# mstebelev/wormhole

Hardware: AMD Instinct MI355X
Metric: examples/sec, DiFacto FM on Criteo-1TB-shaped sparse at 1/2/4/8 MI355X (higher is better)
Workload: dtype fp32; 1 GPU; model=difacto-fm-dim64, global_batch=100000, seq_len=39, parallelism=dp1+kvshard1, minibatch_per_gpu=100000, threshold=100, nnz_per_example=39

## Files before the change

csrc/bind/hip_ops.cc:

```cpp
#include <torch/extension.h>
#include <pybind11/stl.h>
#include <c10/core/DeviceGuard.h>
#include <c10/hip/HIPStream.h>
#include <c10/hip/HIPGuard.h>
#include <c10/hip/HIPCachingAllocator.h>
#include <hip/hip_runtime.h>
#include <torch/csrc/distributed/c10d/ProcessGroup.hpp>
#include <torch/csrc/distributed/c10d/Work.hpp>

#include <algorithm>
#include <map>
#include <array>
#include <cstdio>
#include <cstdlib>
#include <cstring>
#include <chrono>
#include <cmath>
#include <functional>
#include <deque>
#include <map>
#include <mutex>
#include <condition_variable>
#include <thread>
#include <memory>
// ... 603 lines not shown
    wh::kv_occupied(table(), ptr<int32_t>(out), ptr<int64_t>(n), cur_stream(keys_));
    return out.narrow(0, 0, n.item<int64_t>());
  }

  Tensor linear_pull(const Tensor& slot) {
    CHECK_IN(slot, torch::kInt32);
    c10::DeviceGuard g(slot.device());
    auto out = torch::empty({slot.numel()}, slot.options().dtype(torch::kFloat32));
    wh::linear_pull(table(), ptr<int32_t>(slot), slot.numel(), ptr<float>(out), cur_stream(slot));
    return out;
  }

  void linear_push(const Tensor& slot, const Tensor& grad, int64_t algo, double alpha, double beta,
                   double l1, double l2, double sgd_eta) {
    CHECK_IN(slot, torch::kInt32);
    CHECK_IN(grad, torch::kFloat32);
    TORCH_CHECK(grad.numel() >= slot.numel());
    c10::DeviceGuard g(slot.device());
    wh::LinearHP hp{(int)algo, (float)alpha, (float)beta, (float)l1, (float)l2, (float)sgd_eta};
    wh::linear_push(table(), ptr<int32_t>(slot), ptr<float>(grad), slot.numel(), hp,
                    cur_stream(slot));
  }

  static wh::DifactoHP dhp(const std::vector<double>& h, int64_t threshold, bool l1_shrk,
                           int64_t seed) {
    TORCH_CHECK(h.size() == 8, "difacto hyper-parameter vector must have 8 entries");
    wh::DifactoHP hp;
    hp.alpha = (float)h[0]; hp.beta = (float)h[1]; hp.l1 = (float)h[2]; hp.l2 = (float)h[3];
    hp.v_alpha = (float)h[4]; hp.v_beta = (float)h[5]; hp.v_l2 = (float)h[6];
    hp.v_init = (float)h[7];
    hp.threshold = (uint32_t)threshold;
    hp.l1_shrk = l1_shrk ? 1 : 0;
    hp.seed = (uint64_t)seed;
    return hp;
  }

  void difacto_push_cnt(const Tensor& slot, const Tensor& cnt, const std::vector<double>& h,
                        int64_t threshold, bool l1_shrk, int64_t seed) {
    CHECK_IN(slot, torch::kInt32);
    CHECK_DEV(cnt); CHECK_CONT(cnt);
    TORCH_CHECK(cnt.scalar_type() == torch::kFloat32 || cnt.scalar_type() == torch::kInt32,
                "counts must be float32 or int32");
    TORCH_CHECK(cnt.numel() >= slot.numel());
    c10::DeviceGuard g(slot.device());
    const bool f = cnt.scalar_type() == torch::kFloat32;
    wh::difacto_push_cnt(table(), ptr<int32_t>(slot), f ? ptr<float>(cnt) : nullptr,
                         f ? nullptr : ptr<int32_t>(cnt), slot.numel(),
                         dhp(h, threshold, l1_shrk, seed), cur_stream(slot));
  }

  std::vector<Tensor> difacto_pull(const Tensor& slot, bool l1_shrk) {
    CHECK_IN(slot, torch::kInt32);
    c10::DeviceGuard g(slot.device());
    auto s = cur_stream(slot);
    const int64_t n = slot.numel();
    auto f32 = slot.options().dtype(torch::kFloat32);
    auto hdr = torch::empty({n, 2}, f32);
    const int64_t mcap = vstride_ > 0 ? n : 0;
    auto vc = torch::empty({mcap, (int64_t)std::max(vstride_, 1)}, f32);
    if (n > 0) {
      auto vpos = torch::empty({n + 1}, slot.options().dtype(torch::kInt64));
      if (wh::difacto_pull_fused(table(), ptr<int32_t>(slot), n, l1_shrk ? 1 : 0,
                                 lookback(slot.device()), ptr<float>(hdr), ptr<int64_t>(vpos),
                                 ptr<float>(vc), s))
        return {hdr, vc, vpos};
    }
    auto vflag = torch::empty({std::max<int64_t>(n, 1)}, slot.options());
    auto vpos = torch::zeros({n + 1}, slot.options().dtype(torch::kInt64));
    wh::difacto_pull_hdr(table(), ptr<int32_t>(slot), n, l1_shrk ? 1 : 0, ptr<float>(hdr),
                         ptr<int32_t>(vflag), s);
    if (vstride_ > 0 && n > 0) {
      auto stmp = torch::empty({wh::scan_tmp_elems(n)}, vpos.options());
      wh::scan_i32(ptr<int32_t>(vflag), ptr<int64_t>(vpos), n, ptr<int64_t>(stmp), s);
      wh::difacto_pull_rows(table(), ptr<int32_t>(slot), n, ptr<int32_t>(vflag),
                            ptr<int64_t>(vpos), ptr<float>(hdr), ptr<float>(vc), s);
    }
    return {hdr, vc, vpos};
  }

  std::vector<Tensor> difacto_open_pull(const Tensor& keys, bool insert,
                                        const c10::optional<Tensor>& cnt,
                                        const std::vector<double>& h, int64_t threshold,
                                        bool l1_shrk, int64_t seed, bool direct) {
    CHECK_IN(keys, torch::kInt64);
    const int32_t* cp = nullptr;
    if (cnt.has_value() && cnt->defined()) {
      CHECK_IN((*cnt), torch::kInt32);
      TORCH_CHECK(cnt->numel() >= keys.numel(), "open_pull: count size mismatch");
      cp = ptr<int32_t>(*cnt);
    }
    c10::DeviceGuard g(keys.device());
    auto s = cur_stream(keys);
    const int64_t n = keys.numel();
    auto f32 = keys.options().dtype(torch::kFloat32);
    auto slot = torch::empty({n}, keys.options().dtype(torch::kInt32));
    auto hdr = torch::empty({n, 2}, f32);
    auto vpos = torch::empty({n + 1}, keys.options());
    direct = direct && vstride_ > 0;
    auto vc = direct ? V_ : torch::empty({vstride_ > 0 ? n : 0, (int64_t)std::max(vstride_, 1)}, f32);
    if (n == 0) {
      vpos.zero_();
      return {slot, hdr, vc, vpos};
    }
    if (!wh::difacto_open_pull(table(), reinterpret_cast<const uint64_t*>(keys.data_ptr()), n,
                               cp, dhp(h, threshold, l1_shrk, seed), insert ? 1 : 0,
                               lookback(keys.device()), ptr<int32_t>(slot), ptr<float>(hdr),
                               ptr<int64_t>(vpos), direct ? nullptr : ptr<float>(vc), s)) {
      slot = find(keys, insert);
      if (cp) difacto_push_cnt(slot, *cnt, h, threshold, l1_shrk, seed);
      auto r = difacto_pull(slot, l1_shrk);
      return {slot, r[0], r[1], r[2]};
    }
    return {slot, hdr, vc, vpos};
  }

  void difacto_push(const Tensor& slot, const Tensor& hdr, const Tensor& gw, const Tensor& gvc,
                    const std::vector<double>& h, int64_t threshold, bool l1_shrk,
                    int64_t seed) {
    CHECK_IN(slot, torch::kInt32);
    CHECK_IN(hdr, torch::kFloat32);
    CHECK_IN(gw, torch::kFloat32);
    CHECK_DEV(gvc); CHECK_CONT(gvc); CHECK_DT(gvc, torch::kFloat32);
    const int64_t n = slot.numel();
    TORCH_CHECK(hdr.numel() == 2 * n && gw.numel() == n, "push: hdr/gw size mismatch");
    TORCH_CHECK(vstride_ == 0 || (gvc.dim() == 2 && gvc.size(1) == vstride_),
                "push: gvc must be [m, vstride]");
    c10::DeviceGuard g(slot.device());
    wh::difacto_push(table(), ptr<int32_t>(slot), ptr<float>(hdr), ptr<float>(gw),
                     gvc.numel() ? ptr<float>(gvc) : nullptr, n, dhp(h, threshold, l1_shrk, seed),
                     cur_stream(slot));
  }

  std::vector<Tensor> ps_open(const Tensor& keys, bool use_cnt, const Tensor& segS,
                              const Tensor& segHS, int64_t rows_cap, bool insert, bool chains,
                              const std::vector<double>& h, int64_t threshold, bool l1_shrk,
                              int64_t seed, const c10::optional<Tensor>& chain_in = c10::nullopt) {
    CHECK_DEV(keys); CHECK_CONT(keys);
    CHECK_IN(segS, torch::kInt64);
    CHECK_IN(segHS, torch::kInt64);
    const bool rec = keys.scalar_type() == torch::kInt32;
    TORCH_CHECK(rec ? (keys.dim() == 2 && keys.size(1) == 3) : keys.scalar_type() == torch::kInt64,
                "ps_open: keys must be int64 [n] or int32 records [n, 3]");
    TORCH_CHECK(!use_cnt || rec, "ps_open: counts travel in the records");
    const int64_t n = keys.size(0);
    const int P = (int)segS.numel() - 1;
    TORCH_CHECK(P >= 1 && segHS.numel() == P + 1, "ps_open: bad segment tables");
    TORCH_CHECK(n < (1 << 24), "ps_open: at most 2^24 - 1 keys per minibatch and shard");
    epoch_ = epoch_ % 255 + 1;
    ++opens_;
    TORCH_CHECK(vstride_ == 0 || rows_cap >= n, "ps_open: reply buffer too small");
    c10::DeviceGuard g(keys.device());
    auto s = cur_stream(keys);
    auto i32 = keys.options().dtype(torch::kInt32);
    auto f32 = keys.options().dtype(torch::kFloat32);
    const int64_t n1 = std::max<int64_t>(n, 1);
    int64_t at = 0;
    auto carve = [&](int64_t bytes) {
      const int64_t o = at;
      at += (bytes + 255) / 256 * 256;
      return o;
    };
    const int64_t o_s = carve(n1 * 4), o_w = carve(n1 * 4), o_p = carve((n + 1) * 8),
                  o_h = carve(n1);
    auto blk = torch::empty({at}, keys.options().dtype(torch::kUInt8));
    auto slot = blk.narrow(0, o_s, n1 * 4).view(torch::kInt32);
    auto wout = blk.narrow(0, o_w, n1 * 4).view(torch::kFloat32);
    auto vpos = blk.narrow(0, o_p, (n + 1) * 8).view(torch::kInt64);
    const bool prepped = chain_in.has_value() && chain_in->defined() && chain_in->numel() > 0;
    if (prepped) {
      CHECK_IN((*chain_in), torch::kInt32);
      TORCH_CHECK(chain_in->numel() >= std::max<int64_t>(n, 1), "ps_open: prepped chain too small");
      TORCH_CHECK(vbase_.defined(), "ps_open: prepped without a push prep");
    }
    auto chain = prepped ? *chain_in : torch::empty({n1}, i32);
    auto head = blk.narrow(0, o_h, n1);
    auto rbuf = torch::empty({vstride_ > 0 ? rows_cap : 0, (int64_t)std::max(vstride_, 1)}, f32);
    Tensor vcnt;
    if (vstride_ == 0) {
      if (!vcnt0_.defined() || vcnt0_.numel() != P || vcnt0_.device() != keys.device())
        vcnt0_ = torch::zeros({P}, keys.options().dtype(torch::kInt64));
      vcnt = vcnt0_;
    } else {
      vcnt = torch::empty({P}, keys.options().dtype(torch::kInt64));
    }
    if (!vbase_.defined()) vbase_ = torch::empty({1}, vnext_.options());
    const bool ok = wh::ps_open(
        table(), rec ? nullptr : reinterpret_cast<const uint64_t*>(keys.data_ptr()),
        rec ? ptr<int32_t>(keys) : nullptr, n, use_cnt ? 1 : 0, dhp(h, threshold, l1_shrk, seed),
        insert ? 1 : 0, chains ? 1 : 0, (uint32_t)epoch_, ptr<int32_t>(vbase_),
        ptr<int64_t>(segS), ptr<int64_t>(segHS), P, lookback(keys.device()), ptr<int32_t>(slot),
        ptr<float>(wout), ptr<int64_t>(vpos), reinterpret_cast<uint32_t*>(chain.data_ptr()),
        reinterpret_cast<uint8_t*>(head.data_ptr()), ptr<float>(rbuf), ptr<int64_t>(vcnt), s,
        prepped ? 1 : 0);
    TORCH_CHECK(ok, "ps_open: limits exceeded (P <= 256, n < 2^24)");
    return {slot.narrow(0, 0, n), vpos, chain.narrow(0, 0, n), head.narrow(0, 0, n),
            vstride_ > 0 ? rbuf : wout.narrow(0, 0, n), vcnt};
  }

  wh::PsPrep push_prep(const c10::optional<Tensor>& prep_chain, int64_t prep_n) {
    wh::PsPrep pr;
    if (!(prep_chain.has_value() && prep_chain->defined() && prep_chain->numel() > 0)) return pr;
    CHECK_IN((*prep_chain), torch::kInt32);
    TORCH_CHECK(prep_n >= 0 && prep_n <= prep_chain->numel(), "push prep: chain too small");
    if (!vbase_.defined()) vbase_ = torch::empty({1}, vnext_.options());
    pr.chain = reinterpret_cast<uint32_t*>(prep_chain->data_ptr());
    pr.n = prep_n;
    pr.vbase = ptr<int32_t>(vbase_);
    return pr;
  }

  void ps_push_linear(const Tensor& slot, const c10::optional<Tensor>& chain,
                      const c10::optional<Tensor>& head, const Tensor& segS, const Tensor& g,
                      int64_t algo, double alpha, double beta, double l1, double l2, double t0,
// ... 123 lines not shown
  int64_t opens_ = 0;

 private:
  void set_slots(const Tensor& sl) {
    slots_ = sl;
    auto as_i64 = slots_.view(torch::kInt64);
    auto as_f32 = slots_.view(torch::kFloat32);
    keys_ = as_i64.select(1, 0);
    w_ = as_f32.select(1, 2);
    z_ = as_f32.select(1, 3);
    sq_ = as_f32.select(1, 4);
    vrow_ = slots_.select(1, 5);
    cnt_ = slots_.select(1, 6);
  }

  int64_t cap_ = 0, vcap_ = 0, dim_ = 0;
  int vstride_ = 0;
};

static void check_vstride(int64_t vstride) {
  TORCH_CHECK(vstride == 0 || (vstride >= 4 && vstride <= 256 && (vstride & (vstride - 1)) == 0),
              "vstride must be 0 or 4 * 2^k <= 256, got ", vstride);
}

std::vector<Tensor> fm_forward(const Tensor& offset, const Tensor& lid,
                               const c10::optional<Tensor>& val, const Tensor& w_or_hdr,
                               const c10::optional<Tensor>& vc, int64_t vstride,
                               const Tensor& label, int64_t loss, const Tensor& met) {
  check_vstride(vstride);
  CHECK_IN(offset, torch::kInt64);
  CHECK_IN(lid, torch::kInt32);
  CHECK_IN(w_or_hdr, torch::kFloat32);
  CHECK_IN(label, torch::kFloat32);
  CHECK_IN(met, torch::kFloat64);
  TORCH_CHECK(met.numel() >= 4, "met needs 4 doubles");
  const int64_t nrows = offset.numel() - 1;
  TORCH_CHECK(label.numel() == nrows, "label size mismatch");
  const float* vcp = nullptr;
  if (vstride > 0) {
    TORCH_CHECK(w_or_hdr.dim() == 2 && w_or_hdr.size(1) == 2, "hdr must be [U, 2]");
    TORCH_CHECK(vc.has_value() && vc->defined(), "vc required");
    CHECK_IN((*vc), torch::kFloat32);
    TORCH_CHECK(vc->numel() == 0 || (vc->dim() == 2 && vc->size(1) == vstride), "vc must be [m, vstride]");
    vcp = vc->numel() ? ptr<float>(*vc) : nullptr;
  }
  const float* vp = optptr<float>(val);
  c10::DeviceGuard g(offset.device());
  int64_t at = 0;
  auto carve = [&](int64_t bytes) {
    const int64_t o = at;
    at += (bytes + 255) / 256 * 256;
    return o;
  };
  const int64_t nxv = vstride > 0 ? nrows * vstride : 0;
  const int64_t o_py = carve(nrows * 4), o_du = carve(nrows * 4), o_xv = carve(nxv * 4),
                o_pt = carve(wh::fm_fwd_partials() * 8);
  auto blk = torch::empty({std::max<int64_t>(at, 256)}, offset.options().dtype(torch::kUInt8));
  auto py = blk.narrow(0, o_py, nrows * 4).view(torch::kFloat32);
  auto dual = blk.narrow(0, o_du, nrows * 4).view(torch::kFloat32);
  auto xv = blk.narrow(0, o_xv, nxv * 4).view(torch::kFloat32);
  auto part = blk.narrow(0, o_pt, wh::fm_fwd_partials() * 8).view(torch::kFloat64);
  const int lossf = (int)loss | (met.numel() >= 5 ? 256 : 0);
  wh::fm_forward(nrows, ptr<int64_t>(offset), ptr<int32_t>(lid), vp, ptr<float>(w_or_hdr), vcp,
                 (int)vstride, ptr<float>(label), lossf, ptr<float>(py), ptr<float>(dual),
                 vstride > 0 ? ptr<float>(xv) : nullptr, ptr<double>(met), ptr<double>(part),
                 ptr<unsigned int>(dev_ws(offset.device()).fwd_ticket), cur_stream(offset));
  return {py, dual, xv};
}

static std::vector<Tensor> fm_bwd_alloc(const Tensor& csc_off, int64_t nnz, int64_t vc_rows,
                                        int64_t vstride, bool from_ws) {
  auto f32 = csc_off.options().dtype(torch::kFloat32);
  auto u8 = csc_off.options().dtype(torch::kUInt8);
  const int64_t U = csc_off.numel() - 1;
  const int64_t need = wh::fm_bwd_layout(U, nnz, (int)vstride, deterministic());
  Tensor fresh;
  Tensor& scratch = from_ws ? dev_ws(csc_off.device()).bwd_scratch[cur_stream(csc_off)] : fresh;
  if (!scratch.defined() || scratch.numel() < need)
    scratch = torch::empty({from_ws ? need + need / 4 : need}, u8);
  return {torch::empty({U}, f32),
          vstride > 0 ? torch::empty({vc_rows, vstride}, f32) : torch::empty({0}, f32), scratch};
}

static void fm_bwd_launch(const std::vector<Tensor>& pl, const Tensor& csc_off,
                          const Tensor& csc_row, const float* csc_val, const float* dual,
                          const float* xv, const float* hdr, const float* vc, int64_t vstride,
                          int64_t nrows, wh::FmBwdPhase phase, bool two_pass = false) {
  wh::FmBwdProblem p;
  p.nuniq = csc_off.numel() - 1;
  p.nnz = csc_row.numel();
  p.nrows = nrows;
  p.csc_off = ptr<int64_t>(csc_off);
  p.csc_row = ptr<int32_t>(csc_row);
  p.csc_val = csc_val;
  p.dual = dual;
  p.xv = xv;
  p.hdr = hdr;
  p.vc = vc;
  p.vstride = (int)vstride;
  p.gw = ptr<float>(pl[0]);
  p.gvc = pl[1].numel() ? ptr<float>(pl[1]) : nullptr;
  p.deterministic = deterministic();
  const wh::Lookback lb = lookback(csc_off.device());
  wh::fm_backward(p, pl[2].data_ptr(), two_pass ? nullptr : &lb, cur_stream(csc_off), phase);
}

static void fm_bwd_check(const Tensor& csc_off, const Tensor& csc_row, const Tensor& w_or_hdr,
                         int64_t vstride) {
  check_vstride(vstride);
  CHECK_IN(csc_off, torch::kInt64);
  CHECK_IN(csc_row, torch::kInt32);
  CHECK_IN(w_or_hdr, torch::kFloat32);
  TORCH_CHECK(w_or_hdr.numel() == (csc_off.numel() - 1) * (vstride > 0 ? 2 : 1),
              "w/hdr must have U rows");
}

static int64_t fm_bwd_check_run(const Tensor& dual, const c10::optional<Tensor>& xv,
                                const c10::optional<Tensor>& vc, int64_t vstride) {
  CHECK_IN(dual, torch::kFloat32);
  if (vstride == 0) return 0;
  TORCH_CHECK(vc.has_value() && vc->defined() && xv.has_value() && xv->defined(), "vc/xv required");
  CHECK_IN((*vc), torch::kFloat32);
  CHECK_IN((*xv), torch::kFloat32);
  return vc->numel() ? vc->size(0) : 0;
}

std::vector<Tensor> fm_backward(const Tensor& csc_off, const Tensor& csc_row,
                                const c10::optional<Tensor>& csc_val, const Tensor& dual,
                                const c10::optional<Tensor>& xv, const Tensor& w_or_hdr,
                                const c10::optional<Tensor>& vc, int64_t vstride) {
  fm_bwd_check(csc_off, csc_row, w_or_hdr, vstride);
  const int64_t vrows = fm_bwd_check_run(dual, xv, vc, vstride);
  c10::DeviceGuard g(csc_off.device());
  auto pl = fm_bwd_alloc(csc_off, csc_row.numel(), vrows, vstride, true);
  fm_bwd_launch(pl, csc_off, csc_row, optptr<float>(csc_val), ptr<float>(dual),
                vstride > 0 ? optptr<float>(xv) : nullptr, ptr<float>(w_or_hdr),
                vstride > 0 ? optptr<float>(vc) : nullptr, vstride, dual.numel(),
                wh::FmBwdPhase::kAll);
  return {pl[0], pl[1]};
}

std::vector<Tensor> fm_backward_plan(const Tensor& csc_off, const Tensor& csc_row,
                                     const Tensor& w_or_hdr, int64_t vc_rows, int64_t nrows,
                                     int64_t vstride, bool two_pass) {
  fm_bwd_check(csc_off, csc_row, w_or_hdr, vstride);
  TORCH_CHECK(vc_rows >= 0 && nrows >= 0, "bad sizes");
  c10::DeviceGuard g(csc_off.device());
  auto pl = fm_bwd_alloc(csc_off, csc_row.numel(), vc_rows, vstride, false);
  fm_bwd_launch(pl, csc_off, csc_row, nullptr, nullptr, nullptr, ptr<float>(w_or_hdr), nullptr,
                vstride, nrows, wh::FmBwdPhase::kPlan, two_pass);
  return pl;
}

std::vector<Tensor> fm_backward_run(const std::vector<Tensor>& plan, const Tensor& csc_off,
                                    const Tensor& csc_row, const c10::optional<Tensor>& csc_val,
                                    const Tensor& dual, const c10::optional<Tensor>& xv,
                                    const Tensor& w_or_hdr, const c10::optional<Tensor>& vc,
                                    int64_t vstride) {
  fm_bwd_check(csc_off, csc_row, w_or_hdr, vstride);
  const int64_t vrows = fm_bwd_check_run(dual, xv, vc, vstride);
  TORCH_CHECK(plan.size() == 3, "fm_backward_run: not a backward plan");
  const Tensor &gw = plan[0], &gvc = plan[1], &scratch = plan[2];
  CHECK_IN(gw, torch::kFloat32);
  CHECK_IN(gvc, torch::kFloat32);
  CHECK_IN(scratch, torch::kUInt8);
  const int64_t U = csc_off.numel() - 1;
  TORCH_CHECK(gw.numel() == U, "fm_backward_run: U differs from the plan's");
  TORCH_CHECK(vstride > 0 ? gvc.dim() == 2 && gvc.size(0) == vrows && gvc.size(1) == vstride
                          : gvc.numel() == 0,
              "fm_backward_run: vc rows or vstride differ from the plan's");
  TORCH_CHECK(scratch.numel() == wh::fm_bwd_layout(U, csc_row.numel(), (int)vstride, deterministic()),
              "fm_backward_run: the plan was made for a CSC of another size");
  c10::DeviceGuard g(csc_off.device());
  for (const Tensor& t : plan)
    if (t.numel())
      c10::hip::HIPCachingAllocator::recordStream(
          t.storage().data_ptr(), c10::hip::getCurrentHIPStream(csc_off.device().index()));
  fm_bwd_launch(plan, csc_off, csc_row, optptr<float>(csc_val), ptr<float>(dual),
                vstride > 0 ? optptr<float>(xv) : nullptr, ptr<float>(w_or_hdr),
                vstride > 0 ? optptr<float>(vc) : nullptr, vstride, dual.numel(),
                wh::FmBwdPhase::kRun);
  return {gw, gvc};
}

void fm_grad_post(const Tensor& gvc, const Tensor& m, int64_t dim, double clip, double dropout,
                  int64_t seed, bool normalize) {
  CHECK_IN(gvc, torch::kFloat32);
  CHECK_IN(m, torch::kInt64);
  if (gvc.numel() == 0) return;
  TORCH_CHECK(gvc.dim() == 2, "gvc must be [m, vstride]");
  const int64_t vstride = gvc.size(1);
  c10::DeviceGuard g(gvc.device());
  auto s = cur_stream(gvc);
  Tensor sumsq;
  if (normalize) sumsq = torch::zeros({1}, gvc.options().dtype(torch::kFloat64));
  wh::fm_grad_post(ptr<int64_t>(m), gvc.size(0), ptr<float>(gvc), (int)vstride, (int)dim,
                   (float)clip, (float)dropout, (uint64_t)seed,
                   normalize ? ptr<double>(sumsq) : nullptr, s);
  if (normalize)
    wh::fm_grad_scale(ptr<int64_t>(m), gvc.size(0), ptr<float>(gvc), (int)vstride, (int)dim,
                      ptr<double>(sumsq), s);
}

std::vector<Tensor> ps_unpack(const Tensor& rbuf, int64_t U, const Tensor& segS,
                              const Tensor& segHS, const Tensor& vrecv) {
  CHECK_IN(rbuf, torch::kFloat32);
  CHECK_IN(segS, torch::kInt64);
  CHECK_IN(segHS, torch::kInt64);
  CHECK_IN(vrecv, torch::kInt64);
  TORCH_CHECK(rbuf.dim() == 2, "ps_unpack: rbuf must be [R, vstride]");
  const int P = (int)segS.numel() - 1;
  TORCH_CHECK(segHS.numel() == P + 1 && vrecv.numel() == P, "ps_unpack: bad segment tables");
  c10::DeviceGuard g(rbuf.device());
  auto hdr = torch::empty({U, 2}, rbuf.options());
  auto rows = torch::empty({1}, segS.options());
  TORCH_CHECK(wh::ps_unpack(ptr<float>(rbuf), U, (int)rbuf.size(1), ptr<int64_t>(segS),
                            ptr<int64_t>(segHS), ptr<int64_t>(vrecv), P, ptr<float>(hdr),
                            ptr<int64_t>(rows), cur_stream(rbuf)),
              "ps_unpack: limits exceeded");
  return {hdr, rows};
}

Tensor ps_records(const Tensor& uniq, const c10::optional<Tensor>& ucnt) {
  CHECK_IN(uniq, torch::kInt64);
  const int32_t* cp = nullptr;
  if (ucnt.has_value() && ucnt->defined()) {
    CHECK_IN((*ucnt), torch::kInt32);
    TORCH_CHECK(ucnt->numel() == uniq.numel(), "ps_records: count size mismatch");
    cp = ptr<int32_t>(*ucnt);
  }
  c10::DeviceGuard g(uniq.device());
  auto rec = torch::empty({uniq.numel(), 3}, uniq.options().dtype(torch::kInt32));
  wh::ps_records(reinterpret_cast<const uint64_t*>(uniq.data_ptr()), cp, uniq.numel(),
                 ptr<int32_t>(rec), cur_stream(uniq));
  return rec;
}

std::vector<Tensor> ps_c0(const Tensor& owner_cnt, const c10::optional<Tensor>& vcnt, int64_t P,
                          int64_t flag, bool loopback = false) {
  CHECK_IN(owner_cnt, torch::kInt64);
  const int S = (int)owner_cnt.numel() - 1;
  TORCH_CHECK(S >= 1 && S <= P, "ps_c0: owner counts must cover 1..P shards");
  const int64_t* vp = nullptr;
  if (vcnt.has_value() && vcnt->defined()) {
    CHECK_IN((*vcnt), torch::kInt64);
    TORCH_CHECK(vcnt->numel() == P, "ps_c0: vcnt size mismatch");
    vp = ptr<int64_t>(*vcnt);
  }
  c10::DeviceGuard g(owner_cnt.device());
  auto send = torch::empty({4 * P}, owner_cnt.options());
  auto payload = torch::empty({S + 1 + 5 * P}, owner_cnt.options());
  TORCH_CHECK(wh::ps_c0(ptr<int64_t>(owner_cnt), vp, S, (int)P, flag, ptr<int64_t>(send),
                        ptr<int64_t>(payload), cur_stream(owner_cnt), loopback ? 1 : 0),
              "ps_c0: too many peers");
  return {send, payload};
}

void ps_pack_gw(const Tensor& gw, const Tensor& gbuf, const Tensor& segS, const Tensor& segHS,
                const Tensor& vrecv) {
  CHECK_IN(gw, torch::kFloat32);
  CHECK_IN(gbuf, torch::kFloat32);
  CHECK_IN(segS, torch::kInt64);
  CHECK_IN(segHS, torch::kInt64);
  CHECK_IN(vrecv, torch::kInt64);
  TORCH_CHECK(gbuf.dim() == 2, "ps_pack_gw: gbuf must be [R, vstride]");
// ... 1839 lines not shown
#include "step_common.inl"
#include "linear_step.inl"

#include "rccl_comm.h"
#include "psx_native.inl"
#include "difacto_step.inl"

PYBIND11_MODULE(_hip, m) {
  m.doc() = "wormhole_amd gfx950 HIP kernels";
  m.def("scan_excl", &scan_excl);
  py::class_<LocalizeJob>(m, "LocalizeJob")
      .def(py::init<const Tensor&, const Tensor&, const c10::optional<Tensor>&, int64_t, int64_t,
                    py::object, bool>(),
           py::arg("keys"), py::arg("offset"), py::arg("val") = py::none(), py::arg("nshard") = 1,
           py::arg("hint") = 0, py::arg("exchange") = py::none(),
           py::arg("defer_exchange") = false)
      .def("exchange", &LocalizeJob::exchange)
      .def("counts", &LocalizeJob::counts)
      .def("finish", &LocalizeJob::finish);
  m.def("loc_timing_read", []() { return loc_timing_buf().clone(); });
  m.def("loc_retries", []() { return loc_retries(); },
        "localize jobs redone on the hash path after a partition overflow (count)");
  py::class_<LinearStep>(m, "LinearStep")
      .def(py::init<KVStore*, int64_t, double, double, double, double, int64_t, double, bool>(),
           py::arg("store"), py::arg("algo"), py::arg("alpha"), py::arg("beta"), py::arg("l1"),
           py::arg("l2"), py::arg("loss"), py::arg("max_load") = 0.7, py::arg("direct") = true,
           py::keep_alive<1, 2>())
      .def("step", &LinearStep::step, py::arg("keys"), py::arg("offset"), py::arg("val"),
           py::arg("label"), py::arg("train"), py::arg("met"), py::arg("auc_sum"),
           py::arg("next_keys") = py::none(), py::arg("next_offset") = py::none(),
           py::arg("next_val") = py::none(), py::arg("ready") = 0)
      .def("reset", &LinearStep::reset)
      .def("guard_sync", &LinearStep::guard_sync)
      .def_property_readonly("grows", &LinearStep::grows)
      .def_property_readonly("direct", [](const LinearStep& l) { return l.direct(); })
      .def_property("pushes", &LinearStep::pushes, &LinearStep::set_pushes);
  py::class_<RcclComm, std::shared_ptr<RcclComm>>(m, "RcclComm")
      .def(py::init<const std::string&, int64_t, int64_t, int64_t>(), py::arg("uid"),
           py::arg("nranks"), py::arg("rank"), py::arg("device"))
      .def_static("unique_id", &RcclComm::unique_id)
      .def("close", &RcclComm::close)
      .def("a2av", &RcclComm::a2av_t, py::arg("x"), py::arg("send_rows"), py::arg("recv_rows"))
      .def("allreduce_sum", [](RcclComm& c, Tensor t) { c.allreduce_sum(t); })
      .def_property_readonly("size", &RcclComm::size)
      .def_property_readonly("rank", &RcclComm::rank)
      .def_property_readonly("device", &RcclComm::device);
  m.attr("PSX_TX_IDENTITY") = (int)kTxIdentity;
  m.attr("PSX_TX_RCCL") = (int)kTxRccl;
  m.attr("PSX_TX_STAGED") = (int)kTxStaged;
  py::class_<PsxStep>(m, "PsxStep")
      .def(py::init<KVStore*, int64_t, int64_t, int64_t, int64_t, py::object, py::object, bool,
                    std::vector<double>, std::vector<double>, int64_t, bool, int64_t, int64_t,
                    Tensor, Tensor, int64_t, double, int64_t, std::vector<int64_t>,
                    std::vector<double>>(),
           py::arg("store"), py::arg("P"), py::arg("S"), py::arg("rank"), py::arg("tx"),
           py::arg("pg"), py::arg("rccl"), py::arg("linear"), py::arg("lin_hp"), py::arg("hp"), py::arg("threshold"),
           py::arg("l1_shrk"), py::arg("seed"), py::arg("loss"), py::arg("met"),
           py::arg("auc_sum"), py::arg("tau"), py::arg("max_load"), py::arg("cu_reserve"),
           py::arg("filt") = std::vector<int64_t>{0, 0},
           py::arg("post") = std::vector<double>{0.0, 0.0, 0.0, 0.0},
           py::keep_alive<1, 2>())
      .def("train", &PsxStep::train, py::arg("keys"), py::arg("offset"), py::arg("val"),
           py::arg("label"), py::arg("data_pass"), py::arg("next_keys") = py::none(),
           py::arg("next_offset") = py::none(), py::arg("next_val") = py::none(),
           py::arg("ready") = 0)
      .def("flush", &PsxStep::flush)
      .def("drop_job", &PsxStep::drop_job)
      .def("guard_sync", &PsxStep::guard_sync)
      .def("wire", &PsxStep::wire)
      .def("wire_reset", &PsxStep::wire_reset)
      .def("xtime", &PsxStep::xtime,
           "sampled GPU us per exchange C0..C3 and the sample counts (RCCL transport)")
      .def_property_readonly("watchdog_deadline", &PsxStep::watchdog_deadline)
      .def_property_readonly("busy", &PsxStep::busy)
      .def_property_readonly("grows", &PsxStep::grows)
      .def_property_readonly("vgrows", &PsxStep::vgrows)
      .def_property("requests", &PsxStep::requests, &PsxStep::set_requests)
      .def_property("step", &PsxStep::step, &PsxStep::set_step);
  m.def("a2a_plan", &a2a_plan_py, py::arg("rank"), py::arg("world"), py::arg("row_bytes"),
        py::arg("send_rows"), py::arg("recv_rows"),
        "one rank's per-peer all-to-all-v plan: (esz, (own_src, own_dst, own_bytes), sends, recvs)");
  py::class_<DifactoStep>(m, "DifactoStep")
      .def(py::init<KVStore*, std::vector<double>, int64_t, bool, int64_t, int64_t,
                    std::vector<double>, double, bool>(),
           py::arg("store"), py::arg("hp"), py::arg("threshold"), py::arg("l1_shrk"),
           py::arg("seed"), py::arg("loss"), py::arg("post"), py::arg("max_load"),
           py::arg("direct"), py::keep_alive<1, 2>())
      .def("step", &DifactoStep::step, py::arg("keys"), py::arg("offset"), py::arg("val"),
           py::arg("label"), py::arg("train"), py::arg("data_pass"), py::arg("met"),
           py::arg("auc_sum"), py::arg("step"), py::arg("next_keys") = py::none(),
           py::arg("next_offset") = py::none(), py::arg("next_val") = py::none(),
           py::arg("ready") = 0)
      .def("reset", &DifactoStep::reset)
      .def("guard_sync", &DifactoStep::guard_sync)
      .def_property_readonly("direct", &DifactoStep::direct)
      .def_property_readonly("grows", &DifactoStep::grows)
      .def_property_readonly("vgrows", &DifactoStep::vgrows);
  m.def("c10d_a2a_rows", &c10d_a2a_rows, py::arg("pg"), py::arg("x"), py::arg("send_rows"),
        py::arg("recv_rows"));
  m.def("localize", &localize, py::arg("keys"), py::arg("offset"), py::arg("val") = py::none(),
        py::arg("nshard") = 1, py::arg("hint") = 0, py::arg("exchange") = py::none());
  m.def("fm_forward", &fm_forward);
  m.def("set_cu_reserve", [](int64_t n) { wh::fm_set_cu_reserve((int)n); },
        "CUs the persistent FM kernels leave free for concurrent collectives");
  m.def("cu_reserve", []() { return (int64_t)wh::fm_cu_reserve(); });
  m.def("fm_backward", &fm_backward);
  m.def("fm_backward_plan", &fm_backward_plan, py::arg("csc_off"), py::arg("csc_row"),
        py::arg("hdr"), py::arg("vc_rows"), py::arg("nrows"), py::arg("vstride"),
        py::arg("two_pass") = false);
  m.def("fm_backward_run", &fm_backward_run);
  m.def("fm_grad_post", &fm_grad_post);
  m.def("vidx_renumber", &vidx_renumber);
  m.def("ps_unpack", &ps_unpack);
  m.def("ps_pack_gw", &ps_pack_gw);
  m.def("ps_records", &ps_records);
  m.def("ps_c0", &ps_c0, py::arg("owner_cnt"), py::arg("vcnt"), py::arg("P"), py::arg("flag"),
        py::arg("loopback") = false);
  m.def("auc", &auc);
  m.def("quant_rows", &quant_rows);
  m.def("key_mod", &key_mod);
  m.def("dequant_rows", &dequant_rows);
  m.def("trunc_u8", &trunc_u8);
  m.def("ps_qpack", &ps_qpack, py::arg("x"), py::arg("desc"), py::arg("rows"), py::arg("W"),
        py::arg("nb"), py::arg("seed"));
  m.def("ps_qunpack", &ps_qunpack, py::arg("q"), py::arg("desc"), py::arg("W"), py::arg("nb"),
        py::arg("out"));
  m.def("auc_acc", &auc_acc);
  m.def("auc_acc_side", &auc_acc_side);
  m.def("auc_join", &auc_join);
  m.def("auc_host_threads", [](int n) { HostAuc::enable(n); },
        "large training minibatches' AUC on n host threads (0: the device chain)");
  m.def("timing_flush", &timing_flush);
  m.def("auc_sorted", &auc_sorted);
  m.def("synth_criteo", &synth_criteo);
  m.def("gather_rows", &gather_rows);
  m.def("vstride_for", &vstride_for);
  m.def("spmv", &spmv, py::arg("offset"), py::arg("col"), py::arg("val"), py::arg("x"));
  m.def("gbdt_bin", &gbdt_bin);
  m.def("gbdt_hist", &gbdt_hist, py::arg("B"), py::arg("nbin"), py::arg("ridx"), py::arg("gpair"),
        py::arg("qscale"), py::arg("tasks"), py::arg("red"), py::arg("max_fcnt"), py::arg("hist"));
  m.def("gbdt_partition", &gbdt_partition, py::arg("B"), py::arg("ridx"), py::arg("pos_node"),
        py::arg("node_feat"), py::arg("node_bin"), py::arg("node_defl"), py::arg("seg_beg"),
        py::arg("seg_end"), py::arg("nleft"), py::arg("Bc") = py::none());
  m.def("gbdt_seg_fill", &gbdt_seg_fill);
  m.def("gbdt_split", &gbdt_split);
  m.def("owlqn_dir", &owlqn_dir, py::arg("g"), py::arg("w"), py::arg("l1"),
        py::arg("out") = py::none());
  m.def("owlqn_fix_dot", &owlqn_fix_dot);
  m.def("owlqn_step", &owlqn_step);
  m.def("multi_dot", &multi_dot);
  m.def("hist_dots", &hist_dots, py::arg("H"), py::arg("probes"));
  m.def("dir_fix_dot", &dir_fix_dot, py::arg("H"), py::arg("rows"), py::arg("coef"),
        py::arg("steep_row"), py::arg("fix"), py::arg("n") = -1);
  m.def("glm_heads", &glm_heads, py::arg("csc_off"), py::arg("nnz"));
  m.def("glm_fwd", &glm_fwd, py::arg("mode"), py::arg("offset"), py::arg("gcol"), py::arg("val"),
        py::arg("w"), py::arg("bias"), py::arg("base"), py::arg("label"), py::arg("loss"));
  m.def("glm_xtg", &glm_xtg, py::arg("crow"), py::arg("cval"), py::arg("hb"), py::arg("col0"),
        py::arg("ucol"), py::arg("g"), py::arg("grad"), py::arg("all_atomic") = false);
  m.def("glm_grad_from_margin", &glm_grad_from_margin, py::arg("margin"), py::arg("label"),
        py::arg("loss"));
  m.def("glm_runs_reduce", &glm_runs_reduce, py::arg("coff"), py::arg("rlist"), py::arg("S"),
        py::arg("cgid"), py::arg("grad"));
  m.def("gbdt_leaf_add", &gbdt_leaf_add);
  m.def("gbdt_leaf_walk", &gbdt_leaf_walk, py::arg("B"), py::arg("feat"), py::arg("bin"),
        py::arg("defl"), py::arg("left"), py::arg("right"), py::arg("val"), py::arg("margin"),
        py::arg("lds") = true, "margins += the tree's leaf per row (lds: the LDS-resident walk "
        "when the tree and row tile fit; else the global-memory walk)");
  m.def("gbdt_predict", &gbdt_predict);
  m.def("kmeans_pack_x", &kmeans_pack_x);
  m.def("kmeans_pack_c", &kmeans_pack_c);
  m.def("kmeans_assign", &kmeans_assign);
  m.def("kmeans_accum", &kmeans_accum);
  m.def("kmeans_update", &kmeans_update);
  m.def("kmeans_assign_csr", &kmeans_assign_csr, py::arg("offset"), py::arg("col"),
        py::arg("val"), py::arg("Ct"), py::arg("K"));
  m.def("kmeans_accum_csr", &kmeans_accum_csr, py::arg("offset"), py::arg("col"), py::arg("val"),
        py::arg("assign"), py::arg("K"), py::arg("F"));
  m.def("kmeans_pack_x3", &kmeans_pack_x3);
  m.def("gbdt_grow", &gbdt_grow, py::arg("B"), py::arg("Bc"), py::arg("ridx0"), py::arg("gpair"),
        py::arg("qscale"), py::arg("valid"), py::arg("nbin"), py::arg("fgroups"), py::arg("max_fcnt"),
        py::arg("root_tot"), py::arg("cut_vals"), py::arg("cut_off"), py::arg("eta"), py::arg("alpha"),
        py::arg("reg_lambda"), py::arg("min_child_weight"), py::arg("max_depth"), py::arg("rt_eps"),
        py::arg("allreduce"));
  m.def("gbdt_grow_dev", &gbdt_grow_dev, py::arg("B"), py::arg("Bc"), py::arg("ridx0"), py::arg("gpair"),
        py::arg("qscale"), py::arg("valid"), py::arg("nbin"), py::arg("fgroups"), py::arg("max_fcnt"),
        py::arg("root_tot"), py::arg("cut_vals"), py::arg("cut_off"), py::arg("eta"), py::arg("alpha"),
        py::arg("reg_lambda"), py::arg("min_child_weight"), py::arg("max_depth"), py::arg("rt_eps"),
        py::arg("allreduce"), py::arg("reduce_scatter") = py::none(), py::arg("pick") = py::none(),
        py::arg("f_lo") = 0, py::arg("walk") = false, py::arg("defer") = false);
  m.def("gbdt_tree_from_nodes", &gbdt_tree_from_nodes);
  m.def("gbdt_walk_heap", &gbdt_walk_heap, py::arg("B"), py::arg("nodes"), py::arg("margin"),
        py::arg("lds") = true);
  m.def("gbdt_gpair", &gbdt_gpair);
  m.def("gbdt_gpair_softmax", &gbdt_gpair_softmax);
  m.def("gbdt_softmax_out", &gbdt_softmax_out);
  m.def("gbdt_multi_eval", &gbdt_multi_eval);
  m.def("gbdt_qscale", &gbdt_qscale);
  m.def("parse_criteo", &parse_criteo, py::call_guard<py::gil_scoped_release>());
  m.def("parse_libsvm", &parse_libsvm, py::call_guard<py::gil_scoped_release>());
  m.def("csr_gather", &csr_gather, py::call_guard<py::gil_scoped_release>());
  m.def("gbdt_bin_csr", &gbdt_bin_csr);
  m.def("gbdt_hist_csr", &gbdt_hist_csr);
  m.def("gbdt_split_csr", &gbdt_split_csr);
  m.def("gbdt_partition_csr", &gbdt_partition_csr);
  m.def("gbdt_predict_csr", &gbdt_predict_csr);
  m.def("kmeans_pack_c3", &kmeans_pack_c3);
  m.def("kmeans_assign_x3", &kmeans_assign_x3);
  m.def("spmv_t", &spmv_t, py::arg("csc_off"), py::arg("csc_row"), py::arg("csc_val"),
        py::arg("p"));
  py::class_<KVStore>(m, "KVStore")
      .def(py::init<int64_t, int64_t, int64_t, int64_t>(), py::arg("cap"), py::arg("vcap"),
           py::arg("dim"), py::arg("device"))
      .def("find", &KVStore::find)
      .def("occupied", &KVStore::occupied)
      .def("linear_pull", &KVStore::linear_pull)
      .def("linear_push", &KVStore::linear_push)
      .def("difacto_push_cnt", &KVStore::difacto_push_cnt)
      .def("difacto_pull", &KVStore::difacto_pull)
      .def("difacto_open_pull", &KVStore::difacto_open_pull, py::arg("keys"), py::arg("insert"),
           py::arg("cnt"), py::arg("h"), py::arg("threshold"), py::arg("l1_shrk"), py::arg("seed"),
           py::arg("direct") = false)
      .def("difacto_push", &KVStore::difacto_push)
      .def("ps_open", &KVStore::ps_open, py::arg("keys"), py::arg("use_cnt"), py::arg("segS"),
           py::arg("segHS"), py::arg("rows_cap"), py::arg("insert"), py::arg("chains"), py::arg("h"),
           py::arg("threshold"), py::arg("l1_shrk"), py::arg("seed"),
           py::arg("chain_in") = py::none())
      .def("ps_push", &KVStore::ps_push, py::arg("slot"), py::arg("vpos"), py::arg("chain"),
           py::arg("head"), py::arg("segS"), py::arg("segHS"), py::arg("gbuf"), py::arg("h"),
           py::arg("threshold"), py::arg("l1_shrk"), py::arg("seed"),
           py::arg("prep_chain") = py::none(), py::arg("prep_n") = 0)
      .def("ps_push_linear", &KVStore::ps_push_linear, py::arg("slot"), py::arg("chain"),
           py::arg("head"), py::arg("segS"), py::arg("g"), py::arg("algo"), py::arg("alpha"),
           py::arg("beta"), py::arg("l1"), py::arg("l2"), py::arg("t0"),
           py::arg("prep_chain") = py::none(), py::arg("prep_n") = 0)
      .def("grow", &KVStore::grow)
      .def("grow_v", &KVStore::grow_v)
      .def("summary", &KVStore::summary)
      .def("summary_async", &KVStore::summary_async)
      .def("summary_read", &KVStore::summary_read)
      .def_property_readonly("dim", &KVStore::dim)
      .def_property_readonly("vstride", &KVStore::vstride)
      .def_property_readonly("cap", &KVStore::cap)
      .def_property_readonly("vcap", &KVStore::vcap)
      .def_readonly("ps_opens", &KVStore::opens_)
      .def_readonly("slots", &KVStore::slots_)
      .def_readonly("keys", &KVStore::keys_)
      .def_readonly("w", &KVStore::w_)
      .def_readonly("z", &KVStore::z_)
      .def_readonly("sq", &KVStore::sq_)
      .def_readonly("cnt", &KVStore::cnt_)
      .def_readonly("vrow", &KVStore::vrow_)
      .def_readonly("V", &KVStore::V_)
      .def_readonly("VG", &KVStore::VG_)
      .def_readonly("vnext", &KVStore::vnext_)
      .def_property_readonly("stats", [](const KVStore& k) {
        return k.stats_.narrow(1, 0, wh::kStatCount).sum(0);
      })
      .def("reset_stats", [](KVStore& k, int64_t i0, int64_t i1) {
        k.stats_.narrow(1, i0, i1 - i0).zero_();
      })
      .def("add_stat", [](KVStore& k, int64_t i, int64_t v) {
        k.stats_.select(1, i).narrow(0, 0, 1).add_(v);
      });
}
```

csrc/hip/fm.hip:

```cpp
#include "wh_common.h"
#include <string>
#include "wh_kernels.h"
#include "wh_lookback.h"
#include "wh_loss.h"

#include <algorithm>
#include <cstdlib>
#include <type_traits>

namespace wh {
namespace {

constexpr int kThreads = 256;
constexpr int kChunk = 32;
constexpr int kFwdBlocks = 2048;

template <int G>
struct Shape {
  static constexpr int SUB = 64 / G;
  static constexpr int NI = G;
#ifndef WH_FM_TI
#define WH_FM_TI 4
#endif
  static constexpr int TI = G < WH_FM_TI ? G : WH_FM_TI;
  static constexpr int VS = 4 * G;
};

__device__ float kZeroRow[256];

template <int G>
__device__ __forceinline__ void stage_pairs(int2* st, int lane, int idx_val, float f) {
  using S = Shape<G>;
  st[(lane % S::SUB) * S::NI + lane / S::SUB] = make_int2(idx_val, __float_as_int(f));
  __builtin_amdgcn_fence(__ATOMIC_RELEASE, "wavefront");
  __builtin_amdgcn_wave_barrier();
  __builtin_amdgcn_fence(__ATOMIC_ACQUIRE, "wavefront");
}

template <int G>
__device__ __forceinline__ int stage_pairs_compact(int2* st, int lane, int vid, float f) {
  using S = Shape<G>;
  const bool has = vid >= 0;
  const uint64_t m = __ballot(has);
  const int nv = __popcll(m);
  const int pos = __popcll(m & ((1ull << lane) - 1ull));
  if (has) st[(pos % S::SUB) * S::NI + pos / S::SUB] = make_int2(vid, __float_as_int(f));
  __builtin_amdgcn_fence(__ATOMIC_RELEASE, "wavefront");
  __builtin_amdgcn_wave_barrier();
  __builtin_amdgcn_fence(__ATOMIC_ACQUIRE, "wavefront");
  return nv;
}

template <int G>
__global__ __launch_bounds__(kThreads) void k_fm_fwd(int64_t nrows, const int64_t* __restrict__ off,
                                                     const int32_t* __restrict__ lid,
                                                     const float* __restrict__ val,
                                                     const float2* __restrict__ hdr,
                                                     const float* __restrict__ vc, int vstride,
                                                     const float* __restrict__ label, int loss,
                                                     float* __restrict__ py_out,
                                                     float* __restrict__ dual_out,
                                                     float* __restrict__ xv, double* part,
                                                     double* met, unsigned int* ticket, int acc5) {
  using S = Shape<G>;
  __shared__ double sh[kThreads / 64];
  __shared__ int2 stage[kThreads / 64][64];
  const int lane = threadIdx.x & 63, gl = lane & (G - 1), sub = lane / G;
  const int64_t nw = (int64_t)gridDim.x * (kThreads / 64);
  const int64_t w0 =
      __builtin_amdgcn_readfirstlane((int)(((int64_t)blockIdx.x * kThreads + threadIdx.x) >> 6));
  double m_objv = 0, m_objw = 0, m_corr = 0, m_n = 0;
  auto bounds = [&](int64_t r, int64_t& b, int64_t& e) {
    if (r < nrows) {
      b = off[r];
      e = off[r + 1];
    } else {
      b = e = 0;
    }
  };
  auto load_ids = [&](int64_t b, int64_t e, int& l, float& x) {
    const bool ok = b + lane < e;
    l = ok ? lid[b + lane] : -1;
    x = ok ? (val ? val[b + lane] : 1.f) : 0.f;
  };
  auto load_hdr = [&](int l) {
    return l >= 0 ? hdr[l] : make_float2(0.f, __int_as_float(-1));
  };
  int2* st = stage[threadIdx.x >> 6];
  auto gather = [&](int vid, float x, float4& s, float4& q2, bool prefetch_first,
                    auto&& prefetch) {
    const int n = stage_pairs_compact<G>(st, lane, vid, x);
#pragma unroll
    for (int t0 = 0; t0 < S::NI; t0 += S::TI) {
      if (t0 * S::SUB >= n) break;
      float4 v[S::TI];
      float xs[S::TI];
#pragma unroll
// ... 30 lines not shown
    bool fetched = false;
    auto prefetch = [&]() {
      hn = load_hdr(ln);
      load_ids(b2, e2, l2, x2);
      bounds(r + 3 * nw, b3, e3);
      fetched = true;
    };
    gather(__float_as_int(hc.y), xc, s, q2, true, prefetch);
    if (!fetched) prefetch();
    for (int64_t pb = bc + 64; pb < ec; pb += 64) {
      int l;
      float x;
      load_ids(pb, ec, l, x);
      const float2 h = load_hdr(l);
      wl += x * h.x;
      gather(__float_as_int(h.y), x, s, q2, false, prefetch);
    }
#pragma unroll
    for (int o = G; o < 64; o <<= 1) {
      s.x += __shfl_xor(s.x, o, 64); s.y += __shfl_xor(s.y, o, 64);
      s.z += __shfl_xor(s.z, o, 64); s.w += __shfl_xor(s.w, o, 64);
      q2.x += __shfl_xor(q2.x, o, 64); q2.y += __shfl_xor(q2.y, o, 64);
      q2.z += __shfl_xor(q2.z, o, 64); q2.w += __shfl_xor(q2.w, o, 64);
    }
    const float wsum = wave_sum(wl);
    float pt = (s.x * s.x - q2.x) + (s.y * s.y - q2.y) + (s.z * s.z - q2.z) + (s.w * s.w - q2.w);
    pt = group_sum<G>(pt);
    if (sub == 0) reinterpret_cast<float4*>(xv + r * vstride)[gl] = s;
    if (lane == 0) {
      const float p = wsum + 0.5f * pt;
      const float y = label[r];
      const LossOut o = eval_loss(loss, y, p);
      const LossOut ow = eval_loss(loss, y, wsum);
      py_out[r] = p;
      dual_out[r] = o.dual;
      m_objv += o.objv;
      m_objw += ow.objv;
      m_corr += ((y > 0.f && p > 0.f) || (y <= 0.f && p <= 0.f)) ? 1.0 : 0.0;
      m_n += 1.0;
    }
    bc = bn; ec = en; xc = xn; hc = hn;
    bn = b2; en = e2; ln = l2; xn = x2;
    b2 = b3; e2 = e3;
  }
  block_partials(part, sh, m_objv, m_objw, m_corr, m_n, met, ticket, acc5);
}

template <int G>
__global__ __launch_bounds__(kThreads) void k_lin_fwd(int64_t nrows, const int64_t* __restrict__ off,
                                                      const int32_t* __restrict__ lid,
                                                      const float* __restrict__ val,
                                                      const float* __restrict__ w, int wstride,
                                                      const float* __restrict__ label, int loss,
                                                      float* __restrict__ py_out,
                                                      float* __restrict__ dual_out, double* part,
                                                      double* met, unsigned int* ticket, int acc5) {
  __shared__ double sh[kThreads / 64];
  const int gl = threadIdx.x & (G - 1);
  const int64_t ngroups = (int64_t)gridDim.x * (kThreads / G);
  double m_objv = 0, m_corr = 0, m_n = 0;
  for (int64_t row = ((int64_t)blockIdx.x * kThreads + threadIdx.x) / G; row < nrows;
       row += ngroups) {
    float acc = 0.f;
    const int64_t b = off[row], e = off[row + 1];
    for (int64_t j = b + gl; j < e; j += G) {
      const int32_t l = lid[j];
      if (wstride == 1) acc += (val ? val[j] : 1.f) * w[l];
      else if (l >= 0) acc += (val ? val[j] : 1.f) * w[(int64_t)l * wstride];
    }
    acc = group_sum<G>(acc);
    if (gl == 0) {
      const float y = label[row];
      const LossOut o = eval_loss(loss, y, acc);
      py_out[row] = acc;
      dual_out[row] = o.dual;
      m_objv += o.objv;
      m_corr += ((y > 0.f && acc > 0.f) || (y <= 0.f && acc <= 0.f)) ? 1.0 : 0.0;
      m_n += 1.0;
    }
  }
  block_partials(part, sh, m_objv, m_objv, m_corr, m_n, met, ticket, acc5);
}

constexpr int kChunkV = 64;

__device__ __forceinline__ int64_t key_chunks(int64_t cnt, bool isv) {
  return isv ? (cnt + kChunkV - 1) / kChunkV : (cnt + kChunk - 1) / kChunk;
}

__device__ __forceinline__ int32_t key_vidx(const float2* __restrict__ hdr, int64_t k) {
  return hdr ? __float_as_int(hdr[k].y) : -1;
}

struct ChunkOut {
  int32_t* key_s;
  int32_t* beg_s;
  int4* meta_v;
  float* gw;
  float* gvc;
  int vstride;
};

__device__ __forceinline__ void emit_key(const ChunkOut& o, int32_t k, int64_t c0, int32_t nc,
                                         int32_t b0, int32_t cnt, int32_t vid, int isv) {
  const int lane = threadIdx.x & 63;
  if (nc == 1) {
    if (isv) {
      o.meta_v[c0] = make_int4(k, b0, cnt, vid);
    } else {
      o.key_s[c0] = k;
      o.beg_s[c0] = b0;
    }
  }
  uint64_t m = __ballot(nc > 1);
  while (m) {
    const int src = __ffsll((unsigned long long)m) - 1;
    m &= m - 1;
    const int32_t jk = __shfl(k, src, 64);
    const int64_t jc0 = __shfl(c0, src, 64);
    const int32_t jnc = __shfl(nc, src, 64);
    const int32_t jb0 = __shfl(b0, src, 64);
    const int32_t jcnt = __shfl(cnt, src, 64);
    const int32_t jvid = __shfl(vid, src, 64);
    const int jv = __shfl(isv, src, 64);
    for (int32_t q = lane; q < jnc; q += 64) {
      if (jv) {
        const int32_t cb = q * kChunkV;
        const int32_t n = jcnt - cb < kChunkV ? jcnt - cb : kChunkV;
        o.meta_v[jc0 + q] = make_int4(jk, jb0 + cb, n | (1 << 8), jvid);
      } else {
        o.key_s[jc0 + q] = jk;
        o.beg_s[jc0 + q] = jb0 + q * kChunk;
      }
    }
    if (lane == 0) o.gw[jk] = 0.f;
    if (jv) {
      for (int d = lane * 4; d < o.vstride; d += 256)
        *reinterpret_cast<float4*>(o.gvc + (int64_t)jvid * o.vstride + d) =
            make_float4(0.f, 0.f, 0.f, 0.f);
    }
  }
}

__global__ __launch_bounds__(kThreads) void k_chunk_count(int64_t nuniq,
                                                          const int64_t* __restrict__ csc_off,
                                                          const float2* __restrict__ hdr,
                                                          int64_t* cnt_s, int64_t* cnt_v) {
  const int64_t k = (int64_t)blockIdx.x * kThreads + threadIdx.x;
  if (k < nuniq) {
    const bool isv = key_vidx(hdr, k) >= 0;
    const int64_t n = key_chunks(csc_off[k + 1] - csc_off[k], isv);
    cnt_s[k] = isv ? 0 : n;
    cnt_v[k] = isv ? n : 0;
  }
}

__global__ __launch_bounds__(kThreads) void k_chunk_fill(int64_t nuniq,
                                                         const int64_t* __restrict__ csc_off,
                                                         const int64_t* __restrict__ off_s,
                                                         const int64_t* __restrict__ off_v,
                                                         const float2* __restrict__ hdr,
                                                         ChunkOut out) {
  const int64_t k = (int64_t)blockIdx.x * kThreads + threadIdx.x;
  int64_t c0 = 0;
  int32_t nc = 0, b0 = 0, cnt = 0, vid = -1;
  if (k < nuniq) {
    vid = key_vidx(hdr, k);
    const int64_t* off = vid >= 0 ? off_v : off_s;
    c0 = off[k];
    nc = (int32_t)(off[k + 1] - c0);
    b0 = (int32_t)csc_off[k];
    cnt = (int32_t)(csc_off[k + 1] - b0);
  }
  emit_key(out, (int32_t)k, c0, nc, b0, cnt, vid, vid >= 0);
}

constexpr int kPlanPer = 4;
constexpr int kPlanTile = kThreads * kPlanPer;

__global__ __launch_bounds__(kThreads) void k_chunk_plan(int64_t nuniq,
                                                         const int64_t* __restrict__ csc_off,
                                                         const float2* __restrict__ hdr,
                                                         Lookback lb, int ntiles,
                                                         int64_t* off_s_tot, int64_t* off_v_tot,
                                                         ChunkOut out) {
  __shared__ uint32_t shs[16];
  __shared__ int sht;
  const int tile = lb_tile(lb, ntiles, &sht);
  const int64_t k0 = (int64_t)tile * kPlanTile + threadIdx.x * kPlanPer;
  int64_t co[kPlanPer + 1];
#pragma unroll
  for (int r = 0; r <= kPlanPer; ++r) co[r] = k0 + r <= nuniq ? csc_off[k0 + r] : 0;
  int32_t vid[kPlanPer];
#pragma unroll
  for (int r = 0; r < kPlanPer; ++r) vid[r] = k0 + r < nuniq ? key_vidx(hdr, k0 + r) : -1;
  uint32_t c[2] = {0u, 0u};
  uint32_t nc[kPlanPer];
#pragma unroll
  for (int r = 0; r < kPlanPer; ++r) {
    nc[r] = k0 + r < nuniq ? (uint32_t)key_chunks(co[r + 1] - co[r], vid[r] >= 0) : 0u;
    c[vid[r] >= 0 ? 1 : 0] += nc[r];
  }
  uint32_t ex[2], tot[2];
  lb_block_scan<2>(lb, tile, c, ex, tot, shs);
  if (tile == ntiles - 1 && threadIdx.x == 0) {
    *off_s_tot = tot[0];
    *off_v_tot = tot[1];
  }
#pragma unroll
  for (int r = 0; r < kPlanPer; ++r) {
    const int isv = vid[r] >= 0;
    emit_key(out, (int32_t)(k0 + r), isv ? ex[1] : ex[0], (int32_t)nc[r], (int32_t)co[r],
             (int32_t)(co[r + 1] - co[r]), vid[r], isv);
    ex[isv ? 1 : 0] += nc[r];
  }
}

constexpr int kBuckets = 256;
constexpr int kBucketBlocks = 128;
constexpr int kBucketU = 8;

__device__ __forceinline__ int row_bucket(int row, int shift) {
  const int b = row >> shift;
  return b < kBuckets ? b : kBuckets - 1;
// ... 29 lines not shown
constexpr int kScanParts = 4;
constexpr int kScanPer = kBucketBlocks / kScanParts;

__global__ __launch_bounds__(kBuckets * kScanParts) void k_vchunk_scan(int32_t* hist) {
  __shared__ int32_t part[kScanParts][kBuckets];
  __shared__ int32_t excl[kBuckets];
  __shared__ int32_t wtot[kBuckets / 64];
  const int b = threadIdx.x & (kBuckets - 1), q = threadIdx.x / kBuckets;
  int32_t v[kScanPer];
#pragma unroll
  for (int i = 0; i < kScanPer; ++i) v[i] = hist[(q * kScanPer + i) * kBuckets + b];
  int32_t sum = 0;
#pragma unroll
  for (int i = 0; i < kScanPer; ++i) sum += v[i];
  part[q][b] = sum;
  __syncthreads();
  if (q == 0) {
    int32_t t = 0;
#pragma unroll
    for (int r = 0; r < kScanParts; ++r) t += part[r][b];
    const int lane = b & 63;
    int32_t x = t;
#pragma unroll
    for (int o = 1; o < 64; o <<= 1) {
      const int32_t y = __shfl_up(x, o, 64);
      if (lane >= o) x += y;
    }
    if (lane == 63) wtot[b >> 6] = x;
    excl[b] = x - t;
  }
  __syncthreads();
  int32_t base = excl[b];
  for (int w = 0; w < (b >> 6); ++w) base += wtot[w];
  for (int r = 0; r < q; ++r) base += part[r][b];
#pragma unroll
  for (int i = 0; i < kScanPer; ++i) {
    hist[(q * kScanPer + i) * kBuckets + b] = base;
    base += v[i];
  }
}

__global__ __launch_bounds__(kThreads) void k_vchunk_scatter(const int64_t* __restrict__ nchunk_p,
                                                             const int4* __restrict__ meta,
                                                             const int32_t* __restrict__ csc_row,
                                                             int shift,
                                                             const int32_t* __restrict__ hist,
                                                             int4* out) {
  __shared__ int32_t base[kBuckets];
  for (int i = threadIdx.x; i < kBuckets; i += kThreads) base[i] = hist[blockIdx.x * kBuckets + i];
  __syncthreads();
  const int64_t n = *nchunk_p;
  const int64_t per = (n + gridDim.x - 1) / gridDim.x;
  const int64_t c0 = per * blockIdx.x, c1 = c0 + per < n ? c0 + per : n;
  for (int64_t cb = c0 + threadIdx.x; cb < c1; cb += kThreads * kBucketU) {
    int4 m[kBucketU];
    int row[kBucketU];
#pragma unroll
    for (int u = 0; u < kBucketU; ++u) {
      const int64_t c = cb + (int64_t)u * kThreads;
      m[u] = c < c1 ? meta[c] : make_int4(0, -1, 0, 0);
    }
#pragma unroll
    for (int u = 0; u < kBucketU; ++u) row[u] = m[u].y >= 0 ? csc_row[m[u].y] : -1;
#pragma unroll
    for (int u = 0; u < kBucketU; ++u)
      if (row[u] >= 0) out[atomicAdd(&base[row_bucket(row[u], shift)], 1)] = m[u];
  }
}

__global__ __launch_bounds__(kThreads) void k_bwd_scalar(const int64_t* __restrict__ nchunk_p,
                                                         const int32_t* __restrict__ chunk_key,
                                                         const int32_t* __restrict__ chunk_beg,
                                                         const int64_t* __restrict__ csc_off,
                                                         const int32_t* __restrict__ csc_row,
                                                         const float* __restrict__ csc_val,
                                                         const float* __restrict__ dual,
                                                         float* __restrict__ gw_out,
                                                         float* __restrict__ part_gw) {
  const int64_t c = (int64_t)blockIdx.x * kThreads + threadIdx.x;
  if (c >= *nchunk_p) return;
  const int k = chunk_key[c];
  const int kb = (int)csc_off[k], ke = (int)csc_off[k + 1];
  const int b = chunk_beg[c];
  const int e = b + kChunk < ke ? b + kChunk : ke;
  float gw = 0.f;
  int p = b;
  for (; p + 3 < e; p += 4) {
    int i[4];
    float x[4];
#pragma unroll
    for (int u = 0; u < 4; ++u) {
      i[u] = csc_row[p + u];
      x[u] = csc_val ? csc_val[p + u] : 1.f;
    }
#pragma unroll
    for (int u = 0; u < 4; ++u) gw += dual[i[u]] * x[u];
  }
  for (; p < e; ++p) gw += dual[csc_row[p]] * (csc_val ? csc_val[p] : 1.f);
  if (ke - kb <= kChunk) gw_out[k] = gw;
  else if (part_gw) part_gw[c] = gw;
  else atomicAdd(gw_out + k, gw);
}

template <int G>
__global__ __launch_bounds__(kThreads) void k_bwd_v(const int64_t* __restrict__ nchunk_p,
                                                    const int4* __restrict__ meta,
                                                    const int32_t* __restrict__ csc_row,
                                                    const float* __restrict__ csc_val,
                                                    const float* __restrict__ dual,
                                                    const float* __restrict__ xv,
                                                    const float* __restrict__ vc, int vstride,
                                                    float* __restrict__ gw_out,
                                                    float* __restrict__ gvc,
                                                    float* __restrict__ part_gw,
                                                    float* __restrict__ part_gv) {
  using S = Shape<G>;
  __shared__ int2 stage[kThreads / 64][64];
  int2* st = stage[threadIdx.x >> 6];
  const int lane = threadIdx.x & 63, gl = lane & (G - 1), sub = lane / G;
  const int64_t nch = *nchunk_p, nw = (int64_t)gridDim.x * (kThreads / 64);
  const int64_t w0 =
      __builtin_amdgcn_readfirstlane((int)(((int64_t)blockIdx.x * kThreads + threadIdx.x) >> 6));
  auto get_meta = [&](int64_t c) {
    return c < nch ? meta[c] : make_int4(0, 0, 0, -1);
  };
  auto load_rows = [&](const int4& mt, int& r, float& x) {
    const bool ok = lane < (mt.z & 0xff);
    r = ok ? csc_row[mt.y + lane] : -1;
    x = ok ? (csc_val ? csc_val[mt.y + lane] : 1.f) : 0.f;
  };
  int64_t c = w0;
  int4 mc = get_meta(c), mn = get_meta(c + nw), m2 = get_meta(c + 2 * nw),
       m3 = make_int4(0, 0, 0, -1);
  int rc, rn, r2 = -1;
  float xc, xn, x2 = 0.f;
  load_rows(mc, rc, xc);
  float dc = rc >= 0 ? dual[rc] * xc : 0.f;
  load_rows(mn, rn, xn);
  float dn = 0.f;
  for (; c < nch; c += nw) {
    const int n = mc.z & 0xff;
    const bool multi = (mc.z >> 8) != 0;
    float4 acc = make_float4(0.f, 0.f, 0.f, 0.f);
    float4 v = make_float4(0.f, 0.f, 0.f, 0.f);
    stage_pairs<G>(st, lane, rc, dc);
    auto batch = [&](auto tb, int t0) {
      constexpr int TB = decltype(tb)::value;
      float4 a[TB];
      float du[TB];
#pragma unroll
      for (int t = 0; t < TB; ++t) {
        const int2 e = st[sub * S::NI + t0 + t];
        du[t] = __int_as_float(e.y);
        const float* src = e.x >= 0 ? xv + (uint32_t)e.x * (uint32_t)S::VS : kZeroRow;
        a[t] = reinterpret_cast<const float4*>(src)[gl];
      }
      if (t0 == 0) {
        v = reinterpret_cast<const float4*>(vc + (uint32_t)mc.w * (uint32_t)S::VS)[gl];
        dn = rn >= 0 ? dual[rn] * xn : 0.f;
        load_rows(m2, r2, x2);
        m3 = get_meta(c + 3 * nw);
      }
#pragma unroll
      for (int t = 0; t < TB; ++t) {
        acc.x += du[t] * a[t].x; acc.y += du[t] * a[t].y;
        acc.z += du[t] * a[t].z; acc.w += du[t] * a[t].w;
      }
    };
    if (n > S::NI * S::SUB / 2) {
      batch(std::integral_constant<int, S::NI>(), 0);
    } else {
#pragma unroll
      for (int t0 = 0; t0 < S::NI; t0 += S::TI) {
        if (t0 * S::SUB >= n) break;
        batch(std::integral_constant<int, S::TI>(), t0);
      }
    }
    if (n == 0) {
      dn = rn >= 0 ? dual[rn] * xn : 0.f;
      load_rows(m2, r2, x2);
      m3 = get_meta(c + 3 * nw);
    }
    const float gw = wave_sum(dc);
    const float xxp = wave_sum(dc * xc);
#pragma unroll
    for (int o = G; o < 64; o <<= 1) {
      acc.x += __shfl_xor(acc.x, o, 64); acc.y += __shfl_xor(acc.y, o, 64);
      acc.z += __shfl_xor(acc.z, o, 64); acc.w += __shfl_xor(acc.w, o, 64);
    }
    if (lane == 0) {
      if (!multi) gw_out[mc.x] = gw;
      else if (part_gw) part_gw[c] = gw;
      else atomicAdd(gw_out + mc.x, gw);
    }
    acc.x -= xxp * v.x; acc.y -= xxp * v.y; acc.z -= xxp * v.z; acc.w -= xxp * v.w;
    if (!multi || part_gv) {
      float* dst = multi ? part_gv + c * (int64_t)vstride : gvc + (int64_t)mc.w * vstride;
      if (sub == 0) *reinterpret_cast<float4*>(dst + gl * 4) = acc;
    } else {
      float* gv = gvc + (int64_t)mc.w * vstride;
#pragma unroll
      for (int c = 0; c < (S::VS + 63) / 64; ++c) {
        const int d = c * 64 + lane;
        const int src = (d >> 2) & (G - 1);
        const float ax = __shfl(acc.x, src, 64), ay = __shfl(acc.y, src, 64);
        const float az = __shfl(acc.z, src, 64), aw = __shfl(acc.w, src, 64);
        const int comp = d & 3;
        const float a = comp == 0 ? ax : comp == 1 ? ay : comp == 2 ? az : aw;
        if (d < S::VS) atomicAdd(gv + d, a);
      }
    }
    mc = mn; rc = rn; xc = xn; dc = dn;
    mn = m2; rn = r2; xn = x2;
    m2 = m3;
  }
}

__global__ __launch_bounds__(kThreads) void k_bwd_reduce_s(const int64_t* __restrict__ nchunk_p,
                                                           const int32_t* __restrict__ chunk_key,
                                                           const int32_t* __restrict__ chunk_beg,
                                                           const int64_t* __restrict__ csc_off,
                                                           const float* __restrict__ part_gw,
                                                           float* __restrict__ gw_out) {
  const int64_t c = (int64_t)blockIdx.x * kThreads + threadIdx.x;
  if (c >= *nchunk_p) return;
  const int k = chunk_key[c];
  const int64_t kb = csc_off[k], cnt = csc_off[k + 1] - kb;
  if (cnt <= kChunk || chunk_beg[c] != kb) return;
  const int64_t n = (cnt + kChunk - 1) / kChunk;
  float s = 0.f;
  for (int64_t q = 0; q < n; ++q) s += part_gw[c + q];
  gw_out[k] = s;
}

__global__ __launch_bounds__(kThreads) void k_bwd_reduce_v(const int64_t* __restrict__ nchunk_p,
                                                           const int4* __restrict__ meta,
                                                           const int64_t* __restrict__ csc_off,
                                                           const float* __restrict__ part_gw,
                                                           const float* __restrict__ part_gv,
                                                           int vstride, float* __restrict__ gw_out,
                                                           float* __restrict__ gvc) {
  const int lane = threadIdx.x & 63;
  const int64_t c = ((int64_t)blockIdx.x * kThreads + threadIdx.x) >> 6;
  if (c >= *nchunk_p) return;
  const int4 m = meta[c];
  if ((m.z >> 8) == 0 || (int64_t)m.y != csc_off[m.x]) return;
  const int64_t cnt = csc_off[m.x + 1] - m.y;
  const int64_t n = (cnt + kChunkV - 1) / kChunkV;
  float g = 0.f;
  for (int64_t q = 0; q < n; ++q) g += part_gw[c + q];
  for (int d = lane; d < vstride; d += 64) {
    float a = 0.f;
    for (int64_t q = 0; q < n; ++q) a += part_gv[(c + q) * vstride + d];
    gvc[(int64_t)m.w * vstride + d] = a;
  }
  if (lane == 0) gw_out[m.x] = g;
}

__global__ __launch_bounds__(kThreads) void k_grad_post(const int64_t* __restrict__ m_p,
                                                        float* gvc, int vstride, int dim,
                                                        float clip, float dropout, uint64_t seed,
                                                        double* sumsq) {
  __shared__ double sh[kThreads / 64];
  const int64_t total = *m_p * vstride;
  double ss = 0;
  for (int64_t t = (int64_t)blockIdx.x * kThreads + threadIdx.x; t < total;
       t += (int64_t)gridDim.x * kThreads) {
    const int64_t r = t / vstride;
    const int d = (int)(t % vstride);
    if (d >= dim) continue;
    float v = gvc[t];
    if (clip > 0.f) v = fminf(fmaxf(v, -clip), clip);
    if (dropout > 0.f && uhash01(seed, (uint64_t)r, (uint64_t)d) > 1.f - dropout) v = 0.f;
    gvc[t] = v;
    ss += (double)v * v;
  }
  if (sumsq) {
    const double s = block_sum_d(ss, sh);
    if (threadIdx.x == 0) atomicAdd(sumsq, s);
  }
}

__global__ __launch_bounds__(kThreads) void k_grad_scale(const int64_t* __restrict__ m_p,
                                                         float* gvc, int vstride, int dim,
                                                         const double* sumsq) {
  const int64_t t = (int64_t)blockIdx.x * kThreads + threadIdx.x;
  const double n2 = *sumsq;
  if (n2 < 1e-10 || t / vstride >= *m_p || (int)(t % vstride) >= dim) return;
  gvc[t] = (float)(gvc[t] / sqrt(n2));
}

}

template <typename F>
static void dispatch_g(int G, F&& f) {
  switch (G) {
    case 1: f(std::integral_constant<int, 1>()); break;
    case 2: f(std::integral_constant<int, 2>()); break;
    case 4: f(std::integral_constant<int, 4>()); break;
    case 8: f(std::integral_constant<int, 8>()); break;
    case 16: f(std::integral_constant<int, 16>()); break;
    case 32: f(std::integral_constant<int, 32>()); break;
    case 64: f(std::integral_constant<int, 64>()); break;
    default:
      fprintf(stderr, "fm.hip: no kernel for vstride %d (4 * 2^k <= 256 only)\n", 4 * G);
      abort();
  }
}

int64_t fm_fwd_partials() { return 4 * kFwdBlocks; }
int64_t fwd_ticket_words() { return kArriveWords; }

static int g_cu_reserve = 0;

void fm_set_cu_reserve(int cus) { g_cu_reserve = cus < 0 ? 0 : cus; }
int fm_cu_reserve() { return g_cu_reserve; }

static int device_cus() {
  static int cus = 0;
  if (cus == 0) {
    int dev = 0;
    WH_HIP_CHECK(hipGetDevice(&dev));
    WH_HIP_CHECK(hipDeviceGetAttribute(&cus, hipDeviceAttributeMultiprocessorCount, dev));
  }
  return std::max(1, cus - std::min(g_cu_reserve, cus / 2));
}

template <typename K>
static int resident_blocks(K kernel, int cap) {
  const int cus = device_cus();
  int per_cu = 0;
  WH_HIP_CHECK(hipOccupancyMaxActiveBlocksPerMultiprocessor(&per_cu, kernel, kThreads, 0));
  const int n = std::max(1, per_cu) * cus;
  return n < cap ? n : cap;
}

void fm_forward(int64_t nrows, const int64_t* offset, const int32_t* lid, const float* val,
                const float* w_or_hdr, const float* vc, int vstride, const float* label, int loss,
                float* py, float* dual, float* xv, double* met, double* part,
                unsigned int* ticket, hipStream_t s) {
  if (nrows <= 0) return;
  const int acc5 = (loss >> 8) & 1;
  loss &= 0xff;
  if (vstride == 0) {
    constexpr int G = 8;
    const int nblk = grid_for(nrows * G, kThreads, kFwdBlocks);
    hipLaunchKernelGGL(k_lin_fwd<G>, dim3(nblk), dim3(kThreads), 0, s, nrows, offset, lid, val,
                       w_or_hdr, 1, label, loss, py, dual, part, met, ticket, acc5);
    return;
  }
  const float2* hdr = reinterpret_cast<const float2*>(w_or_hdr);
  dispatch_g(vstride / 4, [&](auto g) {
    constexpr int G = decltype(g)::value;
    const int nblk =
        grid_for(nrows * 64, kThreads, resident_blocks(k_fm_fwd<G>, kFwdBlocks));
    hipLaunchKernelGGL(k_fm_fwd<G>, dim3(nblk), dim3(kThreads), 0, s, nrows, offset, lid, val,
                       hdr, vc, vstride, label, loss, py, dual, xv, part, met, ticket, acc5);
  });
}

void lin_forward_strided(int64_t nrows, const int64_t* offset, const int32_t* lid,
                         const float* val, const float* w, int wstride, const float* label,
                         int loss, float* py, float* dual, double* met, double* part,
                         unsigned int* ticket, hipStream_t s) {
  if (nrows <= 0) return;
  const int acc5 = (loss >> 8) & 1;
  loss &= 0xff;
  constexpr int G = 8;
  const int nblk = grid_for(nrows * G, kThreads, kFwdBlocks);
  hipLaunchKernelGGL(k_lin_fwd<G>, dim3(nblk), dim3(kThreads), 0, s, nrows, offset, lid, val, w,
                     wstride, label, loss, py, dual, part, met, ticket, acc5);
}

static int64_t scalar_cap(int64_t nuniq, int64_t nnz) { return nuniq + nnz / kChunk + 1; }
static int64_t v_cap(int64_t nuniq, int64_t nnz) { return nuniq + nnz / kChunkV + 1; }

static int bucket_shift(int64_t nrows) {
  int shift = 0;
  while ((((nrows - 1) >> shift) >= kBuckets)) ++shift;
  return shift;
}

int64_t fm_bwd_layout(int64_t nuniq, int64_t nnz, int vstride, bool deterministic,
                      FmBwdLayout* out) {
  int64_t at = 0;
  auto carve = [&](int64_t bytes) {
    const int64_t o = at;
    at += (bytes + 255) / 256 * 256;
    return o;
  };
  const int64_t cap_s = scalar_cap(nuniq, nnz), cap_v = vstride > 0 ? v_cap(nuniq, nnz) : 0;
  FmBwdLayout l;
  l.key_s = carve(cap_s * 4);
  l.beg_s = carve(cap_s * 4);
  l.meta_v = carve(2 * cap_v * 16);
  l.hist = carve(vstride > 0 ? (int64_t)kBuckets * kBucketBlocks * 4 : 0);
  l.det_s = carve(deterministic ? cap_s * 4 : 0);
  l.det_vw = carve(deterministic ? cap_v * 4 : 0);
  l.det_v = carve(deterministic ? cap_v * vstride * 4 : 0);
  l.off = carve(2 * (nuniq + 1) * 8);
  l.cnt = carve(2 * nuniq * 8);
  l.scan_tmp = carve(scan_tmp_elems(nuniq) * 8);
  if (out) *out = l;
  return at;
}

void fm_backward(const FmBwdProblem& p, void* scratch, const Lookback* lb, hipStream_t s,
                 FmBwdPhase phase) {
  const int64_t nuniq = p.nuniq;
  if (nuniq <= 0) return;
  const int vstride = p.vstride;
  const float2* hdr = vstride > 0 ? reinterpret_cast<const float2*>(p.hdr) : nullptr;
  FmBwdLayout l;
  fm_bwd_layout(nuniq, p.nnz, vstride, p.deterministic, &l);
  char* base = static_cast<char*>(scratch);
  int32_t* key_s = reinterpret_cast<int32_t*>(base + l.key_s);
  int32_t* beg_s = reinterpret_cast<int32_t*>(base + l.beg_s);
  int4* meta_v = reinterpret_cast<int4*>(base + l.meta_v);
  int64_t* off_s = reinterpret_cast<int64_t*>(base + l.off);
  int64_t* off_v = off_s + nuniq + 1;
  const int64_t cap_s = scalar_cap(nuniq, p.nnz), cap_v = v_cap(nuniq, p.nnz);
  const bool bucket =
      hdr && !p.deterministic && p.nrows * (int64_t)vstride * 4 > ((int64_t)2 << 20);
  int4* meta_sorted = bucket ? meta_v + cap_v : meta_v;
  if (phase != FmBwdPhase::kRun) {
    const ChunkOut out = {key_s, beg_s, meta_v, p.gw, p.gvc, vstride};
    const int64_t ntiles = (nuniq + kPlanTile - 1) / kPlanTile;
    if (lb && ntiles <= kLbMaxTiles) {
      hipLaunchKernelGGL(k_chunk_plan, dim3((unsigned)ntiles), dim3(kThreads), 0, s, nuniq,
                         p.csc_off, hdr, *lb, (int)ntiles, off_s + nuniq, off_v + nuniq, out);
    } else {
      int64_t* cnt_s = reinterpret_cast<int64_t*>(base + l.cnt);
      int64_t* cnt_v = cnt_s + nuniq;
      int64_t* scan_tmp = reinterpret_cast<int64_t*>(base + l.scan_tmp);
      const dim3 grid(grid_for(nuniq, kThreads));
      hipLaunchKernelGGL(k_chunk_count, grid, dim3(kThreads), 0, s, nuniq, p.csc_off, hdr, cnt_s,
                         cnt_v);
      scan_i64(cnt_s, off_s, nuniq, scan_tmp, s);
      if (hdr) scan_i64(cnt_v, off_v, nuniq, scan_tmp, s);
      hipLaunchKernelGGL(k_chunk_fill, grid, dim3(kThreads), 0, s, nuniq, p.csc_off, off_s, off_v,
                         hdr, out);
    }
    if (bucket) {
      int32_t* hist = reinterpret_cast<int32_t*>(base + l.hist);
      const int shift = bucket_shift(std::max<int64_t>(p.nrows, 1));
      hipLaunchKernelGGL(k_vchunk_hist, dim3(kBucketBlocks), dim3(kThreads), 0, s, off_v + nuniq,
                         meta_v, p.csc_row, shift, hist);
      hipLaunchKernelGGL(k_vchunk_scan, dim3(1), dim3(kBuckets * kScanParts), 0, s, hist);
      hipLaunchKernelGGL(k_vchunk_scatter, dim3(kBucketBlocks), dim3(kThreads), 0, s,
                         off_v + nuniq, meta_v, p.csc_row, shift, hist, meta_sorted);
    }
  }
  if (phase == FmBwdPhase::kPlan) return;
  const bool det = p.deterministic;
  float* pgs = det ? reinterpret_cast<float*>(base + l.det_s) : nullptr;
  float* pgv_w = det ? reinterpret_cast<float*>(base + l.det_vw) : nullptr;
  float* pgv = det ? reinterpret_cast<float*>(base + l.det_v) : nullptr;
  hipLaunchKernelGGL(k_bwd_scalar, dim3(grid_for(cap_s, kThreads)), dim3(kThreads), 0, s,
                     off_s + nuniq, key_s, beg_s, p.csc_off, p.csc_row, p.csc_val, p.dual, p.gw,
                     pgs);
  if (det)
    hipLaunchKernelGGL(k_bwd_reduce_s, dim3(grid_for(cap_s, kThreads)), dim3(kThreads), 0, s,
                       off_s + nuniq, key_s, beg_s, p.csc_off, pgs, p.gw);
  if (!hdr) return;
  dispatch_g(vstride / 4, [&](auto g) {
    constexpr int G = decltype(g)::value;
    const int64_t vblk =
        std::min<int64_t>((cap_v + 3) / 4, resident_blocks(k_bwd_v<G>, 2048));
    hipLaunchKernelGGL(k_bwd_v<G>, dim3((unsigned)vblk), dim3(kThreads), 0, s, off_v + nuniq,
                       meta_sorted, p.csc_row, p.csc_val, p.dual, p.xv, p.vc, vstride, p.gw,
                       p.gvc, pgv_w, pgv);
  });
  if (det)
    hipLaunchKernelGGL(k_bwd_reduce_v, dim3(grid_for(cap_v * 64, kThreads)), dim3(kThreads), 0, s,
                       off_v + nuniq, meta_v, p.csc_off, pgv_w, pgv, vstride, p.gw, p.gvc);
}

void fm_grad_post(const int64_t* m, int64_t m_cap, float* gvc, int vstride, int dim, float clip,
                  float dropout, uint64_t seed, double* sumsq, hipStream_t s) {
  if (m_cap <= 0 || vstride == 0) return;
  hipLaunchKernelGGL(k_grad_post, dim3(grid_for(m_cap * vstride, kThreads, 1024)), dim3(kThreads),
                     0, s, m, gvc, vstride, dim, clip, dropout, seed, sumsq);
}

void fm_grad_scale(const int64_t* m, int64_t m_cap, float* gvc, int vstride, int dim,
                   const double* sumsq, hipStream_t s) {
  if (m_cap <= 0 || vstride == 0) return;
  hipLaunchKernelGGL(k_grad_scale, dim3(grid_for(m_cap * vstride, kThreads)), dim3(kThreads), 0,
                     s, m, gvc, vstride, dim, sumsq);
}

}
```

csrc/hip/kv_device.h:

```cpp
#pragma once
#include "wh_common.h"
#include "wh_kernels.h"

namespace wh {
namespace kvd {

constexpr int kThreads = 256;
constexpr int kMaxProbe = 256;
constexpr int kPullPer = 4;
constexpr int kPullTile = kThreads * kPullPer;
constexpr int kRowBatch = 8;
constexpr int kPushBatch = 4;

__device__ __forceinline__ uint64_t ld_relaxed(const uint64_t* p) {
  return __hip_atomic_load(p, __ATOMIC_RELAXED, __HIP_MEMORY_SCOPE_AGENT);
}
__device__ __forceinline__ int32_t ld_relaxed_i32(const int32_t* p) {
  return __hip_atomic_load(p, __ATOMIC_RELAXED, __HIP_MEMORY_SCOPE_AGENT);
}

__device__ __forceinline__ unsigned long long* stat_ptr(int64_t* stats, int idx) {
  const int shard =
      (int)((blockIdx.x * (blockDim.x >> 6) + (threadIdx.x >> 6)) & (kStatShards - 1));
  return reinterpret_cast<unsigned long long*>(stats + shard * kStatStride + idx);
}

__device__ __forceinline__ int32_t probe_slot(KVSlot* sl, uint64_t mask, uint64_t k, uint64_t h,
                                              uint64_t pv, int insert, bool* created) {
  for (int probe = 0; probe < kMaxProbe; ++probe) {
    if (pv == k) return (int32_t)h;
    if (pv == kEmptyKey) {
      if (!insert) return -1;
      const uint64_t old = atomicCAS((unsigned long long*)(&sl[h].key),
                                     (unsigned long long)kEmptyKey, (unsigned long long)k);
      if (old == kEmptyKey) { *created = true; return (int32_t)h; }
      if (old == k) return (int32_t)h;
    }
    h = (h + 1) & mask;
    pv = ld_relaxed(&sl[h].key);
  }
  return -1;
}

__device__ __forceinline__ int32_t wave_alloc_rows(const KVTable& t, bool want) {
  const uint64_t m = __ballot(want);
  if (!m) return -1;
  const int lane = threadIdx.x & 63;
  int32_t base = 0;
  const int leader = __ffsll((unsigned long long)m) - 1;
  if (lane == leader) base = atomicAdd(t.vnext, (int)__popcll(m));
  base = __shfl(base, leader, 64);
  if (!want) return -1;
  const int32_t row = base + (int32_t)__popcll(m & ((1ull << lane) - 1));
  if (row >= t.vcap) {
    atomicAdd(stat_ptr(t.stats, 3), 1ull);
    return -1;
  }
  return row;
}

__device__ __forceinline__ float v_init_val(const DifactoHP& hp, uint64_t key, int d, int dim) {
  return d < dim ? (uhash01(hp.seed, key, (uint64_t)d) * 2.f - 1.f) * hp.v_init : 0.f;
}

__device__ __forceinline__ float4 v_init4(const DifactoHP& hp, uint64_t key, int c, int dim) {
  return make_float4(v_init_val(hp, key, c, dim), v_init_val(hp, key, c + 1, dim),
                     v_init_val(hp, key, c + 2, dim), v_init_val(hp, key, c + 3, dim));
}

__device__ __forceinline__ void init_v_row(const KVTable& t, uint64_t key, int32_t row, int gl,
                                           int G, const DifactoHP& hp) {
  float* V = t.V + (int64_t)row * t.vstride;
  float* VG = t.VG + (int64_t)row * t.vstride;
  for (int c = gl * 4; c < t.vstride; c += 4 * G) {
    *reinterpret_cast<float4*>(V + c) = v_init4(hp, key, c, t.dim);
    *reinterpret_cast<float4*>(VG + c) = make_float4(0.f, 0.f, 0.f, 0.f);
  }
}

__device__ __forceinline__ float difacto_ftrl(float w, float gw, float& sq, float& z,
                                              const DifactoHP& hp) {
  const float g = gw + hp.l2 * w;
  const float cg = sq;
  const float cg_new = sqrtf(cg * cg + g * g);
  sq = cg_new;
  z = z - (g - (cg_new - cg) / hp.alpha * w);
  if (z <= hp.l1 && z >= -hp.l1) return 0.f;
  const float eta = (hp.beta + cg_new) / hp.alpha;
  return (z > 0 ? z - hp.l1 : z + hp.l1) / eta;
}

__device__ __forceinline__ void adagrad4(float4& v, float4& cg, const float4& g,
                                         const DifactoHP& hp) {
  float* pv = &v.x;
  float* pc = &cg.x;
  const float* pg = &g.x;
#pragma unroll
  for (int e = 0; e < 4; ++e) {
    const float gg = pg[e] + hp.v_l2 * pv[e];
    pc[e] = sqrtf(pc[e] * pc[e] + gg * gg);
    pv[e] -= hp.v_alpha / (pc[e] + hp.v_beta) * gg;
  }
}

__device__ __forceinline__ float l1l2_solve(float z, float eta, float l1, float l2) {
  if (z <= l1 && z >= -l1) return 0.f;
  return (z > 0 ? z - l1 : z + l1) / (eta + l2);
}

__device__ __forceinline__ float linear_update(KVSlot& e, float g, const LinearHP& hp,
                                               float sgd_eta) {
  const float oldw = e.w;
  float neww;
  if (hp.algo == 1) {
    neww = l1l2_solve(sgd_eta * oldw - g, sgd_eta, hp.l1, hp.l2);
  } else if (hp.algo == 2) {
    const float sq = sqrtf(e.sq * e.sq + g * g);
    e.sq = sq;
    const float eta = (sq + hp.beta) / hp.alpha;
    neww = l1l2_solve(eta * oldw - g, eta, hp.l1, hp.l2);
  } else if (hp.algo == 4) {
    const float gg = g + hp.l2 * oldw;
    const float cg = e.sq;
    const float cg_new = sqrtf(cg * cg + gg * gg);
    e.sq = cg_new;
    const float z = e.z - (gg - (cg_new - cg) / hp.alpha * oldw);
    e.z = z;
    neww = (z <= hp.l1 && z >= -hp.l1)
               ? 0.f
               : (z > 0 ? z - hp.l1 : z + hp.l1) / ((hp.beta + cg_new) / hp.alpha);
  } else {
    const float sq0 = e.sq;
    const float sq = sqrtf(sq0 * sq0 + g * g);
    e.sq = sq;
    const float sigma = (sq - sq0) / hp.alpha;
    const float z = e.z + g - sigma * oldw;
    e.z = z;
    neww = l1l2_solve(-z, (hp.beta + sq) / hp.alpha, hp.l1, hp.l2);
  }
  e.w = neww;
  return neww;
}

__device__ __forceinline__ void count_nnz_delta(float oldw, float neww, int64_t* stats) {
  const int d = (oldw == 0.f && neww != 0.f) ? 1 : ((oldw != 0.f && neww == 0.f) ? -1 : 0);
  long long s = wave_sum_ll(d);
  if ((threadIdx.x & 63) == 0 && s) atomicAdd(stat_ptr(stats, 0), (unsigned long long)s);
}

inline int lanes_per_key(int vstride) {
  if (vstride <= 0) return 1;
  int q = vstride / 4;
  return q >= 64 ? 64 : q;
}

}
}

#define WH_DISPATCH_G(G, KERNEL, ...)                                            \
  switch (G) {                                                                   \
    case 1: hipLaunchKernelGGL(KERNEL<1>, __VA_ARGS__); break;                   \
    case 2: hipLaunchKernelGGL(KERNEL<2>, __VA_ARGS__); break;                   \
    case 4: hipLaunchKernelGGL(KERNEL<4>, __VA_ARGS__); break;                   \
    case 8: hipLaunchKernelGGL(KERNEL<8>, __VA_ARGS__); break;                   \
    case 16: hipLaunchKernelGGL(KERNEL<16>, __VA_ARGS__); break;                 \
    case 32: hipLaunchKernelGGL(KERNEL<32>, __VA_ARGS__); break;                 \
    default: hipLaunchKernelGGL(KERNEL<64>, __VA_ARGS__); break;                 \
  }
```

csrc/hip/kvstore.hip:

```cpp
#include "wh_common.h"
#include "wh_kernels.h"
#include "wh_lookback.h"
#include "kv_device.h"

namespace wh {
namespace {

using namespace kvd;

__global__ __launch_bounds__(kThreads) void k_kv_find(const uint64_t* keys_in, int64_t n,
                                                      KVSlot* tsl, int64_t cap, int insert,
                                                      int32_t* slot, int64_t* stats) {
  const int64_t i = (int64_t)blockIdx.x * kThreads + threadIdx.x;
  bool created = false, failed = false;
  if (i < n) {
    const uint64_t k = keys_in[i];
    const uint64_t mask = (uint64_t)cap - 1;
    const uint64_t h = mix64(k) & mask;
    const int32_t res = probe_slot(tsl, mask, k, h, ld_relaxed(&tsl[h].key), insert, &created);
    if (insert && res < 0) failed = true;
    slot[i] = (int32_t)res;
  }
  const uint64_t bc = __ballot(created), bf = __ballot(failed);
  if ((threadIdx.x & 63) == 0) {
    if (bc) atomicAdd(stat_ptr(stats, 4), (unsigned long long)__popcll(bc));
    if (bf) atomicAdd(stat_ptr(stats, 2), (unsigned long long)__popcll(bf));
  }
}

__global__ __launch_bounds__(kThreads) void k_kv_occupied(const KVSlot* tsl, int64_t cap,
                                                          int32_t* out, int64_t* out_n) {
  const int64_t i = (int64_t)blockIdx.x * kThreads + threadIdx.x;
  const bool occ = i < cap && tsl[i].key != kEmptyKey;
  const uint64_t b = __ballot(occ);
  const int lane = threadIdx.x & 63;
  int64_t base = 0;
  if (lane == 0 && b)
    base = (int64_t)atomicAdd((unsigned long long*)out_n, (unsigned long long)__popcll(b));
  base = __shfl(base, 0, 64);
  if (occ) {
    const int rank = __popcll(b & ((1ull << lane) - 1));
    out[base + rank] = (int32_t)i;
  }
}

__global__ __launch_bounds__(kThreads) void k_linear_pull(const KVSlot* tsl, const int32_t* slot,
                                                          int64_t n, float* out) {
  const int64_t i = (int64_t)blockIdx.x * kThreads + threadIdx.x;
  if (i < n) {
    const int32_t s = slot[i];
    out[i] = s >= 0 ? tsl[s].w : 0.f;
  }
}

__global__ __launch_bounds__(kThreads) void k_linear_push(KVTable t, const int32_t* slot,
                                                          const float* grad, int64_t n,
                                                          LinearHP hp) {
  const int64_t i = (int64_t)blockIdx.x * kThreads + threadIdx.x;
  float oldw = 0.f, neww = 0.f;
  if (i < n) {
    const int32_t s = slot[i];
    if (s >= 0) {
      oldw = t.sl[s].w;
      neww = linear_update(t.sl[s], grad[i], hp, hp.sgd_eta);
    }
  }
  count_nnz_delta(oldw, neww, t.stats);
}



template <int G>
__global__ __launch_bounds__(kThreads) void k_difacto_push_cnt(KVTable t, const int32_t* slot,
                                                               const float* cnt,
                                                               const int32_t* cnti, int64_t n,
                                                               DifactoHP hp) {
  const int lane = threadIdx.x & 63;
  const int64_t i = (int64_t)blockIdx.x * kThreads + threadIdx.x;
  int32_t s = -1;
  bool want = false;
  if (i < n) {
    s = slot[i];
    if (s >= 0) {
      const uint32_t c = t.sl[s].cnt + (cnt ? (uint32_t)cnt[i] : (uint32_t)cnti[i]);
      t.sl[s].cnt = c;
      want = t.vstride > 0 && c > hp.threshold && t.sl[s].vrow < 0 &&
// ... 46 lines not shown
  }
  for_each_row_job<G>(row >= 0, [&](int src, int gl) {
    const int sl = src >= 0 ? src : lane;
    const int32_t jr = __shfl(row, sl, 64), jp = __shfl(vp, sl, 64);
    if (src >= 0) {
      const float* V = t.V + (int64_t)jr * t.vstride;
      float* o = vc + (int64_t)jp * t.vstride;
      for (int c = gl * 4; c < t.vstride; c += 4 * G)
        *reinterpret_cast<float4*>(o + c) = *reinterpret_cast<const float4*>(V + c);
    }
  });
}


template <int G>
__global__ __launch_bounds__(kThreads) void k_difacto_pull(KVTable t, const int32_t* slot,
                                                           int64_t n, int l1_shrk, Lookback lb,
                                                           int ntiles, float2* hdr, int64_t* vpos,
                                                           float* vc) {
  __shared__ uint32_t shs[16];
  __shared__ int sht;
  const int tile = lb_tile(lb, ntiles, &sht);
  const int lane = threadIdx.x & 63;
  const int64_t i0 = (int64_t)tile * kPullTile + threadIdx.x * kPullPer;
  int32_t sl[kPullPer];
  bool vec = false;
  if constexpr (kPullPer == 4) {
    if (i0 + kPullPer <= n && (reinterpret_cast<uintptr_t>(slot) & 15) == 0) {
      const int4 q = *reinterpret_cast<const int4*>(slot + i0);
      sl[0] = q.x; sl[1] = q.y; sl[2] = q.z; sl[3] = q.w;
      vec = true;
    }
  }
  if (!vec) {
#pragma unroll
    for (int r = 0; r < kPullPer; ++r) sl[r] = i0 + r < n ? slot[i0 + r] : -1;
  }
  float w[kPullPer];
  int32_t row[kPullPer];
#pragma unroll
  for (int r = 0; r < kPullPer; ++r) {
    w[r] = sl[r] >= 0 ? t.sl[sl[r]].w : 0.f;
    row[r] = (sl[r] >= 0 && t.vstride > 0) ? t.sl[sl[r]].vrow : -1;
  }
  uint32_t f[1] = {0u}, ex[1], tot[1];
#pragma unroll
  for (int r = 0; r < kPullPer; ++r) {
    if (l1_shrk && w[r] == 0.f) row[r] = -1;
    f[0] += row[r] >= 0 ? 1u : 0u;
  }
  lb_block_scan<1>(lb, tile, f, ex, tot, shs);
  int32_t vp[kPullPer];
  uint32_t run = ex[0];
#pragma unroll
  for (int r = 0; r < kPullPer; ++r) {
    vp[r] = row[r] >= 0 ? (int32_t)run : -1;
    if (i0 + r < n) {
      hdr[i0 + r] = make_float2(w[r], __int_as_float(vp[r]));
      vpos[i0 + r] = run;
    }
    run += row[r] >= 0 ? 1u : 0u;
  }
  if (tile == ntiles - 1 && threadIdx.x == 0) vpos[n] = tot[0];
  if (t.vstride == 0) return;
#pragma unroll
  for (int r = 0; r < kPullPer; ++r) {
    for_each_row_job<G>(row[r] >= 0, [&](int src, int gl) {
      const int sl2 = src >= 0 ? src : lane;
      const int32_t jr = __shfl(row[r], sl2, 64), jp = __shfl(vp[r], sl2, 64);
      if (src >= 0) {
        const float* V = t.V + (int64_t)jr * t.vstride;
        float* o = vc + (int64_t)jp * t.vstride;
        for (int c = gl * 4; c < t.vstride; c += 4 * G)
          *reinterpret_cast<float4*>(o + c) = *reinterpret_cast<const float4*>(V + c);
      }
    });
  }
}

template <int G>
__global__ __launch_bounds__(kThreads) void k_difacto_open_pull(
    KVTable t, const uint64_t* __restrict__ keys, int64_t n, const int32_t* __restrict__ cnt,
    DifactoHP hp, int insert, Lookback lb, int ntiles, int32_t* __restrict__ slot_out,
    float2* hdr, int64_t* vpos, float* vc) {
  __shared__ uint32_t shs[16];
  __shared__ int sht;
  const int tile = lb_tile(lb, ntiles, &sht);
  const int lane = threadIdx.x & 63;
  const int64_t i0 = (int64_t)tile * kPullTile + threadIdx.x * kPullPer;
  const uint64_t mask = (uint64_t)t.cap - 1;
  uint64_t k[kPullPer];
  int32_t sl[kPullPer];
  uint64_t h[kPullPer], prev[kPullPer];
#pragma unroll
  for (int r = 0; r < kPullPer; ++r) k[r] = i0 + r < n ? keys[i0 + r] : kEmptyKey;
#pragma unroll
  for (int r = 0; r < kPullPer; ++r) {
    h[r] = mix64(k[r]) & mask;
    prev[r] = k[r] != kEmptyKey ? ld_relaxed(&t.sl[h[r]].key) : 0;
  }
  int created = 0, failed = 0;
#pragma unroll
  for (int r = 0; r < kPullPer; ++r) {
    sl[r] = -1;
    if (k[r] == kEmptyKey) continue;
    bool cr = false;
    sl[r] = probe_slot(t.sl, mask, k[r], h[r], prev[r], insert, &cr);
    created += cr ? 1 : 0;
    if (insert && sl[r] < 0) ++failed;
    if (i0 + r < n) slot_out[i0 + r] = sl[r];
  }
  float w[kPullPer];
  int32_t row[kPullPer];
  bool fresh[kPullPer];
#pragma unroll
  for (int r = 0; r < kPullPer; ++r) {
    w[r] = 0.f;
    row[r] = -1;
    fresh[r] = false;
    if (sl[r] < 0) continue;
    KVSlot& e = t.sl[sl[r]];
    w[r] = e.w;
    row[r] = t.vstride > 0 ? e.vrow : -1;
    if (cnt) {
      const uint32_t c = e.cnt + (uint32_t)cnt[i0 + r];
      e.cnt = c;
      fresh[r] = t.vstride > 0 && c > hp.threshold && row[r] < 0 &&
                 (!hp.l1_shrk || w[r] != 0.f);
    }
  }
  long long newv = 0;
  if (cnt && t.vstride > 0) {
#pragma unroll
    for (int r = 0; r < kPullPer; ++r) {
      const int32_t nr = wave_alloc_rows(t, fresh[r]);
      fresh[r] = nr >= 0;
      if (nr >= 0) {
        t.sl[sl[r]].vrow = nr;
        row[r] = nr;
        newv += t.dim;
      }
    }
  }
  uint32_t f[1] = {0u}, ex[1], tot[1];
#pragma unroll
  for (int r = 0; r < kPullPer; ++r) {
    if (hp.l1_shrk && w[r] == 0.f) row[r] = -1;
    f[0] += row[r] >= 0 ? 1u : 0u;
  }
  const bool direct = vc == nullptr;
  lb_block_scan<1>(lb, tile, f, ex, tot, shs);
  int32_t vp[kPullPer];
  uint32_t run = ex[0];
#pragma unroll
  for (int r = 0; r < kPullPer; ++r) {
    vp[r] = row[r] >= 0 ? (int32_t)run : -1;
    if (i0 + r < n) {
      hdr[i0 + r] = make_float2(w[r], __int_as_float(direct ? row[r] : vp[r]));
      if (!direct) vpos[i0 + r] = run;
    }
    run += row[r] >= 0 ? 1u : 0u;
  }
  if (tile == ntiles - 1 && threadIdx.x == 0) vpos[n] = tot[0];
  const long long ci = wave_sum_ll(created), cf = wave_sum_ll(failed), cv = wave_sum_ll(newv);
  if (lane == 0) {
    if (ci) atomicAdd(stat_ptr(t.stats, 4), (unsigned long long)ci);
    if (cf) atomicAdd(stat_ptr(t.stats, 2), (unsigned long long)cf);
    if (cv) atomicAdd(stat_ptr(t.stats, 1), (unsigned long long)cv);
  }
  if (t.vstride == 0) return;
  if (t.vstride == 4 * G) {
    constexpr int NG = 64 / G;
    __shared__ int4 jobs[kThreads / 64][kPullPer * 64];
    int4* jl = jobs[threadIdx.x >> 6];
    int nj = 0;
#pragma unroll
    for (int r = 0; r < kPullPer; ++r) {
      const bool has = row[r] >= 0 && (!direct || fresh[r]);
      const uint64_t m = __ballot(has);
      if (has)
        jl[nj + __popcll(m & ((1ull << lane) - 1ull))] =
            make_int4(row[r], vp[r] | (fresh[r] ? (int)0x80000000 : 0), (int)(uint32_t)k[r],
                      (int)(uint32_t)(k[r] >> 32));
      nj += __popcll(m);
    }
    __builtin_amdgcn_fence(__ATOMIC_RELEASE, "wavefront");
    __builtin_amdgcn_wave_barrier();
    __builtin_amdgcn_fence(__ATOMIC_ACQUIRE, "wavefront");
    const int grp = lane / G, gl = lane & (G - 1), c = gl * 4;
    for (int j0 = 0; j0 < nj; j0 += NG * kRowBatch) {
      float4 v[kRowBatch];
#pragma unroll
      for (int b = 0; b < kRowBatch; ++b) {
        const int jj = j0 + b * NG + grp;
        v[b] = make_float4(0.f, 0.f, 0.f, 0.f);
        if (jj < nj) {
          const int4 d = jl[jj];
          if (d.y >= 0) v[b] = *reinterpret_cast<const float4*>(t.V + (int64_t)d.x * t.vstride + c);
        }
      }
#pragma unroll
      for (int b = 0; b < kRowBatch; ++b) {
        const int jj = j0 + b * NG + grp;
        if (jj >= nj) continue;
        const int4 d = jl[jj];
        const int jp = d.y & 0x7fffffff;
        if (d.y < 0) {
          const uint64_t jk = (uint64_t)(uint32_t)d.z | ((uint64_t)(uint32_t)d.w << 32);
          v[b] = v_init4(hp, jk, c, t.dim);
          *reinterpret_cast<float4*>(t.V + (int64_t)d.x * t.vstride + c) = v[b];
          *reinterpret_cast<float4*>(t.VG + (int64_t)d.x * t.vstride + c) =
              make_float4(0.f, 0.f, 0.f, 0.f);
        }
        if (!direct) *reinterpret_cast<float4*>(vc + (int64_t)jp * t.vstride + c) = v[b];
      }
    }
    return;
  }
#pragma unroll
  for (int r = 0; r < kPullPer; ++r) {
    for_each_row_job<G>(row[r] >= 0 && (!direct || fresh[r]), [&](int src, int gl) {
      const int s2 = src >= 0 ? src : lane;
      const int32_t jr = __shfl(row[r], s2, 64), jp = __shfl(vp[r], s2, 64);
      const int jf = __shfl((int)fresh[r], s2, 64);
      const uint64_t jk = __shfl(k[r], s2, 64);
      if (src < 0) return;
      float* V = t.V + (int64_t)jr * t.vstride;
      float* o = vc + (int64_t)jp * t.vstride;
      if (jf) {
        float* VG = t.VG + (int64_t)jr * t.vstride;
        for (int c = gl * 4; c < t.vstride; c += 4 * G) {
          const float4 v = v_init4(hp, jk, c, t.dim);
          *reinterpret_cast<float4*>(V + c) = v;
          *reinterpret_cast<float4*>(VG + c) = make_float4(0.f, 0.f, 0.f, 0.f);
          if (!direct) *reinterpret_cast<float4*>(o + c) = v;
        }
      } else {
        for (int c = gl * 4; c < t.vstride; c += 4 * G)
          *reinterpret_cast<float4*>(o + c) = *reinterpret_cast<const float4*>(V + c);
      }
    });
  }
}

__global__ __launch_bounds__(kThreads) void k_vidx_renumber(float2* hdr, int64_t n, Lookback lb,
                                                            int ntiles, int64_t* count) {
  __shared__ uint32_t shs[16];
  __shared__ int sht;
  const int tile = lb_tile(lb, ntiles, &sht);
  const int64_t i = (int64_t)tile * kThreads + threadIdx.x;
  const bool has = i < n && __float_as_int(hdr[i].y) >= 0;
  uint32_t f[1] = {has ? 1u : 0u}, ex[1], tot[1];
  lb_block_scan<1>(lb, tile, f, ex, tot, shs);
  if (has) hdr[i].y = __int_as_float((int32_t)ex[0]);
  if (tile == ntiles - 1 && threadIdx.x == 0) *count = tot[0];
}

__global__ __launch_bounds__(kThreads) void k_vidx_flag(const float2* hdr, int64_t n,
                                                        int32_t* flag) {
  const int64_t i = (int64_t)blockIdx.x * kThreads + threadIdx.x;
  if (i < n) flag[i] = __float_as_int(hdr[i].y) >= 0 ? 1 : 0;
}

__global__ __launch_bounds__(kThreads) void k_vidx_set(float2* hdr, int64_t n,
                                                       const int32_t* flag, const int64_t* pos) {
  const int64_t i = (int64_t)blockIdx.x * kThreads + threadIdx.x;
  if (i < n && flag[i]) hdr[i].y = __int_as_float((int32_t)pos[i]);
}

template <int G>
__global__ __launch_bounds__(kThreads) void k_difacto_push(KVTable t, const int32_t* slot,
                                                           const float2* __restrict__ hdr,
                                                           const float* __restrict__ gw,
                                                           const float* __restrict__ gvc,
                                                           int64_t n, DifactoHP hp) {
  const int lane = threadIdx.x & 63;
  const int64_t i = (int64_t)blockIdx.x * kThreads + threadIdx.x;
  float oldw = 0.f, neww = 0.f;
  bool want = false;
  int32_t s = -1, row = -1, gvid = -1;
  if (i < n) {
    s = slot[i];
    if (s >= 0) {
      if (t.vstride > 0) gvid = __float_as_int(hdr[i].y);
      const float w = t.sl[s].w;
      const float g = gw[i] + hp.l2 * w;
      const float cg = t.sl[s].sq;
      const float cg_new = sqrtf(cg * cg + g * g);
      t.sl[s].sq = cg_new;
      const float z = t.sl[s].z - (g - (cg_new - cg) / hp.alpha * w);
      t.sl[s].z = z;
      float nw;
      if (z <= hp.l1 && z >= -hp.l1) {
        nw = 0.f;
      } else {
        const float eta = (hp.beta + cg_new) / hp.alpha;
        nw = (z > 0 ? z - hp.l1 : z + hp.l1) / eta;
      }
      t.sl[s].w = nw;
      oldw = w;
      neww = nw;
      if (t.vstride > 0) {
        row = t.sl[s].vrow;
        if (w == 0.f && nw != 0.f) want = t.sl[s].cnt > hp.threshold && row < 0;
      }
    }
  }
  count_nnz_delta(oldw, neww, t.stats);
  if (t.vstride == 0) return;
  const int32_t nrow = wave_alloc_rows(t, want);
  int kind = 0;
  if (nrow >= 0) {
    t.sl[s].vrow = nrow;
    row = nrow;
    kind = 1;
  } else if (gvid >= 0 && row >= 0) {
    kind = 2;
  }
  long long newv = kind == 1 ? t.dim : 0;
  if (t.vstride == 4 * G) {
    constexpr int NG = 64 / G;
    __shared__ int4 jobs[kThreads / 64][64];
    int4* jl = jobs[threadIdx.x >> 6];
    const uint64_t m = __ballot(kind != 0);
    if (kind != 0) jl[__popcll(m & ((1ull << lane) - 1ull))] = make_int4(row, gvid, kind, s);
    const int nj = __popcll(m);
    __builtin_amdgcn_fence(__ATOMIC_RELEASE, "wavefront");
    __builtin_amdgcn_wave_barrier();
    __builtin_amdgcn_fence(__ATOMIC_ACQUIRE, "wavefront");
    const int grp = lane / G, gl = lane & (G - 1), c = gl * 4;
    for (int j0 = 0; j0 < nj; j0 += NG * kPushBatch) {
      float4 v[kPushBatch], cg[kPushBatch], g[kPushBatch];
      uint64_t kk[kPushBatch];
#pragma unroll
      for (int b = 0; b < kPushBatch; ++b) {
        const int jj = j0 + b * NG + grp;
        kk[b] = 0;
        if (jj >= nj) continue;
        const int4 d = jl[jj];
        if (d.z == 2) {
          v[b] = *reinterpret_cast<const float4*>(t.V + (int64_t)d.x * t.vstride + c);
          cg[b] = *reinterpret_cast<const float4*>(t.VG + (int64_t)d.x * t.vstride + c);
          g[b] = *reinterpret_cast<const float4*>(gvc + (int64_t)d.y * t.vstride + c);
        } else {
          kk[b] = t.sl[d.w].key;
        }
      }
#pragma unroll
      for (int b = 0; b < kPushBatch; ++b) {
        const int jj = j0 + b * NG + grp;
        if (jj >= nj) continue;
        const int4 d = jl[jj];
        float* V = t.V + (int64_t)d.x * t.vstride + c;
        float* VG = t.VG + (int64_t)d.x * t.vstride + c;
        if (d.z == 1) {
          *reinterpret_cast<float4*>(V) = v_init4(hp, kk[b], c, t.dim);
          *reinterpret_cast<float4*>(VG) = make_float4(0.f, 0.f, 0.f, 0.f);
          continue;
        }
        float* pv = &v[b].x;
        float* pc = &cg[b].x;
        const float* pg = &g[b].x;
#pragma unroll
        for (int e = 0; e < 4; ++e) {
          const float gg = pg[e] + hp.v_l2 * pv[e];
          pc[e] = sqrtf(pc[e] * pc[e] + gg * gg);
          pv[e] -= hp.v_alpha / (pc[e] + hp.v_beta) * gg;
        }
        *reinterpret_cast<float4*>(V) = v[b];
        *reinterpret_cast<float4*>(VG) = cg[b];
      }
    }
    newv = wave_sum_ll(newv);
    if (lane == 0 && newv) atomicAdd(stat_ptr(t.stats, 1), (unsigned long long)newv);
    return;
  }
  for_each_row_job<G>(kind != 0, [&](int src, int gl) {
    const int sl = src >= 0 ? src : lane;
    const int32_t js = __shfl(s, sl, 64), jr = __shfl(row, sl, 64);
    const int jk = __shfl(kind, sl, 64), jv = __shfl(gvid, sl, 64);
    if (src < 0) return;
    if (jk == 1) {
      init_v_row(t, t.sl[js].key, jr, gl, G, hp);
      return;
    }
    float* V = t.V + (int64_t)jr * t.vstride;
    float* VG = t.VG + (int64_t)jr * t.vstride;
    const float* gv = gvc + (int64_t)jv * t.vstride;
    for (int c = gl * 4; c < t.vstride; c += 4 * G) {
      float4 v = *reinterpret_cast<float4*>(V + c);
      float4 cg = *reinterpret_cast<float4*>(VG + c);
      const float4 g = *reinterpret_cast<const float4*>(gv + c);
      float* pv = &v.x;
      float* pc = &cg.x;
      const float* pg = &g.x;
#pragma unroll
      for (int e = 0; e < 4; ++e) {
        const float gg = pg[e] + hp.v_l2 * pv[e];
        pc[e] = sqrtf(pc[e] * pc[e] + gg * gg);
        pv[e] -= hp.v_alpha / (pc[e] + hp.v_beta) * gg;
      }
      *reinterpret_cast<float4*>(V + c) = v;
      *reinterpret_cast<float4*>(VG + c) = cg;
    }
  });
  newv = wave_sum_ll(newv);
  if (lane == 0 && newv) atomicAdd(stat_ptr(t.stats, 1), (unsigned long long)newv);
}

__global__ __launch_bounds__(kThreads) void k_gather_rows(const float* in, const int32_t* idx,
                                                          int64_t n, int width, float* out) {
  const int64_t tid = (int64_t)blockIdx.x * kThreads + threadIdx.x;
  if (width % 4 == 0) {
    const int q = width / 4;
    const int64_t r = tid / q, c = tid % q;
    if (r >= n) return;
    reinterpret_cast<float4*>(out + r * width)[c] =
        reinterpret_cast<const float4*>(in + (int64_t)idx[r] * width)[c];
  } else {
    const int64_t r = tid / width, c = tid % width;
    if (r >= n) return;
    out[r * width + c] = in[(int64_t)idx[r] * width + c];
  }
}

}

void kv_find(const KVTable& t, const uint64_t* keys, int64_t n, int insert, int32_t* slot,
             hipStream_t s) {
  if (n <= 0) return;
  hipLaunchKernelGGL(k_kv_find, dim3(grid_for(n, kThreads)), dim3(kThreads), 0, s, keys, n,
                     t.sl, t.cap, insert, slot, t.stats);
}

void kv_occupied(const KVTable& t, int32_t* out_slots, int64_t* out_n, hipStream_t s) {
  hipLaunchKernelGGL(k_kv_occupied, dim3(grid_for(t.cap, kThreads)), dim3(kThreads), 0, s,
                     t.sl, t.cap, out_slots, out_n);
}

void linear_pull(const KVTable& t, const int32_t* slot, int64_t n, float* out, hipStream_t s) {
  if (n <= 0) return;
  hipLaunchKernelGGL(k_linear_pull, dim3(grid_for(n, kThreads)), dim3(kThreads), 0, s, t.sl,
                     slot, n, out);
}

void linear_push(const KVTable& t, const int32_t* slot, const float* grad, int64_t n,
                 LinearHP hp, hipStream_t s) {
  if (n <= 0) return;
  hipLaunchKernelGGL(k_linear_push, dim3(grid_for(n, kThreads)), dim3(kThreads), 0, s, t, slot,
                     grad, n, hp);
}

void difacto_push_cnt(const KVTable& t, const int32_t* slot, const float* cnt,
                      const int32_t* cnti, int64_t n, DifactoHP hp, hipStream_t s) {
  if (n <= 0) return;
  const int G = lanes_per_key(t.vstride);
  const dim3 grid(grid_for(n, kThreads)), block(kThreads);
  WH_DISPATCH_G(G, k_difacto_push_cnt, grid, block, 0, s, t, slot, cnt, cnti, n, hp);
}

void difacto_pull_hdr(const KVTable& t, const int32_t* slot, int64_t n, int l1_shrk, float* hdr,
                      int32_t* vflag, hipStream_t s) {
  if (n <= 0) return;
  hipLaunchKernelGGL(k_difacto_pull_hdr, dim3(grid_for(n, kThreads)), dim3(kThreads), 0, s, t,
                     slot, n, l1_shrk, reinterpret_cast<float2*>(hdr), vflag);
}

void difacto_pull_rows(const KVTable& t, const int32_t* slot, int64_t n, const int32_t* vflag,
                       const int64_t* vpos, float* hdr, float* vc, hipStream_t s) {
  if (n <= 0 || t.vstride == 0) return;
  const int G = lanes_per_key(t.vstride);
  const dim3 grid(grid_for(n, kThreads)), block(kThreads);
  WH_DISPATCH_G(G, k_difacto_pull_rows, grid, block, 0, s, t, slot, n, vflag, vpos,
                reinterpret_cast<float2*>(hdr), vc);
}

void difacto_push(const KVTable& t, const int32_t* slot, const float* hdr, const float* gw,
                  const float* gvc, int64_t n, DifactoHP hp, hipStream_t s) {
  if (n <= 0) return;
  const int G = lanes_per_key(t.vstride);
  const dim3 grid(grid_for(n, kThreads)), block(kThreads);
  WH_DISPATCH_G(G, k_difacto_push, grid, block, 0, s, t, slot,
                reinterpret_cast<const float2*>(hdr), gw, gvc, n, hp);
}

void vidx_renumber(float* hdr, int64_t n, int32_t* flag_tmp, int64_t* pos_tmp, int64_t* scan_tmp,
                   hipStream_t s) {
  if (n <= 0) return;
  float2* h = reinterpret_cast<float2*>(hdr);
  hipLaunchKernelGGL(k_vidx_flag, dim3(grid_for(n, kThreads)), dim3(kThreads), 0, s, h, n,
                     flag_tmp);
  scan_i32(flag_tmp, pos_tmp, n, scan_tmp, s);
  hipLaunchKernelGGL(k_vidx_set, dim3(grid_for(n, kThreads)), dim3(kThreads), 0, s, h, n,
                     flag_tmp, pos_tmp);
}

void gather_rows(const float* in, const int32_t* idx, int64_t n, int width, float* out,
                 hipStream_t s) {
  if (n <= 0) return;
  const int64_t work = (width % 4 == 0) ? n * (width / 4) : n * width;
  hipLaunchKernelGGL(k_gather_rows, dim3((unsigned)((work + kThreads - 1) / kThreads)),
                     dim3(kThreads), 0, s, in, idx, n, width, out);
}

}

namespace wh {

bool difacto_pull_fused(const KVTable& t, const int32_t* slot, int64_t n, int l1_shrk,
                        const Lookback& lb, float* hdr, int64_t* vpos, float* vc, hipStream_t s) {
  const int64_t ntiles = (n + kPullTile - 1) / kPullTile;
  if (n <= 0 || ntiles > kLbMaxTiles) return false;
  const int G = lanes_per_key(t.vstride);
  const dim3 grid((unsigned)ntiles), block(kThreads);
  WH_DISPATCH_G(G, k_difacto_pull, grid, block, 0, s, t, slot, n, l1_shrk, lb, (int)ntiles,
                reinterpret_cast<float2*>(hdr), vpos, vc);
  return true;
}

bool vidx_renumber_fused(float* hdr, int64_t n, const Lookback& lb, int64_t* count,
                         hipStream_t s) {
  const int64_t ntiles = (n + kThreads - 1) / kThreads;
  if (n <= 0 || ntiles > kLbMaxTiles) return false;
  hipLaunchKernelGGL(k_vidx_renumber, dim3((unsigned)ntiles), dim3(kThreads), 0, s,
                     reinterpret_cast<float2*>(hdr), n, lb, (int)ntiles, count);
  return true;
}

}

namespace wh {

bool difacto_open_pull(const KVTable& t, const uint64_t* keys, int64_t n, const int32_t* cnt,
                       DifactoHP hp, int insert, const Lookback& lb, int32_t* slot, float* hdr,
                       int64_t* vpos, float* vc, hipStream_t s) {
  const int64_t ntiles = (n + kPullTile - 1) / kPullTile;
  if (n <= 0 || ntiles > kLbMaxTiles) return false;
  const int G = lanes_per_key(t.vstride);
  const dim3 grid((unsigned)ntiles), block(kThreads);
  WH_DISPATCH_G(G, k_difacto_open_pull, grid, block, 0, s, t, keys, n, cnt, hp, insert, lb,
                (int)ntiles, slot, reinterpret_cast<float2*>(hdr), vpos, vc);
  return true;
}

}

namespace wh {
namespace {

using namespace kvd;

__global__ __launch_bounds__(kThreads) void k_kv_rehash(const KVSlot* __restrict__ old,
                                                        int64_t oldcap, KVSlot* nt, int64_t newcap,
                                                        int32_t* remap, int64_t* stats) {
  const int64_t i = (int64_t)blockIdx.x * kThreads + threadIdx.x;
  bool failed = false;
  if (i < oldcap) {
    const KVSlot e = old[i];
    int32_t ns = -1;
    if (e.key != kEmptyKey) {
      const uint64_t mask = (uint64_t)newcap - 1;
      const uint64_t h = mix64(e.key) & mask;
      bool created = false;
      ns = probe_slot(nt, mask, e.key, h, ld_relaxed(&nt[h].key), 1, &created);
      if (ns >= 0) {
        nt[ns].w = e.w;
        nt[ns].z = e.z;
        nt[ns].sq = e.sq;
        nt[ns].cnt = e.cnt;
        nt[ns].vrow = e.vrow;
        nt[ns].tag = e.tag;
      } else {
        failed = true;
      }
    }
    remap[i] = ns;
  }
  const uint64_t bf = __ballot(failed);
  if ((threadIdx.x & 63) == 0 && bf) atomicAdd(stat_ptr(stats, 2), (unsigned long long)__popcll(bf));
}

__global__ __launch_bounds__(64) void k_kv_summary(const int64_t* stats, const int32_t* vnext,
                                                   int64_t* out) {
  const int lane = threadIdx.x;
  long long a = 0, b = 0, c = 0;
  for (int s = lane; s < kStatShards; s += 64) {
    a += stats[s * kStatStride + 4];
    b += stats[s * kStatStride + 2];
    c += stats[s * kStatStride + 3];
  }
  a = wave_sum_ll(a);
  b = wave_sum_ll(b);
  c = wave_sum_ll(c);
  if (lane == 0) {
    out[0] = a;
    out[1] = b;
    out[2] = c;
    out[3] = vnext ? (int64_t)*vnext : 0;
  }
}

}

void kv_rehash(const KVSlot* old, int64_t oldcap, KVSlot* nt, int64_t newcap, int32_t* remap,
               int64_t* stats, hipStream_t s) {
  if (oldcap <= 0) return;
  hipLaunchKernelGGL(k_kv_rehash, dim3(grid_for(oldcap, kThreads)), dim3(kThreads), 0, s, old,
                     oldcap, nt, newcap, remap, stats);
}

void kv_summary(const KVTable& t, int64_t* out, hipStream_t s) {
  hipLaunchKernelGGL(k_kv_summary, dim3(1), dim3(64), 0, s, t.stats, t.vnext, out);
}

}
```

csrc/hip/wh_kernels.h:

```cpp
#pragma once
#include <hip/hip_runtime.h>
#include <stdint.h>

namespace wh {

int64_t scan_tmp_elems(int64_t n);
void scan_i32(const int32_t* in, int64_t* out, int64_t n, int64_t* tmp, hipStream_t s);
void scan_i64(const int64_t* in, int64_t* out, int64_t n, int64_t* tmp, hipStream_t s);
constexpr int kLbMaxTiles = 1 << 16;
constexpr int kLbChannels = 2;
struct Lookback {
  unsigned long long* gran;
  unsigned int* ticket;
  unsigned int* err;
  unsigned int epoch;
};
int64_t lookback_ws_words();
Lookback lookback_bind(void* ws);

void loc_insert(const uint64_t* keys, int64_t nnz, uint64_t* tkeys, int64_t tsize,
                int32_t* slot_of, int64_t* overflow, hipStream_t s);
void key_mod(uint64_t* keys, int64_t n, uint64_t m, hipStream_t s);
int64_t loc_owner_blocks(int64_t tsize);
void loc_owner_count(const uint64_t* tkeys, int64_t tsize, int nshard, int64_t* blkcnt,
                     int64_t* owner_cnt, int64_t* overflow, hipStream_t s);
void loc_assign(uint64_t* tkeys, int64_t tsize, int nshard, const int64_t* blkoff,
                int32_t* tlid, uint64_t* uniq, hipStream_t s);
void loc_rows_lid(const int64_t* offset, int64_t nrows, const int32_t* slot_of,
                  const int32_t* tlid, int32_t* row_of, int32_t* lid, int32_t* pos,
                  hipStream_t s);
size_t loc_sort_tmp_bytes(int64_t nnz, int64_t nuniq);
void loc_csc(const int32_t* row_of, const float* val, int64_t nnz, int64_t nuniq,
             int32_t* lid, int32_t* pos,
             int32_t* slid, int32_t* spos, void* sort_tmp, size_t sort_tmp_bytes,
             int64_t* csc_off, int32_t* ucnt, int32_t* csc_row, float* csc_val, hipStream_t s);

constexpr int kPartMaxDigits = 1024;
constexpr int kPartMaxRows = 1024;
constexpr int kPartMaxOwners = 1024;
constexpr int kPartMaxHeavy = 512;
struct PartPlan {
  bool ok;
  int npo_bits, nho, stride, ndig, R;
  int64_t ntiles;
};
struct PartHeavy {
  const uint64_t* keys;
  const uint32_t* cnt;
  uint64_t* next_keys;
  uint32_t* next_cnt;
  int nho;
  int nho_next;
  uint32_t thr;
};
PartPlan loc_part_plan(int64_t nnz, int64_t nrows, int nshard, int64_t uest, bool heavy);
void loc_part_hist(const uint64_t* keys, const int64_t* offset, int64_t nrows, int nshard,
                   const PartPlan& pl, const PartHeavy& hv, uint32_t* hist, hipStream_t s);
int64_t loc_part_groups(const PartPlan& pl);
void loc_part_offsets(const PartPlan& pl, uint32_t* hist, uint32_t* gsum, int64_t* base,
                      hipStream_t s);
void loc_part_scatter(const uint64_t* keys, const float* val, const int64_t* offset,
                      int64_t nrows, int nshard, const PartPlan& pl, const PartHeavy& hv,
                      const int64_t* base, const uint32_t* gpre, const uint32_t* tpre,
                      uint64_t* pk, int32_t* pr, float* pv, int32_t* pos_of, hipStream_t s);
void loc_part_dedup(const uint64_t* pk, const int32_t* pr, const float* pv, int64_t nnz,
                    int nshard, const PartPlan& pl, const PartHeavy& hv, const int64_t* base,
                    const Lookback& lb,
                    uint64_t* uniq, int32_t* ucnt, int64_t* csc_off, int32_t* csc_row,
                    float* csc_val, int32_t* plid, unsigned long long* up, unsigned int* arrive,
                    int64_t* owner_cnt, hipStream_t s, int64_t* tim = nullptr);
void loc_part_lid(const int32_t* pos_of, const int32_t* plid, int64_t nnz, int32_t* lid,
                  hipStream_t s);
void loc_part_empty(int nshard, int64_t* owner_cnt, int64_t* csc_off, hipStream_t s);

struct alignas(32) KVSlot {
  uint64_t key;
  float w;
  float z;
  float sq;
  int32_t vrow;
  uint32_t cnt;
  uint32_t tag;
};
static_assert(sizeof(KVSlot) == 32, "KVSlot must be one 32-byte sector");
constexpr int kStatShards = 64, kStatStride = 16, kStatCount = 8;
struct KVTable {
  KVSlot* sl;
  float* V;
  float* VG;
  int32_t* vnext;
  int64_t* stats;
  int64_t cap;
  int64_t vcap;
  int vstride;
  int dim;
};
void kv_find(const KVTable& t, const uint64_t* keys, int64_t n, int insert, int32_t* slot,
             hipStream_t s);
void kv_occupied(const KVTable& t, int32_t* out_slots, int64_t* out_n, hipStream_t s);
void kv_rehash(const KVSlot* old, int64_t oldcap, KVSlot* nt, int64_t newcap, int32_t* remap,
               int64_t* stats, hipStream_t s);
void kv_summary(const KVTable& t, int64_t* out, hipStream_t s);

struct LinearHP {
  int algo;
  float alpha, beta, l1, l2;
  float sgd_eta;
};
void linear_pull(const KVTable& t, const int32_t* slot, int64_t n, float* out, hipStream_t s);
void linear_push(const KVTable& t, const int32_t* slot, const float* grad, int64_t n,
                 LinearHP hp, hipStream_t s);

struct DifactoHP {
  float alpha, beta, l1, l2;
  float v_alpha, v_beta, v_l2;
  float v_init;
  uint32_t threshold;
  int l1_shrk;
  uint64_t seed;
};
void difacto_push_cnt(const KVTable& t, const int32_t* slot, const float* cnt,
                      const int32_t* cnti, int64_t n, DifactoHP hp, hipStream_t s);
void difacto_pull_hdr(const KVTable& t, const int32_t* slot, int64_t n, int l1_shrk, float* hdr,
                      int32_t* vflag, hipStream_t s);
void difacto_pull_rows(const KVTable& t, const int32_t* slot, int64_t n, const int32_t* vflag,
                       const int64_t* vpos, float* hdr, float* vc, hipStream_t s);
void difacto_push(const KVTable& t, const int32_t* slot, const float* hdr, const float* gw,
                  const float* gvc, int64_t n, DifactoHP hp, hipStream_t s);
void vidx_renumber(float* hdr, int64_t n, int32_t* flag_tmp, int64_t* pos_tmp, int64_t* scan_tmp,
                   hipStream_t s);
bool difacto_pull_fused(const KVTable& t, const int32_t* slot, int64_t n, int l1_shrk,
                        const Lookback& lb, float* hdr, int64_t* vpos, float* vc, hipStream_t s);
bool difacto_open_pull(const KVTable& t, const uint64_t* keys, int64_t n, const int32_t* cnt,
                       DifactoHP hp, int insert, const Lookback& lb, int32_t* slot, float* hdr,
                       int64_t* vpos, float* vc, hipStream_t s);
bool vidx_renumber_fused(float* hdr, int64_t n, const Lookback& lb, int64_t* count,
                         hipStream_t s);

struct PsPrep {
  uint32_t* chain = nullptr;
  int64_t n = 0;
  int32_t* vbase = nullptr;
};
bool ps_open(const KVTable& t, const uint64_t* keys, const int32_t* rec, int64_t n, int use_cnt,
             DifactoHP hp, int insert, int chains, uint32_t epoch, int32_t* vbase,
             const int64_t* segS, const int64_t* segHS, int P, const Lookback& lb, int32_t* slot,
             float* w_out, int64_t* vpos, uint32_t* chain, uint8_t* head, float* rbuf,
             int64_t* vcnt, hipStream_t s, int prepped = 0);
bool ps_push(const KVTable& t, const int32_t* slot, const int64_t* vpos, const uint32_t* chain,
             const uint8_t* head, int64_t n, const int64_t* segS, const int64_t* segHS, int P,
             const float* gbuf, DifactoHP hp, hipStream_t s, PsPrep prep = PsPrep());
void ps_records(const uint64_t* uniq, const int32_t* ucnt, int64_t U, int32_t* rec,
                hipStream_t s);
bool ps_c0(const int64_t* owner_cnt, const int64_t* vcnt, int S, int P, int64_t flag,
           int64_t* send, int64_t* payload, hipStream_t s, int loop = 0);
bool ps_push_linear(const KVTable& t, const int32_t* slot, const uint32_t* chain,
                    const uint8_t* head, int64_t n, const int64_t* segS, int P, const float* g,
                    LinearHP hp, double t0, hipStream_t s, PsPrep prep = PsPrep());
bool ps_unpack(const float* rbuf, int64_t U, int vstride, const int64_t* segS,
               const int64_t* segHS, const int64_t* vrecv, int P, float* hdr, int64_t* rows_total,
               hipStream_t s);
bool ps_pack_gw(const float* gw, int64_t U, int vstride, const int64_t* segS,
                const int64_t* segHS, const int64_t* vrecv, int P, float* gbuf, hipStream_t s);

int64_t fm_fwd_partials();
int64_t fwd_ticket_words();
void lin_forward_strided(int64_t nrows, const int64_t* offset, const int32_t* lid,
                         const float* val, const float* w, int wstride, const float* label,
                         int loss, float* py, float* dual, double* met, double* part,
                         unsigned int* ticket, hipStream_t s);
int ld_rows_per_tile(int64_t nnz, int64_t nrows);
int ld_tile_table(int64_t nnz);
void ld_touch(const KVTable& t, const uint64_t* keys, const int64_t* off, int64_t nrows,
              int64_t nnz, int R, uint32_t stamp, int insert, int32_t* lid, int32_t* tlist,
              unsigned int* tcnt, int32_t* ovf, unsigned int* ovf_cnt, hipStream_t s);
void ld_backward(const int32_t* lid, const float* val, const int64_t* off, int64_t nrows,
                 int64_t nnz, int R, const float* dual, float* grad, hipStream_t s);
void ld_push(const KVTable& t, int64_t ntiles, int T, const int32_t* tlist,
             const unsigned int* tcnt, const int32_t* ovf, unsigned int* ovf_cnt, float* grad,
             LinearHP hp, hipStream_t s);
void fm_set_cu_reserve(int cus);
int fm_cu_reserve();
void fm_forward(int64_t nrows, const int64_t* offset, const int32_t* lid, const float* val,
                const float* w_or_hdr, const float* vc, int vstride, const float* label, int loss,
                float* py, float* dual, float* xv, double* met, double* part,
                unsigned int* ticket, hipStream_t s);
struct FmBwdProblem {
  int64_t nuniq, nnz, nrows;
  const int64_t* csc_off;
  const int32_t* csc_row;
  const float* csc_val;
  const float *dual, *xv;
  const float *hdr, *vc;
  int vstride;
  float *gw, *gvc;
  bool deterministic;
};
enum class FmBwdPhase { kAll, kPlan, kRun };
struct FmBwdLayout {
  int64_t key_s, beg_s;
  int64_t meta_v;
  int64_t hist;
  int64_t det_s, det_vw, det_v;
  int64_t off;
  int64_t cnt, scan_tmp;
};
int64_t fm_bwd_layout(int64_t nuniq, int64_t nnz, int vstride, bool deterministic,
                      FmBwdLayout* out = nullptr);
void fm_backward(const FmBwdProblem& p, void* scratch, const Lookback* lb, hipStream_t s,
                 FmBwdPhase phase);
void fm_grad_post(const int64_t* m, int64_t m_cap, float* gvc, int vstride, int dim, float clip,
                  float dropout, uint64_t seed, double* sumsq, hipStream_t s);
void fm_grad_scale(const int64_t* m, int64_t m_cap, float* gvc, int vstride, int dim,
                   const double* sumsq, hipStream_t s);

void spmv(int64_t nrows, const int64_t* off, const int32_t* col, const float* val, const float* x,
          float* y, hipStream_t s);
size_t auc_sort_tmp_bytes(int64_t n);
void sort_by_score(const float* py, const float* label, int64_t n, float* py_sorted,
                   float* label_sorted, void* tmp, size_t tmp_bytes, hipStream_t s);
void auc_from_sorted(const float* label_sorted, int64_t n, double* out, int64_t* tmp_i64,
                     hipStream_t s);
int64_t auc_ws_bytes(int64_t n);
int64_t auc_ws_persistent_bytes();
int64_t auc_ws_lohi_offset();
void auc_accumulate(const float* py, const float* label, int64_t n, void* persist, void* scratch,
                    double* auc_sum, hipStream_t s);

void synth_criteo(int64_t nrows, uint64_t seed, uint64_t step, const int64_t* card,
                  int nfield, uint64_t* keys, float* label, int64_t* offset, hipStream_t s);

int kmeans_ks(int f);
bool kmeans_x3_supported(int f);
int64_t kmeans_x3_xp_bytes(int64_t n, int f);
int64_t kmeans_x3_cp_bytes(int k, int f);
void kmeans_pack_x3(const float* X, int64_t n, int f, void* Xp3, hipStream_t s);
void kmeans_pack_c3(const float* C, int k, int f, void* Cp3, hipStream_t s);
void kmeans_assign_x3(const void* Xp3, const float* xnorm, const float* X, int64_t n, int f,
                      const void* Cp3, const float* C, int k, int32_t* assign, float* score,
                      int32_t* amb, float* ct, hipStream_t s);
void kmeans_pack_x(const float* X, int64_t n, int f, float* Xp, hipStream_t s);
int64_t kmeans_cp_elems(int k, int f);
void kmeans_pack_c(const float* C, int k, int f, float* Cp, hipStream_t s);
void kmeans_assign(const float* Xp, int64_t n, int f, const float* Cp, int k, int32_t* assign,
                   float* score, hipStream_t s);
void kmeans_accum(const float* X, int64_t n, int f, const int32_t* assign, float* sums,
                  hipStream_t s);
int64_t kmeans_accum_scratch(int64_t n, int k);
void kmeans_assign_csr(const int64_t* off, const int32_t* col, const float* val, int64_t n,
                       const float* Ct, int K, int Kp, int32_t* assign, hipStream_t s);
void kmeans_accum_csr(const int64_t* off, const int32_t* col, const float* val, int64_t n,
                      const int32_t* assign, int F, float* sums, hipStream_t s);
void kmeans_update(const float* sums, const float* C, int k, int f, float* out,
                   unsigned long long* nempty, hipStream_t s);
bool kmeans_accum_sorted(const float* X, int64_t n, int f, int k, const int32_t* assign,
                         float* sums, void* scratch, hipStream_t s);

void owlqn_dir(const float* g, const float* w, int64_t n, float l1, float* d, hipStream_t s);
int64_t owlqn_part_doubles();
void owlqn_fix_dot(float* d, const float* steep, int64_t n, int fix, double* part, double* vdot,
                   hipStream_t s);
void owlqn_step(const float* w, const float* d, int64_t n, float alpha, int fix, float* nw,
                double* part, double* l1sum, hipStream_t s);
bool hist_dots(const float* H, int R, int64_t n, int64_t ld, const int32_t* probe, int K,
               double* part, double* out, hipStream_t s);
bool dir_fix_dot(const float* H, int64_t n, int64_t ld, const int32_t* rows, const float* coef,
                 int nrow, int steep_row, int fix, float* d, double* part, double* vdot,
                 hipStream_t s);
bool multi_dot(const float* H, int R, int64_t n, const int32_t* ia, const int32_t* ib, int np,
               double* out, hipStream_t s);

void sum_parts(const double* part, int nblk, int nv, double* out, hipStream_t s, int stride = 0);
int64_t glm_fwd_blocks(int64_t nrows);
void glm_fwd(int mode, int64_t nrows, const int64_t* off, const int32_t* gcol, const float* val,
             const float* w, const float* bias, float base, const float* label, int loss,
             float* out, double* part, double* sums, hipStream_t s);
void glm_grad_from_margin(int64_t nrows, const float* margin, const float* label, int loss,
                          float* g, double* part, double* sums, hipStream_t s);
int64_t glm_xtg_waves(int64_t nnz);
void glm_runs_reduce(int64_t ncol, const int64_t* coff, const int32_t* rlist, const float* S,
                     const int32_t* cgid, float* grad, hipStream_t s);
int64_t glm_heads_words(int64_t nnz);
void glm_heads(const int64_t* csc_off, int64_t U, uint64_t* hb, int64_t words, hipStream_t s);
void glm_xtg(int64_t nnz, const int32_t* crow, const float* cval, const uint64_t* hb,
             const int32_t* col0w, const int32_t* ucol, const float* g, float* grad,
             int all_atomic, hipStream_t s);

void gbdt_bin(const float* X, int64_t n, int f, const float* cuts, const int32_t* cut_off,
              uint8_t* B, hipStream_t s);
size_t gbdt_hist_lds(int fcnt, int nbin);
int64_t gbdt_hist_pstride(int max_fcnt, int nbin);
// ... 109 lines not shown
```

csrc/hip/wh_lookback.h:

```cpp
#pragma once
#include <hip/hip_runtime.h>
#include <stdint.h>

#include "wh_kernels.h"

namespace wh {

__device__ __forceinline__ unsigned long long lb_load(const unsigned long long* p) {
  return __hip_atomic_load(p, __ATOMIC_RELAXED, __HIP_MEMORY_SCOPE_AGENT);
}
__device__ __forceinline__ void lb_store(unsigned long long* p, unsigned long long v) {
  __hip_atomic_store(p, v, __ATOMIC_RELAXED, __HIP_MEMORY_SCOPE_AGENT);
}

constexpr int kArriveGroups = 16;
constexpr int kArriveStride = 16;
constexpr int kArriveWords = (kArriveGroups + 1) * kArriveStride;
__device__ __forceinline__ bool arrive_last(unsigned int* ticket, unsigned bid, unsigned nb) {
  const unsigned ng = nb < (unsigned)kArriveGroups ? nb : (unsigned)kArriveGroups;
  const unsigned g = bid % ng, gsize = (nb - g + ng - 1) / ng;
  unsigned int* gc = ticket + g * kArriveStride;
  if (atomicAdd(gc, 1u) != gsize - 1) return false;
  __hip_atomic_store(gc, 0u, __ATOMIC_RELAXED, __HIP_MEMORY_SCOPE_AGENT);
  unsigned int* fc = ticket + kArriveGroups * kArriveStride;
// ... 30 lines not shown
  if (tile == 0) {
    if (lane == 0) lb_store(g, tag_i | agg);
    return 0;
  }
  if (lane == 0) lb_store(g + tile, tag_a | agg);
  uint32_t run = 0;
  int base = tile - 1;
  while (true) {
    unsigned long long v[kW];
#pragma unroll
    for (int j = 0; j < kW; ++j) {
      const int t = base - (j * 64 + lane);
      v[j] = t >= 0 ? lb_load(g + t) : tag_i;
    }
    unsigned spins = 0;
    while (true) {
      bool ready = true;
#pragma unroll
      for (int j = 0; j < kW; ++j) {
        const unsigned long long tg = v[j] & hi;
        ready &= tg == tag_a || tg == tag_i;
      }
      if (__all(ready)) break;
      if (++spins > (1u << 22)) {
        if (lane == 0) atomicOr(lb.err, 1u);
#pragma unroll
        for (int j = 0; j < kW; ++j) v[j] = tag_i;
        break;
      }
      __builtin_amdgcn_s_sleep(1);
#pragma unroll
      for (int j = 0; j < kW; ++j) {
        const unsigned long long tg = v[j] & hi;
        const int t = base - (j * 64 + lane);
        if (tg != tag_a && tg != tag_i && t >= 0) v[j] = lb_load(g + t);
      }
    }
    bool done = false;
#pragma unroll
    for (int j = 0; j < kW; ++j) {
      if (done) break;
      const uint64_t inc = __ballot((v[j] & hi) == tag_i);
      const int first = inc ? __ffsll((unsigned long long)inc) - 1 : 63;
      run += lb_wave_sum(lane <= first ? (uint32_t)v[j] : 0u);
      done = inc != 0;
    }
    if (done) break;
    base -= 64 * kW;
  }
  if (lane == 0) lb_store(g + tile, tag_i | (uint32_t)(run + agg));
  return run;
}

template <int NV>
__device__ __forceinline__ void lb_block_scan(const Lookback& lb, int tile, const uint32_t (&v)[NV],
                                              uint32_t (&excl)[NV], uint32_t (&total)[NV],
                                              uint32_t* sh) {
  const int lane = threadIdx.x & 63, wid = threadIdx.x >> 6;
  const int nw = blockDim.x >> 6;
  uint32_t inc[NV];
#pragma unroll
  for (int c = 0; c < NV; ++c) {
    uint32_t x = v[c];
#pragma unroll
    for (int o = 1; o < 64; o <<= 1) {
      const uint32_t y = __shfl_up(x, o, 64);
      if (lane >= o) x += y;
    }
    inc[c] = x;
    if (lane == 63) sh[c * 4 + wid] = x;
  }
  __syncthreads();
  uint32_t wbase[NV], btot[NV];
#pragma unroll
  for (int c = 0; c < NV; ++c) {
    wbase[c] = 0;
    btot[c] = 0;
    for (int i = 0; i < nw; ++i) {
      const uint32_t s = sh[c * 4 + i];
      if (i < wid) wbase[c] += s;
      btot[c] += s;
    }
  }
  if (wid == 0) {
#pragma unroll
    for (int c = 0; c < NV; ++c) {
      const uint32_t p = lb_exclusive(lb, c, tile, btot[c]);
      if (lane == 0) sh[8 + c] = p;
    }
  }
  __syncthreads();
#pragma unroll
  for (int c = 0; c < NV; ++c) {
    const uint32_t p = sh[8 + c];
    excl[c] = p + wbase[c] + inc[c] - v[c];
    total[c] = p + btot[c];
  }
}

}
```

wormhole_amd/models/difacto.py:

```python

import os

import torch

from .. import ops
from ._pipeline import begin_next, localize_current
from ..kv import ShardedKV, make_store
from ..utils import trace

TRAIN, VAL, PRED = 0, 1, 2


class DifactoLearner:
    def __init__(self, conf, comm, device, cap=1 << 22, vcap=1 << 20, seed=0, nshard=None):
        self.conf = conf
        self.comm = comm
        self.device = torch.device(device)
        emb = conf.embedding[0] if conf.embedding else None
        self.dim = emb.dim if emb is not None else 0
        self.emb = emb
        self.vstride = ops.vstride_for(self.dim)
        self.store = make_store(cap, vcap, self.dim, self.device)
        self.kv = ShardedKV(self.store, comm, nshard, fixed_bytes=getattr(conf, "fixed_bytes", 0),
                            seed=seed)
        if hasattr(comm, "set_compression"):
            comm.set_compression(getattr(conf, "msg_compression", False))
        self.seed = seed
        self.l1_shrk = bool(conf.l1_shrk)
        if emb is not None:
            v_alpha = emb.lr_eta if emb.has("lr_eta") else conf.lr_eta
            v_beta = emb.lr_beta if emb.has("lr_beta") else conf.lr_beta
            self.hp = [conf.lr_eta, conf.lr_beta, conf.lambda_l1, conf.lambda_l2,
                       v_alpha, v_beta, emb.lambda_l2, emb.init_scale]
            self.threshold = int(emb.threshold)
        else:
            self.hp = [conf.lr_eta, conf.lr_beta, conf.lambda_l1, conf.lambda_l2,
                       conf.lr_eta, conf.lr_beta, 0.0, 0.01]
            self.threshold = 0
        self.met = torch.zeros(4, dtype=torch.float64, device=self.device)
        self.auc_sum = torch.zeros(1, dtype=torch.float64, device=self.device)
        self.n_mb = 0
        self.max_key = 0
        self._job = None
        self.uhint = 0
        self.defer_push = True
        self.step = 0
        self.last_sizes = None
        self.loss = ops.LOSS_LOGIT
        self.last_empty = False
        post = emb is not None and (emb.grad_clipping > 0 or emb.dropout > 0
                                    or bool(emb.grad_normalization))
        self.direct_pull = (self.device.type == "cuda" and comm.size == 1 and self.vstride > 0
                            and not post)
        self.psx = None
        if comm.size > 1:
            from ..kv.psx import Psx
            self.psx = Psx(self)
        self._nat = None
        if (self.psx is None and self.device.type == "cuda" and self.vstride > 0
                and os.environ.get("WH_DIFACTO_NATIVE", "1") != "0"):
            from .. import _native
            e = emb
            self._nat = _native.hip().DifactoStep(
                store=self.store, hp=[float(x) for x in self.hp], threshold=self.threshold,
                l1_shrk=self.l1_shrk, seed=int(seed), loss=int(self.loss),
                post=[float(e.grad_clipping), float(e.dropout),
                      1.0 if e.grad_normalization else 0.0, float(self.dim)],
                max_load=float(self.kv.guard.max_load), direct=self.direct_pull)

    def psx_linear_hp(self):
        c = self.conf
        return 4, float(c.lr_eta), float(c.lr_beta), float(c.lambda_l1), float(c.lambda_l2)

    def process(self, keys, offset, val, label, wtype=TRAIN, data_pass=0, next_batch=None):
        train = wtype == TRAIN
        if self.psx is not None:
            if train:
                self.psx.train(keys, offset, val, label, data_pass, next_batch)
                self.last_empty = self.psx.last_empty
                return None
            py = self.psx.evaluate(keys, offset, val, label)
            self.last_empty = self.psx.last_empty
            return py if wtype == PRED else None
        self.last_empty = offset.numel() <= 1 and self.comm.size == 1
        if self._nat is not None and not self.max_key:
            nk = no = nv = None
            ready = 0
            if next_batch is not None:
                nk, no, nv = next_batch[:3]
                if len(next_batch) > 3 and next_batch[3] is not None:
                    ready = next_batch[3].cuda_event
            py, u, m = self._nat.step(keys=keys, offset=offset, val=val, label=label,
                                      train=train, data_pass=int(data_pass), met=self.met,
                                      auc_sum=self.auc_sum, step=self.step, next_keys=nk,
                                      next_offset=no, next_val=nv, ready=ready)
            self.last_sizes = (u, m)
            if label.numel():
                self.n_mb += 1
            self.step += 1
            return py if wtype == PRED else None
        with trace.span("localize"):
            loc = localize_current(self, keys, offset, val)
        uniq, ucnt, owner_cnt, lid, csc_off, csc_row, csc_val = loc[:7]
        self.uhint = uniq.numel()
        push_cnt = train and data_pass == 0 and self.dim > 0
        with trace.span("pull"):
            sess, hdr, vc = self.kv.difacto_open_pull(
                uniq, owner_cnt, train, ucnt if push_cnt else None, self.hp, self.threshold,
                self.l1_shrk, self.seed, recv=loc[7] if len(loc) > 7 else None,
                direct=self.direct_pull)
        self.last_sizes = (uniq.numel(), sess.m)
        if next_batch is not None:
            begin_next(self, next_batch, uniq.numel())
        if self.vstride == 0:
            hdr, vc = hdr[:, 0].contiguous(), None
        with trace.span("forward"):
            py, dual, xv = ops.fm_forward(offset, lid, val, hdr, vc, self.vstride, label,
                                          ops.LOSS_LOGIT, self.met)
            if not train:
                ops.auc_acc(py, label, self.auc_sum)
        if label.numel():
            self.n_mb += 1
        if train:
            with trace.span("backward"):
                gw, gvc = ops.fm_backward(csc_off, csc_row, csc_val, dual, xv, hdr, vc,
                                          self.vstride)
                if self.emb is not None and self.vstride > 0:
                    ops.fm_grad_post(gvc, sess.m, self.dim, self.emb.grad_clipping,
                                     self.emb.dropout, self.seed + 7919 * self.step + 1,
                                     bool(self.emb.grad_normalization))
            ops.auc_acc(py, label, self.auc_sum)
            with trace.span("push"):
                self.kv.difacto_push(sess, gw, gvc, self.hp, self.threshold, self.l1_shrk,
                                     self.seed, defer=self.defer_push)
        self.step += 1
        return py if wtype == PRED else None

    def flush(self):
        if self.psx is not None:
            self.psx.flush()
        if self._nat is not None:
            g = self.kv.guard
            g.grows, g.vgrows = max(g.grows, self._nat.grows), max(g.vgrows, self._nat.vgrows)
        self.kv.flush()

    def take_progress(self):
        self.kv.flush()
        ops.auc_join(self.auc_sum)
        m = self.met.tolist()
        a = float(self.auc_sum.item())
        st = self.store.stats
# ... 8 lines not shown
```

Baseline: 137.9 million examples/s.

## Fuse backward chunk planning into open-pull and V AdaGrad update into backward

Has the open/pull kernel emit the backward pass's chunk plan through a third lookback channel, so no separate planning pass is needed. Adds a fused mode where the V-gradient backward kernel applies the AdaGrad update directly to the embedding table instead of writing gvc for a later push. The push can then take unique counts. The changes target kernel launches and gradient round-trips through memory, at the cost of more complex kernels and a wider lookback scan. Fused V is on by default through an environment flag.

```diff
diff --git a/csrc/bind/hip_ops.cc b/csrc/bind/hip_ops.cc
--- a/csrc/bind/hip_ops.cc
+++ b/csrc/bind/hip_ops.cc
@@ -709,6 +709,16 @@
                                         const c10::optional<Tensor>& cnt,
                                         const std::vector<double>& h, int64_t threshold,
                                         bool l1_shrk, int64_t seed, bool direct) {
+    return difacto_open_pull(keys, insert, cnt, h, threshold, l1_shrk, seed, direct, nullptr,
+                             nullptr);
+  }
+
+  std::vector<Tensor> difacto_open_pull(const Tensor& keys, bool insert,
+                                        const c10::optional<Tensor>& cnt,
+                                        const std::vector<double>& h, int64_t threshold,
+                                        bool l1_shrk, int64_t seed, bool direct,
+                                        const wh::FmBwdPlanDst* plan, bool* planned) {
+    if (planned) *planned = false;
     CHECK_IN(keys, torch::kInt64);
     const int32_t* cp = nullptr;
     if (cnt.has_value() && cnt->defined()) {
@@ -732,18 +742,25 @@
     if (!wh::difacto_open_pull(table(), reinterpret_cast<const uint64_t*>(keys.data_ptr()), n,
                                cp, dhp(h, threshold, l1_shrk, seed), insert ? 1 : 0,
                                lookback(keys.device()), ptr<int32_t>(slot), ptr<float>(hdr),
-                               ptr<int64_t>(vpos), direct ? nullptr : ptr<float>(vc), s)) {
+                               ptr<int64_t>(vpos), direct ? nullptr : ptr<float>(vc), s, plan)) {
       slot = find(keys, insert);
       if (cp) difacto_push_cnt(slot, *cnt, h, threshold, l1_shrk, seed);
       auto r = difacto_pull(slot, l1_shrk);
       return {slot, r[0], r[1], r[2]};
     }
+    if (planned) *planned = plan != nullptr;
     return {slot, hdr, vc, vpos};
   }
 
   void difacto_push(const Tensor& slot, const Tensor& hdr, const Tensor& gw, const Tensor& gvc,
                     const std::vector<double>& h, int64_t threshold, bool l1_shrk,
                     int64_t seed) {
+    difacto_push_after(slot, hdr, gw, gvc, h, threshold, l1_shrk, seed, c10::nullopt);
+  }
+
+  void difacto_push_after(const Tensor& slot, const Tensor& hdr, const Tensor& gw,
+                          const Tensor& gvc, const std::vector<double>& h, int64_t threshold,
+                          bool l1_shrk, int64_t seed, const c10::optional<Tensor>& ucnt) {
     CHECK_IN(slot, torch::kInt32);
     CHECK_IN(hdr, torch::kFloat32);
     CHECK_IN(gw, torch::kFloat32);
@@ -752,10 +769,16 @@
     TORCH_CHECK(hdr.numel() == 2 * n && gw.numel() == n, "push: hdr/gw size mismatch");
     TORCH_CHECK(vstride_ == 0 || (gvc.dim() == 2 && gvc.size(1) == vstride_),
                 "push: gvc must be [m, vstride]");
+    const int32_t* uc = nullptr;
+    if (ucnt.has_value()) {
+      CHECK_IN((*ucnt), torch::kInt32);
+      TORCH_CHECK(ucnt->numel() >= n, "push: count size mismatch");
+      uc = ptr<int32_t>(*ucnt);
+    }
     c10::DeviceGuard g(slot.device());
     wh::difacto_push(table(), ptr<int32_t>(slot), ptr<float>(hdr), ptr<float>(gw),
                      gvc.numel() ? ptr<float>(gvc) : nullptr, n, dhp(h, threshold, l1_shrk, seed),
-                     cur_stream(slot));
+                     cur_stream(slot), uc);
   }
 
   std::vector<Tensor> ps_open(const Tensor& keys, bool use_cnt, const Tensor& segS,
@@ -1045,10 +1068,16 @@
           vstride > 0 ? torch::empty({vc_rows, vstride}, f32) : torch::empty({0}, f32), scratch};
 }
 
+struct FmFuse {
+  float *v, *vg;
+  wh::DifactoHP hp;
+};
+
 static void fm_bwd_launch(const std::vector<Tensor>& pl, const Tensor& csc_off,
                           const Tensor& csc_row, const float* csc_val, const float* dual,
                           const float* xv, const float* hdr, const float* vc, int64_t vstride,
-                          int64_t nrows, wh::FmBwdPhase phase, bool two_pass = false) {
+                          int64_t nrows, wh::FmBwdPhase phase, bool two_pass = false,
+                          const FmFuse* fuse = nullptr) {
   wh::FmBwdProblem p;
   p.nuniq = csc_off.numel() - 1;
   p.nnz = csc_row.numel();
@@ -1064,6 +1093,11 @@
   p.gw = ptr<float>(pl[0]);
   p.gvc = pl[1].numel() ? ptr<float>(pl[1]) : nullptr;
   p.deterministic = deterministic();
+  if (fuse) {
+    p.fuse_v = fuse->v;
+    p.fuse_vg = fuse->vg;
+    p.fuse_hp = fuse->hp;
+  }
   const wh::Lookback lb = lookback(csc_off.device());
   wh::fm_backward(p, pl[2].data_ptr(), two_pass ? nullptr : &lb, cur_stream(csc_off), phase);
 }
@@ -1088,19 +1122,50 @@
   return vc->numel() ? vc->size(0) : 0;
 }
 
+static wh::FmBwdPlanDst fm_bwd_plan_dst(const std::vector<Tensor>& pl, const Tensor& csc_off,
+                                        int64_t nnz, int64_t nrows, int64_t vstride) {
+  wh::FmBwdProblem p = {};
+  p.nuniq = csc_off.numel() - 1;
+  p.nnz = nnz;
+  p.nrows = nrows;
+  p.csc_off = ptr<int64_t>(csc_off);
+  p.vstride = (int)vstride;
+  p.gw = ptr<float>(pl[0]);
+  p.gvc = pl[1].numel() ? ptr<float>(pl[1]) : nullptr;
+  p.deterministic = deterministic();
+  return wh::fm_bwd_plan_dst(p, pl[2].data_ptr());
+}
+
+static std::vector<Tensor> fm_backward_impl(const Tensor& csc_off, const Tensor& csc_row,
+                                            const c10::optional<Tensor>& csc_val,
+                                            const Tensor& dual, const c10::optional<Tensor>& xv,
+                                            const Tensor& w_or_hdr,
+                                            const c10::optional<Tensor>& vc, int64_t vstride,
+                                            const FmFuse* fuse,
+                                            const std::vector<Tensor>* planned = nullptr) {
+  fm_bwd_check(csc_off, csc_row, w_or_hdr, vstride);
+  const int64_t vrows = fm_bwd_check_run(dual, xv, vc, vstride);
+  c10::DeviceGuard g(csc_off.device());
+  if (planned) {
+    TORCH_CHECK((*planned)[1].numel() == vrows * vstride, "backward: gvc rows differ from vc's");
+    fm_bwd_launch(*planned, csc_off, csc_row, optptr<float>(csc_val), ptr<float>(dual),
+                  optptr<float>(xv), ptr<float>(w_or_hdr), optptr<float>(vc), vstride,
+                  dual.numel(), wh::FmBwdPhase::kBucketRun, false, fuse);
+    return {(*planned)[0], (*planned)[1]};
+  }
+  auto pl = fm_bwd_alloc(csc_off, csc_row.numel(), vrows, vstride, true);
+  fm_bwd_launch(pl, csc_off, csc_row, optptr<float>(csc_val), ptr<float>(dual),
+                vstride > 0 ? optptr<float>(xv) : nullptr, ptr<float>(w_or_hdr),
+                vstride > 0 ? optptr<float>(vc) : nullptr, vstride, dual.numel(),
+                wh::FmBwdPhase::kAll, false, fuse);
+  return {pl[0], pl[1]};
+}
+
 std::vector<Tensor> fm_backward(const Tensor& csc_off, const Tensor& csc_row,
                                 const c10::optional<Tensor>& csc_val, const Tensor& dual,
                                 const c10::optional<Tensor>& xv, const Tensor& w_or_hdr,
                                 const c10::optional<Tensor>& vc, int64_t vstride) {
-  fm_bwd_check(csc_off, csc_row, w_or_hdr, vstride);
-  const int64_t vrows = fm_bwd_check_run(dual, xv, vc, vstride);
-  c10::DeviceGuard g(csc_off.device());
-  auto pl = fm_bwd_alloc(csc_off, csc_row.numel(), vrows, vstride, true);
-  fm_bwd_launch(pl, csc_off, csc_row, optptr<float>(csc_val), ptr<float>(dual),
-                vstride > 0 ? optptr<float>(xv) : nullptr, ptr<float>(w_or_hdr),
-                vstride > 0 ? optptr<float>(vc) : nullptr, vstride, dual.numel(),
-                wh::FmBwdPhase::kAll);
-  return {pl[0], pl[1]};
+  return fm_backward_impl(csc_off, csc_row, csc_val, dual, xv, w_or_hdr, vc, vstride, nullptr);
 }
 
 std::vector<Tensor> fm_backward_plan(const Tensor& csc_off, const Tensor& csc_row,
@@ -1144,6 +1209,40 @@
                 vstride > 0 ? optptr<float>(vc) : nullptr, vstride, dual.numel(),
                 wh::FmBwdPhase::kRun);
   return {gw, gvc};
+}
+
+py::tuple difacto_open_pull_plan(KVStore& store, const Tensor& keys, bool insert,
+                                 const c10::optional<Tensor>& cnt, const std::vector<double>& h,
+                                 int64_t threshold, bool l1_shrk, int64_t seed, bool direct,
+                                 const Tensor& csc_off, const Tensor& csc_row, int64_t nrows) {
+  CHECK_IN(csc_off, torch::kInt64);
+  CHECK_IN(csc_row, torch::kInt32);
+  TORCH_CHECK(csc_off.numel() == keys.numel() + 1, "open_pull_plan: csc_off must have U + 1");
+  c10::DeviceGuard g(keys.device());
+  const int64_t vstride = store.vstride();
+  check_vstride(vstride);
+  TORCH_CHECK(vstride > 0, "open_pull_plan: an embedding store");
+  const int64_t vrows = direct ? store.V_.size(0) : keys.numel();
+  auto pl = fm_bwd_alloc(csc_off, csc_row.numel(), vrows, vstride, false);
+  const wh::FmBwdPlanDst dst = fm_bwd_plan_dst(pl, csc_off, csc_row.numel(), nrows, vstride);
+  bool planned = false;
+  auto o = store.difacto_open_pull(keys, insert, cnt, h, threshold, l1_shrk, seed, direct, &dst,
+                                   &planned);
+  if (!planned) return py::make_tuple(o[0], o[1], o[2], o[3], std::vector<Tensor>());
+  fm_bwd_launch(pl, csc_off, csc_row, nullptr, nullptr, nullptr, ptr<float>(o[1]), nullptr,
+                vstride, nrows, wh::FmBwdPhase::kBucket);
+  return py::make_tuple(o[0], o[1], o[2], o[3], pl);
+}
+
+Tensor fm_backward_plan_totals(const std::vector<Tensor>& plan, const Tensor& csc_off,
+                               int64_t nnz, int64_t vstride) {
+  TORCH_CHECK(plan.size() == 3, "not a backward plan");
+  const wh::FmBwdPlanDst d = fm_bwd_plan_dst(plan, csc_off, nnz, 0, vstride);
+  const int64_t base = reinterpret_cast<int64_t>(plan[2].data_ptr());
+  const int64_t a = reinterpret_cast<int64_t>(d.tot_s) - base;
+  const int64_t b = reinterpret_cast<int64_t>(d.tot_v) - base;
+  auto i64 = plan[2].view(torch::kInt64);
+  return torch::stack({i64[a / 8], i64[b / 8]});
 }
 
 void fm_grad_post(const Tensor& gvc, const Tensor& m, int64_t dim, double clip, double dropout,
@@ -3149,10 +3248,10 @@
         "one rank's per-peer all-to-all-v plan: (esz, (own_src, own_dst, own_bytes), sends, recvs)");
   py::class_<DifactoStep>(m, "DifactoStep")
       .def(py::init<KVStore*, std::vector<double>, int64_t, bool, int64_t, int64_t,
-                    std::vector<double>, double, bool>(),
+                    std::vector<double>, double, bool, bool>(),
            py::arg("store"), py::arg("hp"), py::arg("threshold"), py::arg("l1_shrk"),
            py::arg("seed"), py::arg("loss"), py::arg("post"), py::arg("max_load"),
-           py::arg("direct"), py::keep_alive<1, 2>())
+           py::arg("direct"), py::arg("fused_v") = true, py::keep_alive<1, 2>())
       .def("step", &DifactoStep::step, py::arg("keys"), py::arg("offset"), py::arg("val"),
            py::arg("label"), py::arg("train"), py::arg("data_pass"), py::arg("met"),
            py::arg("auc_sum"), py::arg("step"), py::arg("next_keys") = py::none(),
@@ -3161,6 +3260,7 @@
       .def("reset", &DifactoStep::reset)
       .def("guard_sync", &DifactoStep::guard_sync)
       .def_property_readonly("direct", &DifactoStep::direct)
+      .def_property_readonly("fused_v", &DifactoStep::fused_v)
       .def_property_readonly("grows", &DifactoStep::grows)
       .def_property_readonly("vgrows", &DifactoStep::vgrows);
   m.def("c10d_a2a_rows", &c10d_a2a_rows, py::arg("pg"), py::arg("x"), py::arg("send_rows"),
@@ -3176,6 +3276,14 @@
         py::arg("hdr"), py::arg("vc_rows"), py::arg("nrows"), py::arg("vstride"),
         py::arg("two_pass") = false);
   m.def("fm_backward_run", &fm_backward_run);
+  m.def("difacto_open_pull_plan", &difacto_open_pull_plan, py::arg("store"), py::arg("keys"),
+        py::arg("insert"), py::arg("cnt"), py::arg("h"), py::arg("threshold"),
+        py::arg("l1_shrk"), py::arg("seed"), py::arg("direct"), py::arg("csc_off"),
+        py::arg("csc_row"), py::arg("nrows"),
+        "(tests) the open with the backward's chunk plan: (slot, hdr, vc, vpos, plan)");
+  m.def("fm_backward_plan_totals", &fm_backward_plan_totals, py::arg("plan"),
+        py::arg("csc_off"), py::arg("nnz"), py::arg("vstride"),
+        "(tests) a backward plan's chunk totals {scalar, V}");
   m.def("fm_grad_post", &fm_grad_post);
   m.def("vidx_renumber", &vidx_renumber);
   m.def("ps_unpack", &ps_unpack);
@@ -3284,7 +3392,11 @@
       .def("linear_push", &KVStore::linear_push)
       .def("difacto_push_cnt", &KVStore::difacto_push_cnt)
       .def("difacto_pull", &KVStore::difacto_pull)
-      .def("difacto_open_pull", &KVStore::difacto_open_pull, py::arg("keys"), py::arg("insert"),
+      .def("difacto_open_pull",
+           py::overload_cast<const Tensor&, bool, const c10::optional<Tensor>&,
+                             const std::vector<double>&, int64_t, bool, int64_t, bool>(
+               &KVStore::difacto_open_pull),
+           py::arg("keys"), py::arg("insert"),
            py::arg("cnt"), py::arg("h"), py::arg("threshold"), py::arg("l1_shrk"), py::arg("seed"),
            py::arg("direct") = false)
       .def("difacto_push", &KVStore::difacto_push)
diff --git a/csrc/hip/fm.hip b/csrc/hip/fm.hip
--- a/csrc/hip/fm.hip
+++ b/csrc/hip/fm.hip
@@ -1,5 +1,7 @@
 #include "wh_common.h"
 #include <string>
+#include "kv_device.h"
+#include "wh_chunk_plan.h"
 #include "wh_kernels.h"
 #include "wh_lookback.h"
 #include "wh_loss.h"
@@ -12,7 +14,6 @@
 namespace {
 
 constexpr int kThreads = 256;
-constexpr int kChunk = 32;
 constexpr int kFwdBlocks = 2048;
 
 template <int G>
@@ -209,64 +210,9 @@
   block_partials(part, sh, m_objv, m_objv, m_corr, m_n, met, ticket, acc5);
 }
 
-constexpr int kChunkV = 64;
-
-__device__ __forceinline__ int64_t key_chunks(int64_t cnt, bool isv) {
-  return isv ? (cnt + kChunkV - 1) / kChunkV : (cnt + kChunk - 1) / kChunk;
-}
 
 __device__ __forceinline__ int32_t key_vidx(const float2* __restrict__ hdr, int64_t k) {
   return hdr ? __float_as_int(hdr[k].y) : -1;
-}
-
-struct ChunkOut {
-  int32_t* key_s;
-  int32_t* beg_s;
-  int4* meta_v;
-  float* gw;
-  float* gvc;
-  int vstride;
-};
-
-__device__ __forceinline__ void emit_key(const ChunkOut& o, int32_t k, int64_t c0, int32_t nc,
-                                         int32_t b0, int32_t cnt, int32_t vid, int isv) {
-  const int lane = threadIdx.x & 63;
-  if (nc == 1) {
-    if (isv) {
-      o.meta_v[c0] = make_int4(k, b0, cnt, vid);
-    } else {
-      o.key_s[c0] = k;
-      o.beg_s[c0] = b0;
-    }
-  }
-  uint64_t m = __ballot(nc > 1);
-  while (m) {
-    const int src = __ffsll((unsigned long long)m) - 1;
-    m &= m - 1;
-    const int32_t jk = __shfl(k, src, 64);
-    const int64_t jc0 = __shfl(c0, src, 64);
-    const int32_t jnc = __shfl(nc, src, 64);
-    const int32_t jb0 = __shfl(b0, src, 64);
-    const int32_t jcnt = __shfl(cnt, src, 64);
-    const int32_t jvid = __shfl(vid, src, 64);
-    const int jv = __shfl(isv, src, 64);
-    for (int32_t q = lane; q < jnc; q += 64) {
-      if (jv) {
-        const int32_t cb = q * kChunkV;
-        const int32_t n = jcnt - cb < kChunkV ? jcnt - cb : kChunkV;
-        o.meta_v[jc0 + q] = make_int4(jk, jb0 + cb, n | (1 << 8), jvid);
-      } else {
-        o.key_s[jc0 + q] = jk;
-        o.beg_s[jc0 + q] = jb0 + q * kChunk;
-      }
-    }
-    if (lane == 0) o.gw[jk] = 0.f;
-    if (jv) {
-      for (int d = lane * 4; d < o.vstride; d += 256)
-        *reinterpret_cast<float4*>(o.gvc + (int64_t)jvid * o.vstride + d) =
-            make_float4(0.f, 0.f, 0.f, 0.f);
-    }
-  }
 }
 
 __global__ __launch_bounds__(kThreads) void k_chunk_count(int64_t nuniq,
@@ -462,7 +408,7 @@
   const int k = chunk_key[c];
   const int kb = (int)csc_off[k], ke = (int)csc_off[k + 1];
   const int b = chunk_beg[c];
-  const int e = b + kChunk < ke ? b + kChunk : ke;
+  const int e = b + kChunkS < ke ? b + kChunkS : ke;
   float gw = 0.f;
   int p = b;
   for (; p + 3 < e; p += 4) {
@@ -477,12 +423,12 @@
     for (int u = 0; u < 4; ++u) gw += dual[i[u]] * x[u];
   }
   for (; p < e; ++p) gw += dual[csc_row[p]] * (csc_val ? csc_val[p] : 1.f);
-  if (ke - kb <= kChunk) gw_out[k] = gw;
+  if (ke - kb <= kChunkS) gw_out[k] = gw;
   else if (part_gw) part_gw[c] = gw;
   else atomicAdd(gw_out + k, gw);
 }
 
-template <int G>
+template <int G, bool FUSED>
 __global__ __launch_bounds__(kThreads) void k_bwd_v(const int64_t* __restrict__ nchunk_p,
                                                     const int4* __restrict__ meta,
                                                     const int32_t* __restrict__ csc_row,
@@ -493,8 +439,11 @@
                                                     float* __restrict__ gw_out,
                                                     float* __restrict__ gvc,
                                                     float* __restrict__ part_gw,
-                                                    float* __restrict__ part_gv) {
+                                                    float* __restrict__ part_gv, float* fv,
+                                                    float* fvg, DifactoHP hp) {
   using S = Shape<G>;
+  constexpr bool kSplit = 64 / G >= 4;
+  const float* vrows = FUSED ? fv : vc;
   __shared__ int2 stage[kThreads / 64][64];
   int2* st = stage[threadIdx.x >> 6];
   const int lane = threadIdx.x & 63, gl = lane & (G - 1), sub = lane / G;
@@ -523,6 +472,7 @@
     const bool multi = (mc.z >> 8) != 0;
     float4 acc = make_float4(0.f, 0.f, 0.f, 0.f);
     float4 v = make_float4(0.f, 0.f, 0.f, 0.f);
+    float4 vg = make_float4(0.f, 0.f, 0.f, 0.f);
     stage_pairs<G>(st, lane, rc, dc);
     auto batch = [&](auto tb, int t0) {
       constexpr int TB = decltype(tb)::value;
@@ -536,7 +486,11 @@
         a[t] = reinterpret_cast<const float4*>(src)[gl];
       }
       if (t0 == 0) {
-        v = reinterpret_cast<const float4*>(vc + (uint32_t)mc.w * (uint32_t)S::VS)[gl];
+        v = reinterpret_cast<const float4*>(vrows + (uint32_t)mc.w * (uint32_t)S::VS)[gl];
+        if (FUSED && !multi) {
+          if (kSplit) vg.x = fvg[(uint32_t)mc.w * (uint32_t)S::VS + gl * 4 + (sub & 3)];
+          else vg = reinterpret_cast<const float4*>(fvg + (uint32_t)mc.w * (uint32_t)S::VS)[gl];
+        }
         dn = rn >= 0 ? dual[rn] * xn : 0.f;
         load_rows(m2, r2, x2);
         m3 = get_meta(c + 3 * nw);
@@ -574,7 +528,25 @@
       else atomicAdd(gw_out + mc.x, gw);
     }
     acc.x -= xxp * v.x; acc.y -= xxp * v.y; acc.z -= xxp * v.z; acc.w -= xxp * v.w;
-    if (!multi || part_gv) {
+    if (FUSED && !multi) {
+      if (kSplit) {
+        const int comp = sub & 3;
+        const float a = comp == 0 ? acc.x : comp == 1 ? acc.y : comp == 2 ? acc.z : acc.w;
+        float v1 = comp == 0 ? v.x : comp == 1 ? v.y : comp == 2 ? v.z : v.w;
+        kvd::adagrad1(v1, vg.x, a, hp);
+        if (sub < 4) {
+          const uint32_t at = (uint32_t)mc.w * (uint32_t)S::VS + gl * 4 + comp;
+          fv[at] = v1;
+          fvg[at] = vg.x;
+        }
+      } else {
+        kvd::adagrad4(v, vg, acc, hp);
+        if (sub == 0) {
+          reinterpret_cast<float4*>(fv + (uint32_t)mc.w * (uint32_t)S::VS)[gl] = v;
+          reinterpret_cast<float4*>(fvg + (uint32_t)mc.w * (uint32_t)S::VS)[gl] = vg;
+        }
+      }
+    } else if (!multi || part_gv) {
       float* dst = multi ? part_gv + c * (int64_t)vstride : gvc + (int64_t)mc.w * vstride;
       if (sub == 0) *reinterpret_cast<float4*>(dst + gl * 4) = acc;
     } else {
@@ -606,8 +578,8 @@
   if (c >= *nchunk_p) return;
   const int k = chunk_key[c];
   const int64_t kb = csc_off[k], cnt = csc_off[k + 1] - kb;
-  if (cnt <= kChunk || chunk_beg[c] != kb) return;
-  const int64_t n = (cnt + kChunk - 1) / kChunk;
+  if (cnt <= kChunkS || chunk_beg[c] != kb) return;
+  const int64_t n = (cnt + kChunkS - 1) / kChunkS;
   float s = 0.f;
   for (int64_t q = 0; q < n; ++q) s += part_gw[c + q];
   gw_out[k] = s;
@@ -752,7 +724,7 @@
                      wstride, label, loss, py, dual, part, met, ticket, acc5);
 }
 
-static int64_t scalar_cap(int64_t nuniq, int64_t nnz) { return nuniq + nnz / kChunk + 1; }
+static int64_t scalar_cap(int64_t nuniq, int64_t nnz) { return nuniq + nnz / kChunkS + 1; }
 static int64_t v_cap(int64_t nuniq, int64_t nnz) { return nuniq + nnz / kChunkV + 1; }
 
 static int bucket_shift(int64_t nrows) {
@@ -785,6 +757,16 @@
   return at;
 }
 
+FmBwdPlanDst fm_bwd_plan_dst(const FmBwdProblem& p, void* scratch) {
+  FmBwdLayout l;
+  fm_bwd_layout(p.nuniq, p.nnz, p.vstride, p.deterministic, &l);
+  char* base = static_cast<char*>(scratch);
+  int64_t* off_s = reinterpret_cast<int64_t*>(base + l.off);
+  return {p.csc_off, reinterpret_cast<int32_t*>(base + l.key_s),
+          reinterpret_cast<int32_t*>(base + l.beg_s), base + l.meta_v, p.gw, p.gvc, p.vstride,
+          off_s + p.nuniq, off_s + p.nuniq + 1 + p.nuniq};
+}
+
 void fm_backward(const FmBwdProblem& p, void* scratch, const Lookback* lb, hipStream_t s,
                  FmBwdPhase phase) {
   const int64_t nuniq = p.nuniq;
@@ -803,7 +785,7 @@
   const bool bucket =
       hdr && !p.deterministic && p.nrows * (int64_t)vstride * 4 > ((int64_t)2 << 20);
   int4* meta_sorted = bucket ? meta_v + cap_v : meta_v;
-  if (phase != FmBwdPhase::kRun) {
+  if (phase == FmBwdPhase::kAll || phase == FmBwdPhase::kPlan) {
     const ChunkOut out = {key_s, beg_s, meta_v, p.gw, p.gvc, vstride};
     const int64_t ntiles = (nuniq + kPlanTile - 1) / kPlanTile;
     if (lb && ntiles <= kLbMaxTiles) {
@@ -821,17 +803,17 @@
       hipLaunchKernelGGL(k_chunk_fill, grid, dim3(kThreads), 0, s, nuniq, p.csc_off, off_s, off_v,
                          hdr, out);
     }
-    if (bucket) {
-      int32_t* hist = reinterpret_cast<int32_t*>(base + l.hist);
-      const int shift = bucket_shift(std::max<int64_t>(p.nrows, 1));
-      hipLaunchKernelGGL(k_vchunk_hist, dim3(kBucketBlocks), dim3(kThreads), 0, s, off_v + nuniq,
-                         meta_v, p.csc_row, shift, hist);
-      hipLaunchKernelGGL(k_vchunk_scan, dim3(1), dim3(kBuckets * kScanParts), 0, s, hist);
-      hipLaunchKernelGGL(k_vchunk_scatter, dim3(kBucketBlocks), dim3(kThreads), 0, s,
-                         off_v + nuniq, meta_v, p.csc_row, shift, hist, meta_sorted);
-    }
-  }
-  if (phase == FmBwdPhase::kPlan) return;
+  }
+  if (phase != FmBwdPhase::kRun && bucket) {
+    int32_t* hist = reinterpret_cast<int32_t*>(base + l.hist);
+    const int shift = bucket_shift(std::max<int64_t>(p.nrows, 1));
+    hipLaunchKernelGGL(k_vchunk_hist, dim3(kBucketBlocks), dim3(kThreads), 0, s, off_v + nuniq,
+                       meta_v, p.csc_row, shift, hist);
+    hipLaunchKernelGGL(k_vchunk_scan, dim3(1), dim3(kBuckets * kScanParts), 0, s, hist);
+    hipLaunchKernelGGL(k_vchunk_scatter, dim3(kBucketBlocks), dim3(kThreads), 0, s,
+                       off_v + nuniq, meta_v, p.csc_row, shift, hist, meta_sorted);
+  }
+  if (phase == FmBwdPhase::kPlan || phase == FmBwdPhase::kBucket) return;
   const bool det = p.deterministic;
   float* pgs = det ? reinterpret_cast<float*>(base + l.det_s) : nullptr;
   float* pgv_w = det ? reinterpret_cast<float*>(base + l.det_vw) : nullptr;
@@ -845,11 +827,18 @@
   if (!hdr) return;
   dispatch_g(vstride / 4, [&](auto g) {
     constexpr int G = decltype(g)::value;
-    const int64_t vblk =
-        std::min<int64_t>((cap_v + 3) / 4, resident_blocks(k_bwd_v<G>, 2048));
-    hipLaunchKernelGGL(k_bwd_v<G>, dim3((unsigned)vblk), dim3(kThreads), 0, s, off_v + nuniq,
-                       meta_sorted, p.csc_row, p.csc_val, p.dual, p.xv, p.vc, vstride, p.gw,
-                       p.gvc, pgv_w, pgv);
+    auto run = [&](auto kernel, const float* vc) {
+      const int64_t vblk = std::min<int64_t>((cap_v + 3) / 4, resident_blocks(kernel, 2048));
+      hipLaunchKernelGGL(kernel, dim3((unsigned)vblk), dim3(kThreads), 0, s, off_v + nuniq,
+                         meta_sorted, p.csc_row, p.csc_val, p.dual, p.xv, vc, vstride, p.gw,
+                         p.gvc, pgv_w, pgv, p.fuse_v, p.fuse_vg, p.fuse_hp);
+    };
+    if (p.fuse_v && p.fuse_v != p.vc) {
+      fprintf(stderr, "fm.hip: the fused update needs vc to be the V slab itself\n");
+      abort();
+    }
+    if (p.fuse_v) run(k_bwd_v<G, true>, nullptr);
+    else run(k_bwd_v<G, false>, p.vc);
   });
   if (det)
     hipLaunchKernelGGL(k_bwd_reduce_v, dim3(grid_for(cap_v * 64, kThreads)), dim3(kThreads), 0, s,
diff --git a/csrc/hip/kv_device.h b/csrc/hip/kv_device.h
--- a/csrc/hip/kv_device.h
+++ b/csrc/hip/kv_device.h
@@ -90,17 +90,19 @@
   return (z > 0 ? z - hp.l1 : z + hp.l1) / eta;
 }
 
+__device__ __forceinline__ void adagrad1(float& v, float& cg, float g, const DifactoHP& hp) {
+  const float gg = __fmaf_rn(hp.v_l2, v, g);
+  cg = sqrtf(__fadd_rn(__fmul_rn(cg, cg), __fmul_rn(gg, gg)));
+  const float eta = __fdiv_rn(hp.v_alpha, __fadd_rn(cg, hp.v_beta));
+  v = __fmaf_rn(-eta, gg, v);
+}
+
 __device__ __forceinline__ void adagrad4(float4& v, float4& cg, const float4& g,
                                          const DifactoHP& hp) {
-  float* pv = &v.x;
-  float* pc = &cg.x;
-  const float* pg = &g.x;
-#pragma unroll
-  for (int e = 0; e < 4; ++e) {
-    const float gg = pg[e] + hp.v_l2 * pv[e];
-    pc[e] = sqrtf(pc[e] * pc[e] + gg * gg);
-    pv[e] -= hp.v_alpha / (pc[e] + hp.v_beta) * gg;
-  }
+  adagrad1(v.x, cg.x, g.x, hp);
+  adagrad1(v.y, cg.y, g.y, hp);
+  adagrad1(v.z, cg.z, g.z, hp);
+  adagrad1(v.w, cg.w, g.w, hp);
 }
 
 __device__ __forceinline__ float l1l2_solve(float z, float eta, float l1, float l2) {
diff --git a/csrc/hip/kvstore.hip b/csrc/hip/kvstore.hip
--- a/csrc/hip/kvstore.hip
+++ b/csrc/hip/kvstore.hip
@@ -2,6 +2,7 @@
 #include "wh_kernels.h"
 #include "wh_lookback.h"
 #include "kv_device.h"
+#include "wh_chunk_plan.h"
 
 namespace wh {
 namespace {
@@ -214,7 +215,7 @@
 __global__ __launch_bounds__(kThreads) void k_difacto_open_pull(
     KVTable t, const uint64_t* __restrict__ keys, int64_t n, const int32_t* __restrict__ cnt,
     DifactoHP hp, int insert, Lookback lb, int ntiles, int32_t* __restrict__ slot_out,
-    float2* hdr, int64_t* vpos, float* vc) {
+    float2* hdr, int64_t* vpos, float* vc, ChunkPlanArg plan) {
   __shared__ uint32_t shs[16];
   __shared__ int sht;
   const int tile = lb_tile(lb, ntiles, &sht);
@@ -226,6 +227,10 @@
   uint64_t h[kPullPer], prev[kPullPer];
 #pragma unroll
   for (int r = 0; r < kPullPer; ++r) k[r] = i0 + r < n ? keys[i0 + r] : kEmptyKey;
+  int64_t co[kPullPer + 1];
+#pragma unroll
+  for (int r = 0; r <= kPullPer; ++r)
+    co[r] = plan.csc_off && i0 + r <= n ? plan.csc_off[i0 + r] : 0;
 #pragma unroll
   for (int r = 0; r < kPullPer; ++r) {
     h[r] = mix64(k[r]) & mask;
@@ -274,14 +279,27 @@
       }
     }
   }
-  uint32_t f[1] = {0u}, ex[1], tot[1];
+  uint32_t f[3] = {0u, 0u, 0u}, ex[3], tot[3];
+  uint32_t nc[kPullPer];
 #pragma unroll
   for (int r = 0; r < kPullPer; ++r) {
     if (hp.l1_shrk && w[r] == 0.f) row[r] = -1;
     f[0] += row[r] >= 0 ? 1u : 0u;
+    nc[r] = plan.csc_off && i0 + r < n ? (uint32_t)key_chunks(co[r + 1] - co[r], row[r] >= 0)
+                                       : 0u;
+    if (row[r] >= 0) f[2] += nc[r];
+    else f[1] += nc[r];
   }
   const bool direct = vc == nullptr;
-  lb_block_scan<1>(lb, tile, f, ex, tot, shs);
+  if (plan.csc_off) {
+    lb_block_scan<3>(lb, tile, f, ex, tot, shs);
+  } else {
+    const uint32_t f1[1] = {f[0]};
+    uint32_t ex1[1], tot1[1];
+    lb_block_scan<1>(lb, tile, f1, ex1, tot1, shs);
+    ex[0] = ex1[0];
+    tot[0] = tot1[0];
+  }
   int32_t vp[kPullPer];
   uint32_t run = ex[0];
 #pragma unroll
@@ -294,6 +312,20 @@
     run += row[r] >= 0 ? 1u : 0u;
   }
   if (tile == ntiles - 1 && threadIdx.x == 0) vpos[n] = tot[0];
+  if (plan.csc_off) {
+    if (tile == ntiles - 1 && threadIdx.x == 0) {
+      *plan.tot_s = tot[1];
+      *plan.tot_v = tot[2];
+    }
+#pragma unroll
+    for (int r = 0; r < kPullPer; ++r) {
+      const int isv = row[r] >= 0;
+      emit_key(plan.out, (int32_t)(i0 + r), isv ? ex[2] : ex[1], (int32_t)nc[r], (int32_t)co[r],
+               (int32_t)(co[r + 1] - co[r]), direct ? row[r] : vp[r], isv);
+      if (isv) ex[2] += nc[r];
+      else ex[1] += nc[r];
+    }
+  }
   const long long ci = wave_sum_ll(created), cf = wave_sum_ll(failed), cv = wave_sum_ll(newv);
   if (lane == 0) {
     if (ci) atomicAdd(stat_ptr(t.stats, 4), (unsigned long long)ci);
@@ -405,7 +437,8 @@
                                                            const float2* __restrict__ hdr,
                                                            const float* __restrict__ gw,
                                                            const float* __restrict__ gvc,
-                                                           int64_t n, DifactoHP hp) {
+                                                           int64_t n, DifactoHP hp,
+                                                           const int32_t* __restrict__ ucnt) {
   const int lane = threadIdx.x & 63;
   const int64_t i = (int64_t)blockIdx.x * kThreads + threadIdx.x;
   float oldw = 0.f, neww = 0.f;
@@ -446,7 +479,7 @@
     t.sl[s].vrow = nrow;
     row = nrow;
     kind = 1;
-  } else if (gvid >= 0 && row >= 0) {
+  } else if (gvid >= 0 && row >= 0 && !(ucnt && ucnt[i] <= kChunkV)) {
     kind = 2;
   }
   long long newv = kind == 1 ? t.dim : 0;
@@ -490,15 +523,7 @@
           *reinterpret_cast<float4*>(VG) = make_float4(0.f, 0.f, 0.f, 0.f);
           continue;
         }
-        float* pv = &v[b].x;
-        float* pc = &cg[b].x;
-        const float* pg = &g[b].x;
-#pragma unroll
-        for (int e = 0; e < 4; ++e) {
-          const float gg = pg[e] + hp.v_l2 * pv[e];
-          pc[e] = sqrtf(pc[e] * pc[e] + gg * gg);
-          pv[e] -= hp.v_alpha / (pc[e] + hp.v_beta) * gg;
-        }
+        adagrad4(v[b], cg[b], g[b], hp);
         *reinterpret_cast<float4*>(V) = v[b];
         *reinterpret_cast<float4*>(VG) = cg[b];
       }
@@ -522,16 +547,7 @@
     for (int c = gl * 4; c < t.vstride; c += 4 * G) {
       float4 v = *reinterpret_cast<float4*>(V + c);
       float4 cg = *reinterpret_cast<float4*>(VG + c);
-      const float4 g = *reinterpret_cast<const float4*>(gv + c);
-      float* pv = &v.x;
-      float* pc = &cg.x;
-      const float* pg = &g.x;
-#pragma unroll
-      for (int e = 0; e < 4; ++e) {
-        const float gg = pg[e] + hp.v_l2 * pv[e];
-        pc[e] = sqrtf(pc[e] * pc[e] + gg * gg);
-        pv[e] -= hp.v_alpha / (pc[e] + hp.v_beta) * gg;
-      }
+      adagrad4(v, cg, *reinterpret_cast<const float4*>(gv + c), hp);
       *reinterpret_cast<float4*>(V + c) = v;
       *reinterpret_cast<float4*>(VG + c) = cg;
     }
@@ -608,12 +624,12 @@
 }
 
 void difacto_push(const KVTable& t, const int32_t* slot, const float* hdr, const float* gw,
-                  const float* gvc, int64_t n, DifactoHP hp, hipStream_t s) {
+                  const float* gvc, int64_t n, DifactoHP hp, hipStream_t s, const int32_t* ucnt) {
   if (n <= 0) return;
   const int G = lanes_per_key(t.vstride);
   const dim3 grid(grid_for(n, kThreads)), block(kThreads);
   WH_DISPATCH_G(G, k_difacto_push, grid, block, 0, s, t, slot,
-                reinterpret_cast<const float2*>(hdr), gw, gvc, n, hp);
+                reinterpret_cast<const float2*>(hdr), gw, gvc, n, hp, ucnt);
 }
 
 void vidx_renumber(float* hdr, int64_t n, int32_t* flag_tmp, int64_t* pos_tmp, int64_t* scan_tmp,
@@ -665,13 +681,13 @@
 
 bool difacto_open_pull(const KVTable& t, const uint64_t* keys, int64_t n, const int32_t* cnt,
                        DifactoHP hp, int insert, const Lookback& lb, int32_t* slot, float* hdr,
-                       int64_t* vpos, float* vc, hipStream_t s) {
+                       int64_t* vpos, float* vc, hipStream_t s, const FmBwdPlanDst* plan) {
   const int64_t ntiles = (n + kPullTile - 1) / kPullTile;
   if (n <= 0 || ntiles > kLbMaxTiles) return false;
   const int G = lanes_per_key(t.vstride);
   const dim3 grid((unsigned)ntiles), block(kThreads);
   WH_DISPATCH_G(G, k_difacto_open_pull, grid, block, 0, s, t, keys, n, cnt, hp, insert, lb,
-                (int)ntiles, slot, reinterpret_cast<float2*>(hdr), vpos, vc);
+                (int)ntiles, slot, reinterpret_cast<float2*>(hdr), vpos, vc, chunk_plan_arg(plan));
   return true;
 }
 
diff --git a/csrc/hip/wh_chunk_plan.h b/csrc/hip/wh_chunk_plan.h
--- /dev/null
+++ b/csrc/hip/wh_chunk_plan.h
@@ -0,0 +1,81 @@
+#pragma once
+#include <hip/hip_runtime.h>
+#include <stdint.h>
+
+#include "wh_kernels.h"
+
+namespace wh {
+
+constexpr int kChunkS = 32;
+
+__device__ __forceinline__ int64_t key_chunks(int64_t cnt, bool isv) {
+  return isv ? (cnt + kChunkV - 1) / kChunkV : (cnt + kChunkS - 1) / kChunkS;
+}
+
+struct ChunkOut {
+  int32_t* key_s;
+  int32_t* beg_s;
+  int4* meta_v;
+  float* gw;
+  float* gvc;
+  int vstride;
+};
+
+struct ChunkPlanArg {
+  const int64_t* csc_off;
+  ChunkOut out;
+  int64_t* tot_s;
+  int64_t* tot_v;
+};
+
+inline ChunkPlanArg chunk_plan_arg(const FmBwdPlanDst* d) {
+  ChunkPlanArg a = {};
+  if (d)
+    a = {d->csc_off,
+         {d->key_s, d->beg_s, static_cast<int4*>(d->meta_v), d->gw, d->gvc, d->vstride},
+         d->tot_s, d->tot_v};
+  return a;
+}
+
+__device__ __forceinline__ void emit_key(const ChunkOut& o, int32_t k, int64_t c0, int32_t nc,
+                                         int32_t b0, int32_t cnt, int32_t vid, int isv) {
+  const int lane = threadIdx.x & 63;
+  if (nc == 1) {
+    if (isv) {
+      o.meta_v[c0] = make_int4(k, b0, cnt, vid);
+    } else {
+      o.key_s[c0] = k;
+      o.beg_s[c0] = b0;
+    }
+  }
+  uint64_t m = __ballot(nc > 1);
+  while (m) {
+    const int src = __ffsll((unsigned long long)m) - 1;
+    m &= m - 1;
+    const int32_t jk = __shfl(k, src, 64);
+    const int64_t jc0 = __shfl(c0, src, 64);
+    const int32_t jnc = __shfl(nc, src, 64);
+    const int32_t jb0 = __shfl(b0, src, 64);
+    const int32_t jcnt = __shfl(cnt, src, 64);
+    const int32_t jvid = __shfl(vid, src, 64);
+    const int jv = __shfl(isv, src, 64);
+    for (int32_t q = lane; q < jnc; q += 64) {
+      if (jv) {
+        const int32_t cb = q * kChunkV;
+        const int32_t n = jcnt - cb < kChunkV ? jcnt - cb : kChunkV;
+        o.meta_v[jc0 + q] = make_int4(jk, jb0 + cb, n | (1 << 8), jvid);
+      } else {
+        o.key_s[jc0 + q] = jk;
+        o.beg_s[jc0 + q] = jb0 + q * kChunkS;
+      }
+    }
+    if (lane == 0) o.gw[jk] = 0.f;
+    if (jv) {
+      for (int d = lane * 4; d < o.vstride; d += 256)
+        *reinterpret_cast<float4*>(o.gvc + (int64_t)jvid * o.vstride + d) =
+            make_float4(0.f, 0.f, 0.f, 0.f);
+    }
+  }
+}
+
+}
diff --git a/csrc/hip/wh_kernels.h b/csrc/hip/wh_kernels.h
--- a/csrc/hip/wh_kernels.h
+++ b/csrc/hip/wh_kernels.h
@@ -8,7 +8,7 @@
 void scan_i32(const int32_t* in, int64_t* out, int64_t n, int64_t* tmp, hipStream_t s);
 void scan_i64(const int64_t* in, int64_t* out, int64_t n, int64_t* tmp, hipStream_t s);
 constexpr int kLbMaxTiles = 1 << 16;
-constexpr int kLbChannels = 2;
+constexpr int kLbChannels = 3;
 struct Lookback {
   unsigned long long* gran;
   unsigned int* ticket;
@@ -126,14 +126,17 @@
 void difacto_pull_rows(const KVTable& t, const int32_t* slot, int64_t n, const int32_t* vflag,
                        const int64_t* vpos, float* hdr, float* vc, hipStream_t s);
 void difacto_push(const KVTable& t, const int32_t* slot, const float* hdr, const float* gw,
-                  const float* gvc, int64_t n, DifactoHP hp, hipStream_t s);
+                  const float* gvc, int64_t n, DifactoHP hp, hipStream_t s,
+                  const int32_t* ucnt = nullptr);
 void vidx_renumber(float* hdr, int64_t n, int32_t* flag_tmp, int64_t* pos_tmp, int64_t* scan_tmp,
                    hipStream_t s);
 bool difacto_pull_fused(const KVTable& t, const int32_t* slot, int64_t n, int l1_shrk,
                         const Lookback& lb, float* hdr, int64_t* vpos, float* vc, hipStream_t s);
+struct FmBwdPlanDst;
 bool difacto_open_pull(const KVTable& t, const uint64_t* keys, int64_t n, const int32_t* cnt,
                        DifactoHP hp, int insert, const Lookback& lb, int32_t* slot, float* hdr,
-                       int64_t* vpos, float* vc, hipStream_t s);
+                       int64_t* vpos, float* vc, hipStream_t s,
+                       const FmBwdPlanDst* plan = nullptr);
 bool vidx_renumber_fused(float* hdr, int64_t n, const Lookback& lb, int64_t* count,
                          hipStream_t s);
 
@@ -195,8 +198,12 @@
   int vstride;
   float *gw, *gvc;
   bool deterministic;
-};
-enum class FmBwdPhase { kAll, kPlan, kRun };
+  float* fuse_v = nullptr;
+  float* fuse_vg = nullptr;
+  DifactoHP fuse_hp = {};
+};
+constexpr int kChunkV = 64;
+enum class FmBwdPhase { kAll, kPlan, kRun, kBucket, kBucketRun };
 struct FmBwdLayout {
   int64_t key_s, beg_s;
   int64_t meta_v;
@@ -207,6 +214,15 @@
 };
 int64_t fm_bwd_layout(int64_t nuniq, int64_t nnz, int vstride, bool deterministic,
                       FmBwdLayout* out = nullptr);
+struct FmBwdPlanDst {
+  const int64_t* csc_off;
+  int32_t *key_s, *beg_s;
+  void* meta_v;
+  float *gw, *gvc;
+  int vstride;
+  int64_t *tot_s, *tot_v;
+};
+FmBwdPlanDst fm_bwd_plan_dst(const FmBwdProblem& p, void* scratch);
 void fm_backward(const FmBwdProblem& p, void* scratch, const Lookback* lb, hipStream_t s,
                  FmBwdPhase phase);
 void fm_grad_post(const int64_t* m, int64_t m_cap, float* gvc, int vstride, int dim, float clip,
diff --git a/csrc/hip/wh_lookback.h b/csrc/hip/wh_lookback.h
--- a/csrc/hip/wh_lookback.h
+++ b/csrc/hip/wh_lookback.h
@@ -136,17 +136,19 @@
       btot[c] += s;
     }
   }
-  if (wid == 0) {
+  const bool split = nw >= NV;
+  if (split ? wid < NV : wid == 0) {
 #pragma unroll
     for (int c = 0; c < NV; ++c) {
+      if (split && wid != c) continue;
       const uint32_t p = lb_exclusive(lb, c, tile, btot[c]);
-      if (lane == 0) sh[8 + c] = p;
+      if (lane == 0) sh[4 * NV + c] = p;
     }
   }
   __syncthreads();
 #pragma unroll
   for (int c = 0; c < NV; ++c) {
-    const uint32_t p = sh[8 + c];
+    const uint32_t p = sh[4 * NV + c];
     excl[c] = p + wbase[c] + inc[c] - v[c];
     total[c] = p + btot[c];
   }
diff --git a/wormhole_amd/models/difacto.py b/wormhole_amd/models/difacto.py
--- a/wormhole_amd/models/difacto.py
+++ b/wormhole_amd/models/difacto.py
@@ -66,7 +66,8 @@
                 l1_shrk=self.l1_shrk, seed=int(seed), loss=int(self.loss),
                 post=[float(e.grad_clipping), float(e.dropout),
                       1.0 if e.grad_normalization else 0.0, float(self.dim)],
-                max_load=float(self.kv.guard.max_load), direct=self.direct_pull)
+                max_load=float(self.kv.guard.max_load), direct=self.direct_pull,
+                fused_v=os.environ.get("WH_DIFACTO_FUSED_V", "1") != "0")
 
     def psx_linear_hp(self):
         c = self.conf
```

Result: faster. 140.9 million examples/s, median of 6 (+2.1%).
